# Gancheekim/ATM-VFI

Hardware: AMD Instinct MI355X
Metric: interpolated frames/s at 1080p (network_base, bs=1) (higher is better)
Workload: dtype f32 (contractions as fp16 hi/lo split x3 MFMA, fp32 accumulate; ~22 significand bits)

## Files before the change

atm-vfi_amd/csrc/api.hip:

```cpp
#include "common.h"

#include <string.h>

#include <vector>

namespace atmvfi {

static thread_local char g_err[512] = "";

void set_error(const char* fmt, ...) {
    va_list ap;
    va_start(ap, fmt);
    vsnprintf(g_err, sizeof(g_err), fmt, ap);
    va_end(ap);
}

int check_launch(const char* what) {
    const hipError_t e = hipGetLastError();
    if (e != hipSuccess) {
        set_error("%s: launch failed: %s", what, hipGetErrorString(e));
        return ATMVFI_ELAUNCH;
    }
    return ATMVFI_OK;
}

#ifdef ATMVFI_RANGE_CHECK
static std::vector<RangeWordSetter>& range_registry() {
    static std::vector<RangeWordSetter> v;
    return v;
}
void range_registry_add(RangeWordSetter s) { range_registry().push_back(s); }
#endif

}

extern "C" int atmvfi_range_word_set(uint32_t* word, void* stream) {
#ifdef ATMVFI_RANGE_CHECK
    for (atmvfi::RangeWordSetter set : atmvfi::range_registry()) {
        const int e = set(reinterpret_cast<unsigned*>(word), (hipStream_t)stream);
        ATMVFI_REQUIRE(e == 0, ATMVFI_ELAUNCH, "range_word_set: hipMemcpyToSymbolAsync failed (%d)", e);
    }
    return ATMVFI_OK;
#else
    (void)word; (void)stream;
    atmvfi::set_error("range_word_set: this is the default build; the operand range check lives in libatmvfi_hip_checked.so (make checked)");
    return ATMVFI_EINVAL;
#endif
}
extern "C" int atmvfi_range_checked(void) {
#ifdef ATMVFI_RANGE_CHECK
    return 1;
#else
    return 0;
#endif
}

extern "C" int atmvfi_version(void) { return (0 << 16) | (28 << 8) | 0; }
extern "C" const char* atmvfi_last_error(void) { return atmvfi::g_err; }
#ifndef ATMVFI_SOURCE_DIGEST
#define ATMVFI_SOURCE_DIGEST "unknown (api.hip compiled outside the Makefile)"
#endif
extern "C" const char* atmvfi_source_digest(void) { return ATMVFI_SOURCE_DIGEST; }
```

atm-vfi_amd/csrc/attention.hip:

```cpp
#include "common.h"

#include <math.h>

namespace {

__device__ __forceinline__ int slots16(int n) { return (n + 15) & ~15; }

template <int NT>
__global__ __launch_bounds__(64 * NT) void window_attn_kernel(
    const float* __restrict__ qkv, const RowSink out, float* __restrict__ motion,
    const int* __restrict__ labels, int N, int nW, int ws, int heads, int hd, int C, int Bw, int kv_shift,
    float scale) {
    fp16_saturate_on();
    extern __shared__ __attribute__((aligned(16))) float smem[];
    constexpr int NPAD = NT * 16;
    const int nchunks = (hd + 15) >> 4;
    const int DPAD = 16 * nchunks;
    const int PK = slots16(DPAD / 4), PV = slots16(NPAD / 4);
    float* Ks = smem;
    float* Vt = Ks + NPAD * PK * 4;
    int* Ls = reinterpret_cast<int*>(Vt + DPAD * PV * 4);

    const int tid = threadIdx.x;
    const int slot = blockIdx.x >> 3;
    const int b = (slot / heads) * 8 + (blockIdx.x & 7);
    const int h = slot % heads;
    if (b >= Bw) return;
    const int bk = (b + kv_shift) % Bw;
    const int C3 = 3 * C;
    const int lane = tid & 63;
    const int w = tid >> 6;
    const int r = lane & 15;
    const int g = lane >> 4;
    const int q = 16 * w + r;
    const bool qok = q < N;

    constexpr int MAXC = NT >= 13 ? 4 : 8;
    f32x4 qf[MAXC];
    const float* qrow = qkv + ((long long)b * N + (qok ? q : 0)) * C3 + h * hd;
#pragma unroll
    for (int c = 0; c < MAXC; ++c) {
        qf[c] = (f32x4){0.f, 0.f, 0.f, 0.f};
        const int d = 16 * c + 4 * g;
        if (c < nchunks && qok && d < hd) qf[c] = *reinterpret_cast<const f32x4*>(qrow + d);
    }

    const int dg = DPAD >> 2;
    constexpr int UNR = 6;
    for (int base = 0; base < NPAD * dg; base += 64 * NT * UNR) {
        f32x4 kv[UNR], vv[UNR];
        int keyv[UNR], d4v[UNR];
        bool okv[UNR];
#pragma unroll
        for (int u = 0; u < UNR; ++u) {
            const int idx = base + u * 64 * NT + tid;
            const int key = idx / dg;
            const int d4 = idx - key * dg;
            keyv[u] = key;
            d4v[u] = d4;
            okv[u] = key < N && (d4 << 2) < hd;
            const float* p = qkv + ((long long)bk * N + (okv[u] ? key : 0)) * C3 + C + h * hd + (okv[u] ? (d4 << 2) : 0);
            kv[u] = *reinterpret_cast<const f32x4*>(p);
            vv[u] = *reinterpret_cast<const f32x4*>(p + C);
        }
#pragma unroll
        for (int u = 0; u < UNR; ++u) {
            const int key = keyv[u], d4 = d4v[u], d = d4 << 2;
            if (key < NPAD) {
                const f32x4 z = (f32x4){0.f, 0.f, 0.f, 0.f};
                const f32x4 k4 = okv[u] ? kv[u] : z, v4 = okv[u] ? vv[u] : z;
                *reinterpret_cast<f32x4*>(Ks + (key * PK + (d4 ^ (key & 15))) * 4) = k4;
                const int ks = key >> 2, ke = key & 3;
#pragma unroll
                for (int e = 0; e < 4; ++e) Vt[((d + e) * PV + (ks ^ ((d + e) & 15))) * 4 + ke] = v4[e];
            }
        }
    }
    for (int idx = tid; idx < NPAD; idx += 64 * NT)
        Ls[idx] = (labels && idx < N) ? labels[(long long)(b % nW) * N + idx] : 0;
    __syncthreads();

    f32x4 s[NT];
#pragma unroll
    for (int kt = 0; kt < NT; ++kt) s[kt] = (f32x4){0.f, 0.f, 0.f, 0.f};
#pragma unroll
    for (int c = 0; c < MAXC; ++c) {
        if (c < nchunks) {
#pragma unroll
            for (int kt = 0; kt < NT; ++kt) {
                const f32x4 kf = *reinterpret_cast<const f32x4*>(Ks + ((16 * kt + r) * PK + ((4 * c + g) ^ r)) * 4);
#pragma unroll
                for (int ks = 0; ks < 4; ++ks)
                    s[kt] = __builtin_amdgcn_mfma_f32_16x16x4f32(kf[ks], qf[c][ks], s[kt], 0, 0, 0);
            }
        }
    }

    const int lab_q = Ls[qok ? q : 0];
    float mx = -INFINITY;
#pragma unroll
    for (int kt = 0; kt < NT; ++kt) {
        const int4 lk = *reinterpret_cast<const int4*>(Ls + 16 * kt + 4 * g);
        const int lks[4] = {lk.x, lk.y, lk.z, lk.w};
#pragma unroll
        for (int e = 0; e < 4; ++e) {
            const int key = 16 * kt + 4 * g + e;
            float v = s[kt][e] * scale;
// ... 3 lines not shown
            mx = fmaxf(mx, v);
        }
    }
    mx = fmaxf(mx, __shfl_xor(mx, 16));
    mx = fmaxf(mx, __shfl_xor(mx, 32));
    float sum = 0.f;
#pragma unroll
    for (int kt = 0; kt < NT; ++kt)
#pragma unroll
        for (int e = 0; e < 4; ++e) {
            const float p = expf(s[kt][e] - mx);
            s[kt][e] = p;
            sum += p;
        }
    const float inv_ws = 1.0f / (float)ws;
    sum += __shfl_xor(sum, 16);
    sum += __shfl_xor(sum, 32);
    const float inv = 1.0f / sum;
    const float qy = floorf(((float)q + 0.5f) * inv_ws), qx = (float)q - qy * (float)ws;
    float mox = 0.f, moy = 0.f;
#pragma unroll
    for (int kt = 0; kt < NT; ++kt)
#pragma unroll
        for (int e = 0; e < 4; ++e) {
            const int key = 16 * kt + 4 * g + e;
            const float p = s[kt][e] * inv;
            s[kt][e] = p;
            const float ky = floorf(((float)key + 0.5f) * inv_ws);
            mox += p * (((float)key - ky * (float)ws) - qx);
            moy += p * (ky - qy);
        }
    if (motion) {
        mox += __shfl_xor(mox, 16);
        mox += __shfl_xor(mox, 32);
        moy += __shfl_xor(moy, 16);
        moy += __shfl_xor(moy, 32);
        if (g == 0 && qok) {
            float* mp = motion + (((long long)b * N + q) * heads + h) * 2;
            mp[0] = mox;
            mp[1] = moy;
        }
    }

    const long long orow = (long long)b * N + (qok ? q : 0);
    for (int dt = 0; dt < nchunks; ++dt) {
        f32x4 o = (f32x4){0.f, 0.f, 0.f, 0.f};
#pragma unroll
        for (int kt = 0; kt < NT; ++kt) {
            const f32x4 vf = *reinterpret_cast<const f32x4*>(Vt + ((16 * dt + r) * PV + ((4 * kt + g) ^ r)) * 4);
#pragma unroll
            for (int ks = 0; ks < 4; ++ks)
                o = __builtin_amdgcn_mfma_f32_16x16x4f32(vf[ks], s[kt][ks], o, 0, 0, 0);
        }
        const int d = 16 * dt + 4 * g;
        if (qok && d < hd) sink_store4(out, orow, h * hd + d, o);
    }
}

typedef __fp16 h16x4_t __attribute__((__vector_size__(4 * sizeof(__fp16))));
__device__ __forceinline__ f16x8_t tr_pair(unsigned a0, unsigned a1) {
    const h16x4_t x = __builtin_amdgcn_ds_read_tr16_b64_v4f16((__attribute__((address_space(3))) h16x4_t*)(unsigned long long)a0);
    const h16x4_t y = __builtin_amdgcn_ds_read_tr16_b64_v4f16((__attribute__((address_space(3))) h16x4_t*)(unsigned long long)a1);
    struct Two { h16x4_t x, y; };
    return __builtin_bit_cast(f16x8_t, (Two){x, y});
}

#ifdef ATMVFI_STAMP
__device__ unsigned long long* g_attn_stamp = nullptr;
#define AT_STAMP(i)                                                     \
    do {                                                                \
        if (stamping) {                                                 \
            const unsigned long long t_ = __builtin_amdgcn_s_memtime(); \
            tacc[i] += t_ - tlast;                                      \
            tlast = t_;                                                 \
        }                                                               \
    } while (0)
#else
#define AT_STAMP(i) do { } while (0)
#endif
template <int NT, int DCH>
__global__ __launch_bounds__(64 * NT, (NT <= 4 ? 3 : NT <= 8 ? 2 : NT <= 12 ? 3 : 4)) void window_attn_x3_kernel(
    const float* __restrict__ qkv, const RowSink out, float* __restrict__ motion,
    const int* __restrict__ labels, int N, int nW, int ws, int heads, int hd, int C, int Bw, int kv_shift,
    float scale, int vitems) {
    extern __shared__ __attribute__((aligned(16))) float smem[];
    fp16_saturate_on();
    constexpr int NPAD = NT * 16, KT2 = (NT + 1) / 2, VROWS = 32 * KT2, T = 64 * NT;
    constexpr bool PERSIST = NT <= 8, PREFETCH = PERSIST, PREFETCH_Q = PERSIST;
    constexpr int UNR = 2 * DCH;
    constexpr int D32 = DCH;
    const int DT = (hd + (motion ? 4 : 0) + 15) >> 4;
    constexpr int SPK = D32 <= 1 ? 4 : D32 == 2 ? 8 : 16;
    constexpr int KS = SPK * 16;
    const int VS = 32 * DT + ((DT & 1) ? 0 : 32);
    unsigned char* Kh = reinterpret_cast<unsigned char*>(smem);
    unsigned char* Kl = Kh + NPAD * KS;
    unsigned char* Vh = Kl + NPAD * KS;
    unsigned char* Vl = Vh + VROWS * VS;
    int* Ls = reinterpret_cast<int*>(Vl + VROWS * VS);

    const int tid = threadIdx.x;
    const int C3 = 3 * C;
    const int lane = tid & 63;
    const int w = tid >> 6;
    const int r = lane & 15;
    const int g = lane >> 4;
    const int q = 16 * w + r;
    const bool qok = q < N;
    const float inv_ws = 1.0f / (float)ws;

    {
        const f32x4 z4 = (f32x4){0.f, 0.f, 0.f, 0.f};
        const f16x4 z = (f16x4){(_Float16)0.f, (_Float16)0.f, (_Float16)0.f, (_Float16)0.f};
        if constexpr (PERSIST) {
            const int words16 = (2 * NPAD * KS + 2 * VROWS * VS) >> 4;
            for (int idx = tid; idx < words16; idx += T) reinterpret_cast<f32x4*>(smem)[idx] = z4;
            __syncthreads();
        } else {
            const int dg0 = hd >> 2, kpad = 8 * DCH - dg0;
            auto kzero = [&](int row, int d4) {
                const int sw = SPK == 16 ? (row & 15) : SPK == 8 ? ((row >> 1) & 7) : ((0x1320 >> (((row >> 2) & 3) * 4)) & 3);
                const int off = row * KS + ((((d4 >> 1) ^ sw) & (SPK - 1)) << 4) + ((d4 & 1) << 3);
                *reinterpret_cast<f16x4*>(Kh + off) = z;
                *reinterpret_cast<f16x4*>(Kl + off) = z;
            };
            for (int idx = tid; idx < N * kpad; idx += T) kzero(idx / kpad, dg0 + idx % kpad);
            for (int idx = tid; idx < (NPAD - N) * 8 * DCH; idx += T) kzero(N + idx / (8 * DCH), idx % (8 * DCH));
            const int vtail16 = ((VROWS - N) * VS) >> 4;
            for (int idx = tid; idx < vtail16; idx += T) {
                reinterpret_cast<f32x4*>(Vh + N * VS)[idx] = z4;
                reinterpret_cast<f32x4*>(Vl + N * VS)[idx] = z4;
            }
        }
        if (motion && tid < N) {
            const float ky = floorf(((float)tid + 0.5f) * inv_ws), kx = (float)tid - ky * (float)ws;
            *reinterpret_cast<f16x4*>(Vh + tid * VS + (hd << 1)) = (f16x4){(_Float16)kx, (_Float16)ky, (_Float16)0.f, (_Float16)0.f};
            *reinterpret_cast<f16x4*>(Vl + tid * VS + (hd << 1)) = z;
        }
    }

    const int dgr = hd >> 2;
    const int units = N * dgr;
    const float inv_dgr = 1.0f / (float)dgr;
    constexpr int ksw_mask = SPK - 1;
    int goff[UNR], koff[UNR], voff[UNR];
    constexpr bool ROWGROUPS = DCH != 3;
    constexpr int LPR = 8 * DCH, RPP = T / LPR;
#pragma unroll
    for (int u = 0; u < UNR; ++u) {
        const int idx = u * T + tid;
        const int row = ROWGROUPS ? u * RPP + tid / LPR : (int)(((float)idx + 0.5f) * inv_dgr);
        const int d4 = ROWGROUPS ? tid % LPR : idx - row * dgr;
        const bool ok = ROWGROUPS ? (row < N && d4 < dgr) : idx < units;
        const int sw = SPK == 16 ? (row & 15) : SPK == 8 ? ((row >> 1) & 7) : ((0x1320 >> (((row >> 2) & 3) * 4)) & 3);
        goff[u] = ok ? row * C3 + (d4 << 2) : 0;
        koff[u] = ok ? row * KS + ((((d4 >> 1) ^ sw) & ksw_mask) << 4) + ((d4 & 1) << 3) : -1;
        voff[u] = row * VS + (d4 << 3);
    }

    auto item_of = [&](int v, int& b, int& h) {
        const int slot = v >> 3;
        b = (slot / heads) * 8 + (v & 7);
        h = slot % heads;
    };
    auto convert_store = [&](const f32x4 k4, const f32x4 v4, int ko, int vo) {
        f16x2 h0, l0, h1, l1;
        split_pair((f32x2){k4.x, k4.y}, h0, l0);
        split_pair((f32x2){k4.z, k4.w}, h1, l1);
        *reinterpret_cast<f16x4*>(Kh + ko) = (f16x4){h0.x, h0.y, h1.x, h1.y};
        *reinterpret_cast<f16x4*>(Kl + ko) = (f16x4){l0.x, l0.y, l1.x, l1.y};
        split_pair((f32x2){v4.x, v4.y}, h0, l0);
        split_pair((f32x2){v4.z, v4.w}, h1, l1);
        *reinterpret_cast<f16x4*>(Vh + vo) = (f16x4){h0.x, h0.y, h1.x, h1.y};
        *reinterpret_cast<f16x4*>(Vl + vo) = (f16x4){l0.x, l0.y, l1.x, l1.y};
    };

    int v = blockIdx.x, b, h;
    item_of(v, b, h);
    while (v < vitems && b >= Bw) {
        v += gridDim.x;
        item_of(v, b, h);
    }
    if (v >= vitems) return;

    f32x4 k0[UNR], v0[UNR];
    auto request0 = [&](int bb, int hh) {
        const float* kvbase = qkv + (long long)((bb + kv_shift) % Bw) * N * C3 + C + hh * hd;
#pragma unroll
        for (int u = 0; u < UNR; ++u) {
            if (ROWGROUPS ? u * RPP < N : u * T < units) {
                k0[u] = *reinterpret_cast<const f32x4*>(kvbase + goff[u]);
                v0[u] = *reinterpret_cast<const f32x4*>(kvbase + goff[u] + C);
            }
        }
    };
    request0(b, h);
    f32x4 qx[DCH][2];
    auto request_q = [&](int bb, int hh) {
        const float* qrow = qkv + ((long long)bb * N + (qok ? q : 0)) * C3 + hh * hd;
#pragma unroll
        for (int c = 0; c < DCH; ++c)
#pragma unroll
            for (int hf = 0; hf < 2; ++hf) {
                const int d = 32 * c + 8 * g + 4 * hf;
                qx[c][hf] = *reinterpret_cast<const f32x4*>(qrow + (d < hd ? d : 0));
            }
    };
    request_q(b, h);
#ifdef ATMVFI_STAMP
    const bool stamping = g_attn_stamp && blockIdx.x == 0 && tid < 64;
    unsigned long long tacc[8] = {0, 0, 0, 0, 0, 0, 0, 0}, tlast = 0, titems = 0;
#endif

    const int rsw = SPK == 16 ? r : SPK == 8 ? (r >> 1) : ((0x1320 >> ((r >> 2) * 4)) & 3);
    const unsigned vlane = (unsigned)((4 * g + ((lane >> 2) & 3)) * VS + ((lane & 3) << 3));
    const unsigned vh0 = lds_offset(Vh) + vlane, vl0 = lds_offset(Vl) + vlane;
    const float qy = floorf(((float)q + 0.5f) * inv_ws), qxc = (float)q - qy * (float)ws;
    constexpr float LOG2E = 1.4426950408889634f;
    const float sl2 = scale * LOG2E;

    for (;;) {
#ifdef ATMVFI_STAMP
        if (stamping) { tlast = __builtin_amdgcn_s_memtime(); ++titems; }
#endif
#pragma unroll
        for (int u = 0; u < UNR; ++u)
            if (koff[u] >= 0) convert_store(k0[u], v0[u], koff[u], voff[u]);
        AT_STAMP(0);
        if (labels && tid < N) Ls[tid] = labels[(long long)(b % nW) * N + tid];

        f16x8_t qh[DCH], ql[DCH];
#pragma unroll
        for (int c = 0; c < DCH; ++c) {
            if (c < D32) {
                f16x2 hh[4], ll[4];
#pragma unroll
                for (int hf = 0; hf < 2; ++hf) {
                    const bool ok = qok && (32 * c + 8 * g + 4 * hf) < hd;
                    const f32x4 x = qx[c][hf];
                    split_pair(ok ? (f32x2){x.x, x.y} : (f32x2){0.f, 0.f}, hh[2 * hf], ll[2 * hf]);
                    split_pair(ok ? (f32x2){x.z, x.w} : (f32x2){0.f, 0.f}, hh[2 * hf + 1], ll[2 * hf + 1]);
                }
                qh[c] = (f16x8_t){hh[0].x, hh[0].y, hh[1].x, hh[1].y, hh[2].x, hh[2].y, hh[3].x, hh[3].y};
                ql[c] = (f16x8_t){ll[0].x, ll[0].y, ll[1].x, ll[1].y, ll[2].x, ll[2].y, ll[3].x, ll[3].y};
// ... 91 lines not shown
        }

        AT_STAMP(5);
        const long long orow = (long long)b * N + (qok ? q : 0);
        for (int dt = 0; dt < DT; ++dt) {
            f32x4 acc = (f32x4){0.f, 0.f, 0.f, 0.f}, cor = (f32x4){0.f, 0.f, 0.f, 0.f};
#pragma unroll
            for (int k2 = 0; k2 < KT2; ++k2) {
                const unsigned o0 = (unsigned)(32 * k2 * VS + 32 * dt), o1 = o0 + (unsigned)(16 * VS);
                const f16x8_t vh = tr_pair(vh0 + o0, vh0 + o1), vl = tr_pair(vl0 + o0, vl0 + o1);
                acc = __builtin_amdgcn_mfma_f32_16x16x32_f16(vh, ph[k2], acc, 0, 0, 0);
                cor = __builtin_amdgcn_mfma_f32_16x16x32_f16(vh, pl[k2], cor, 0, 0, 0);
                cor = __builtin_amdgcn_mfma_f32_16x16x32_f16(vl, ph[k2], cor, 0, 0, 0);
            }
            const f32x4 o = (acc + cor * (1.0f / 1024.0f)) * inv;
            const int d = 16 * dt + 4 * g;
            if (qok && d < hd) sink_store4(out, orow, h * hd + d, o);
            if (motion && qok && d == hd) {
                float* mp = motion + (((long long)b * N + q) * heads + h) * 2;
                mp[0] = o[0] - qxc;
                mp[1] = o[1] - qy;
            }
        }
        AT_STAMP(6);
        if (!has_next) break;
        v = vn;
        b = bn;
        h = hn;
        if (!PREFETCH) request0(b, h);
        if (!PREFETCH_Q) request_q(b, h);
        __syncthreads();
        AT_STAMP(7);
    }
#ifdef ATMVFI_STAMP
    if (stamping && tid == 0) {
        for (int i = 0; i < 8; ++i) g_attn_stamp[i] = tacc[i];
        g_attn_stamp[8] = titems;
    }
#endif
}

__global__ void motion_head_kernel(const float* __restrict__ motion, const int* __restrict__ row_map,
                                   const float* __restrict__ w0, const float* __restrict__ b0,
                                   const float* __restrict__ w1, const float* __restrict__ b1,
                                   float* __restrict__ out, int out_ld, long long out_gstride, int out_rpg,
                                   long long rows, int heads, _Float16* __restrict__ phi, _Float16* __restrict__ plo,
                                   long long plane_rows, int pc0, int pgc) {
    fp16_saturate_on();
    const long long m = (long long)blockIdx.x * blockDim.x + threadIdx.x;
    if (m >= rows) return;
    const long long ro = row_map ? row_map[m] : m;
    if (ro < 0) return;
    const float* mp = motion + m * heads * 2;
    const int hid = heads >> 1;
    float ox = b1[0], oy = b1[0];
    for (int j = 0; j < hid; ++j) {
        float ax = b0[j], ay = b0[j];
        for (int hh = 0; hh < heads; ++hh) {
            const float wv = w0[j * heads + hh];
            ax += wv * mp[hh * 2];
            ay += wv * mp[hh * 2 + 1];
        }
        ox += w1[j] * gelu_erf(ax);
        oy += w1[j] * gelu_erf(ay);
    }
    const long long off = (out_rpg > 0) ? (ro / out_rpg) * out_gstride + (ro % out_rpg) * (long long)out_ld
                                        : ro * (long long)out_ld;
    out[off] = ox;
    out[off + 1] = oy;
    if (phi) {
        const long long grp = out_rpg > 0 ? ro / out_rpg : 0;
        const long long prow = out_rpg > 0 ? ro - grp * out_rpg : ro;
        const int c = pc0 + (int)grp * pgc;
        f16x2 h, l;
        split_pair((f32x2){ox, oy}, h, l);
        const long long poff = ((long long)(c >> 5) * plane_rows + prow) * 32 + (c & 31);
        *reinterpret_cast<f16x2*>(phi + poff) = h;
        *reinterpret_cast<f16x2*>(plo + poff) = l;
    }
}

template <int NT>
int launch_attn(const float* qkv, const RowSink out, float* motion, const int* labels, int Bw, int nW, int N, int ws,
                int heads, int hd, int kv_shift, hipStream_t s) {
    const int dpad = (hd + 15) / 16 * 16, npad = NT * 16;
    const size_t lds = ((size_t)npad * ((dpad / 4 + 15) / 16 * 16) * 4 + (size_t)dpad * ((npad / 4 + 15) / 16 * 16) * 4 + npad) * sizeof(float);
    ATMVFI_REQUIRE(hd <= (NT >= 13 ? 64 : 128), ATMVFI_EINVAL, "window_attention: head dim %d too large for a %d-token window", hd, N);
    ATMVFI_REQUIRE(lds <= 160 * 1024, ATMVFI_EINVAL,
                   "window_attention: K/V tile of %zu bytes exceeds the 160 KiB LDS (ws %d, hd %d)", lds, ws, hd);
    auto kern = window_attn_kernel<NT>;
    if (lds > 48 * 1024) {
        const hipError_t e = atmvfi::allow_dynamic_lds<window_attn_kernel<NT>>(lds);
        ATMVFI_REQUIRE(e == hipSuccess, ATMVFI_ELAUNCH, "window_attention: hipFuncSetAttribute: %s", hipGetErrorString(e));
    }
    const float scale = 1.0f / sqrtf((float)hd);
    hipLaunchKernelGGL(kern, dim3((unsigned)((Bw + 7) / 8 * 8 * heads)), dim3(64 * NT), lds, s, qkv, out, motion, labels, N, nW, ws,
                       heads, hd, heads * hd, Bw, kv_shift, scale);
    return atmvfi::check_launch("window_attention");
}

template <int NT, int DCH>
int launch_attn_x3(const float* qkv, const RowSink out, float* motion, const int* labels, int Bw, int nW, int N, int ws,
                   int heads, int hd, int kv_shift, hipStream_t s) {
    const int d32 = (hd + 31) / 32, dt = (hd + (motion ? 4 : 0) + 15) / 16, npad = NT * 16, vrows = 32 * ((NT + 1) / 2);
    const int ks = (d32 <= 1 ? 4 : d32 == 2 ? 8 : 16) * 16, vs = 32 * dt + ((dt & 1) ? 0 : 32);
    const size_t lds = 2 * (size_t)npad * ks + 2 * (size_t)vrows * vs + (size_t)npad * sizeof(int);
    ATMVFI_REQUIRE(hd <= (NT >= 13 ? 64 : 128), ATMVFI_EINVAL, "window_attention: head dim %d too large for a %d-token window", hd, N);
    ATMVFI_REQUIRE(lds <= 160 * 1024, ATMVFI_EINVAL,
                   "window_attention: K/V tile of %zu bytes exceeds the 160 KiB LDS (ws %d, hd %d)", lds, ws, hd);
    if (lds > 48 * 1024) {
        const hipError_t e = atmvfi::allow_dynamic_lds<window_attn_x3_kernel<NT, DCH>>(lds);
        ATMVFI_REQUIRE(e == hipSuccess, ATMVFI_ELAUNCH, "window_attention: hipFuncSetAttribute: %s", hipGetErrorString(e));
    }
    const float scale = 1.0f / sqrtf((float)hd);
    const int vitems = (Bw + 7) / 8 * 8 * heads;
    static std::atomic<long long> occ_cache[atmvfi::kMaxDevices];
    int dev = 0;
    const bool cached = hipGetDevice(&dev) == hipSuccess && dev >= 0 && dev < atmvfi::kMaxDevices;
    long long oc = cached ? occ_cache[dev].load(std::memory_order_relaxed) : 0;
    if ((oc >> 8) != (long long)lds || (oc & 255) == 0) {
        int n = 0;
        if (hipOccupancyMaxActiveBlocksPerMultiprocessor(&n, window_attn_x3_kernel<NT, DCH>, 64 * NT, lds) != hipSuccess || n < 1) n = 1;
        oc = ((long long)lds << 8) | (n > 255 ? 255 : n);
        if (cached) occ_cache[dev].store(oc, std::memory_order_relaxed);
    }
    const int per_cu = (int)(oc & 255);
    int grid = atmvfi::cu_count() * per_cu;
    if (grid > vitems || NT > 8) grid = vitems;
    hipLaunchKernelGGL((window_attn_x3_kernel<NT, DCH>), dim3((unsigned)grid), dim3(64 * NT), lds, s, qkv, out, motion, labels, N, nW, ws,
                       heads, hd, heads * hd, Bw, kv_shift, scale, vitems);
    return atmvfi::check_launch("window_attention_f16x3");
}

template <int NT>
int launch_attn_x3_d(const float* qkv, const RowSink out, float* motion, const int* labels, int Bw, int nW, int N, int ws,
                     int heads, int hd, int kv_shift, hipStream_t s) {
    ATMVFI_REQUIRE(hd <= (NT >= 13 ? 64 : 128), ATMVFI_EINVAL, "window_attention: head dim %d too large for a %d-token window", hd, N);
    switch ((hd + 31) / 32) {
        case 1: return launch_attn_x3<NT, 1>(qkv, out, motion, labels, Bw, nW, N, ws, heads, hd, kv_shift, s);
        case 2: return launch_attn_x3<NT, 2>(qkv, out, motion, labels, Bw, nW, N, ws, heads, hd, kv_shift, s);
    }
    if constexpr (NT <= 12) {
        if (hd <= 96) return launch_attn_x3<NT, 3>(qkv, out, motion, labels, Bw, nW, N, ws, heads, hd, kv_shift, s);
        return launch_attn_x3<NT, 4>(qkv, out, motion, labels, Bw, nW, N, ws, heads, hd, kv_shift, s);
    }
    return ATMVFI_EINVAL;
}

int attention_entry(bool x3, const float* qkv, float* out, float* motion, const int32_t* labels, int Bw, int nW, int ws, int heads,
                    int hd, int kv_shift, void* out_hi, void* out_lo, int plane_ld, void* stream) {
    ATMVFI_REQUIRE(qkv, ATMVFI_EINVAL, "window_attention: null pointer");
    ATMVFI_REQUIRE(sink_ok(out, heads * hd, heads * hd, out_hi, out_lo, plane_ld, (long long)Bw * ws * ws), ATMVFI_EALIGN,
                   "window_attention: output needs fp32 rows and/or both fp16 planes (plane rows >= Bw*ws*ws), 16-byte aligned");
    const RowSink sink{out, heads * hd, (_Float16*)out_hi, (_Float16*)out_lo, plane_ld};
    ATMVFI_REQUIRE(Bw > 0 && nW > 0 && Bw % nW == 0, ATMVFI_EINVAL, "window_attention: Bw %d must be a positive multiple of nW %d", Bw, nW);
    ATMVFI_REQUIRE(ws >= 1 && ws <= 16, ATMVFI_EINVAL, "window_attention: window size %d outside 1..16", ws);
    ATMVFI_REQUIRE(heads > 0 && hd > 0 && hd % 4 == 0 && hd <= 128, ATMVFI_EINVAL, "window_attention: head dim %d must be a multiple of 4, at most 128", hd);
    ATMVFI_REQUIRE(kv_shift >= 0 && kv_shift < Bw, ATMVFI_EINVAL, "window_attention: kv_shift out of range");
    ATMVFI_REQUIRE(atmvfi::aligned16(qkv), ATMVFI_EALIGN, "window_attention: qkv must be 16-byte aligned");
    ATMVFI_REQUIRE(((long long)Bw + 8) * heads < (1ll << 31), ATMVFI_EINVAL, "window_attention: grid too large");
    const int N = ws * ws;
    const int nt = (N + 15) / 16;
    hipStream_t s = (hipStream_t)stream;
#define ATMVFI_ATTN_CASE(k)                                                                                              \
    case k:                                                                                                              \
        return x3 ? launch_attn_x3_d<k>(qkv, sink, motion, labels, Bw, nW, N, ws, heads, hd, kv_shift, s)                 \
                  : launch_attn<k>(qkv, sink, motion, labels, Bw, nW, N, ws, heads, hd, kv_shift, s);
    switch (nt) {
        ATMVFI_ATTN_CASE(1) ATMVFI_ATTN_CASE(2) ATMVFI_ATTN_CASE(3) ATMVFI_ATTN_CASE(4) ATMVFI_ATTN_CASE(5)
        ATMVFI_ATTN_CASE(6) ATMVFI_ATTN_CASE(7) ATMVFI_ATTN_CASE(8) ATMVFI_ATTN_CASE(9) ATMVFI_ATTN_CASE(10)
        ATMVFI_ATTN_CASE(11) ATMVFI_ATTN_CASE(12) ATMVFI_ATTN_CASE(13) ATMVFI_ATTN_CASE(14) ATMVFI_ATTN_CASE(15)
        ATMVFI_ATTN_CASE(16)
    }
#undef ATMVFI_ATTN_CASE
    atmvfi::set_error("window_attention: unsupported token count %d", N);
    return ATMVFI_EINVAL;
}

}

#ifdef ATMVFI_STAMP
extern "C" int atmvfi_debug_set_attn_stamp_buffer(void* buf) {
    return hipMemcpyToSymbol(HIP_SYMBOL(g_attn_stamp), &buf, sizeof(buf)) == hipSuccess ? 0 : ATMVFI_ELAUNCH;
}
#endif

extern "C" int atmvfi_window_attention_f16x3(const float* qkv, float* out, float* motion, const int32_t* labels, int Bw,
                                              int nW, int ws, int heads, int hd, int kv_shift, void* out_hi, void* out_lo,
                                              int plane_ld, void* stream) {
    return attention_entry(true, qkv, out, motion, labels, Bw, nW, ws, heads, hd, kv_shift, out_hi, out_lo, plane_ld, stream);
}

extern "C" int atmvfi_window_attention(const float* qkv, float* out, float* motion, const int32_t* labels, int Bw,
                                        int nW, int ws, int heads, int hd, int kv_shift, void* out_hi, void* out_lo,
                                        int plane_ld, void* stream) {
    return attention_entry(false, qkv, out, motion, labels, Bw, nW, ws, heads, hd, kv_shift, out_hi, out_lo, plane_ld, stream);
}

extern "C" int atmvfi_window_attn_cross_motion(const float* qkv, float* out, float* motion, const int32_t* labels,
                                                int Bw, int nW, int ws, int heads, int hd, void* stream) {
    ATMVFI_REQUIRE(motion, ATMVFI_EINVAL, "window_attn_cross_motion: motion output required");
    ATMVFI_REQUIRE(Bw % 2 == 0, ATMVFI_EINVAL, "window_attn_cross_motion: Bw must be even (two frames)");
    return atmvfi_window_attention(qkv, out, motion, labels, Bw, nW, ws, heads, hd, Bw / 2, nullptr, nullptr, 0, stream);
}

extern "C" int atmvfi_window_attn_self(const float* qkv, float* out, const int32_t* labels, int Bw, int nW, int ws,
                                        int heads, int hd, void* stream) {
    return atmvfi_window_attention(qkv, out, nullptr, labels, Bw, nW, ws, heads, hd, 0, nullptr, nullptr, 0, stream);
}

extern "C" int atmvfi_motion_head_planes(const float* motion, const int32_t* row_map, const float* w0, const float* b0,
                                         const float* w1, const float* b1, float* out, int out_ld, int64_t out_gstride, int out_rpg,
                                         int64_t rows, int heads, void* out_hi, void* out_lo, int64_t plane_rows, int plane_c0, int plane_gc,
                                         void* stream) {
    ATMVFI_REQUIRE(motion && w0 && b0 && w1 && b1 && out, ATMVFI_EINVAL, "motion_head: null pointer");
    ATMVFI_REQUIRE(rows > 0 && heads >= 2 && heads % 2 == 0, ATMVFI_EINVAL, "motion_head: bad rows/heads");
    ATMVFI_REQUIRE((out_hi == nullptr) == (out_lo == nullptr), ATMVFI_EINVAL, "motion_head: the plane sink needs both planes");
    if (out_hi)
        ATMVFI_REQUIRE(plane_rows > 0 && plane_c0 >= 0 && plane_c0 % 2 == 0 && plane_gc % 2 == 0 && atmvfi::aligned16(out_hi) && atmvfi::aligned16(out_lo),
                       ATMVFI_EINVAL, "motion_head: plane sink needs plane_rows > 0, even channel offsets and 16-byte aligned planes");
    const unsigned blocks = (unsigned)((rows + 255) / 256);
    hipLaunchKernelGGL(motion_head_kernel, dim3(blocks), dim3(256), 0, (hipStream_t)stream, motion, row_map, w0, b0, w1,
                       b1, out, out_ld, (long long)out_gstride, out_rpg, (long long)rows, heads, (_Float16*)out_hi, (_Float16*)out_lo,
                       (long long)plane_rows, plane_c0, plane_gc);
    return atmvfi::check_launch("motion_head");
}

extern "C" int atmvfi_motion_head(const float* motion, const int32_t* row_map, const float* w0, const float* b0, const float* w1,
                                  const float* b1, float* out, int out_ld, int64_t out_gstride, int out_rpg, int64_t rows, int heads,
                                  void* stream) {
    return atmvfi_motion_head_planes(motion, row_map, w0, b0, w1, b1, out, out_ld, out_gstride, out_rpg, rows, heads, nullptr, nullptr, 0, 0,
                                     0, stream);
}
```

atm-vfi_amd/csrc/plan_dispatch.inc:

```
#define ATMVFI_PLAN_NFN 72
static const char* const kPlanFnNames[ATMVFI_PLAN_NFN] = {
    "atmvfi_conv2d",
    "atmvfi_conv3p",
    "atmvfi_conv3x3_f16x3",
    "atmvfi_deconv2x2",
    "atmvfi_dwconv3x3_gelu",
    "atmvfi_ensemble_select",
    "atmvfi_f32_to_yuv420p10",
    "atmvfi_field_bob",
    "atmvfi_field_rows",
    "atmvfi_final_residual",
    "atmvfi_flow_warp",
    "atmvfi_flow_warp_ex",
    "atmvfi_flow_warp_nhwc",
    "atmvfi_flow_warp_tiled",
    "atmvfi_flow_warp_up2",
    "atmvfi_flow_warp_up2_tiled",
    "atmvfi_frame_borders",
    "atmvfi_frame_compose",
    "atmvfi_frame_difference",
    "atmvfi_frame_f32_to_u8",
    "atmvfi_frame_half",
    "atmvfi_frame_rot180",
    "atmvfi_frame_signature",
    "atmvfi_frame_u8_to_f32",
    "atmvfi_frame_u8_window",
    "atmvfi_gemm",
    "atmvfi_head1x1_planes",
    "atmvfi_image_pyramid",
    "atmvfi_image_pyramid_pack",
    "atmvfi_l1_mean",
    "atmvfi_layernorm",
    "atmvfi_linear",
    "atmvfi_motion_head",
    "atmvfi_motion_head_planes",
    "atmvfi_pack_dw_weight",
    "atmvfi_pack_frames",
    "atmvfi_pack_weight",
    "atmvfi_pack_weight_conv3x3",
    "atmvfi_pack_weight_split",
    "atmvfi_pool_blocks",
    "atmvfi_range_word_set",
    "atmvfi_refine_tail",
    "atmvfi_resize_bilinear_ac",
    "atmvfi_rgb16_decode",
    "atmvfi_rgb16_encode",
    "atmvfi_rgb_to_yuv420",
    "atmvfi_shutter_accumulate",
    "atmvfi_shutter_resolve",
    "atmvfi_split_planes",
    "atmvfi_split_planes_at",
    "atmvfi_ssim_psnr",
    "atmvfi_stem_fused",
    "atmvfi_synth_up2",
    "atmvfi_tta_merge",
    "atmvfi_warp_blend",
    "atmvfi_warp_blend_planes",
    "atmvfi_warp_blend_tiled",
    "atmvfi_window_attention",
    "atmvfi_window_attention_f16x3",
    "atmvfi_window_attn_cross_motion",
    "atmvfi_window_attn_self",
    "atmvfi_yuv420_to_rgb",
    "atmvfi_yuv420_window",
    "atmvfi_yuv420p10_to_f32",
    "atmvfi_yuv_borders",
    "atmvfi_yuv_compose",
    "atmvfi_yuv_pack",
    "atmvfi_yuv_sub_decode",
    "atmvfi_yuv_sub_encode",
    "atmvfi_yuv_surface_decode",
    "atmvfi_yuv_surface_encode",
    "atmvfi_yuv_unpack",
};
static const int kPlanFnArgs[ATMVFI_PLAN_NFN] = {1, 1, 19, 1, 13, 13, 10, 10, 5, 8, 10, 9, 14, 10, 8, 8, 7, 15, 12, 9, 5, 5, 11, 9, 15, 1, 10, 8, 9, 7, 14, 1, 12, 17, 3, 6, 7, 5, 8, 8, 1, 10, 13, 15, 10, 13, 13, 7, 8, 10, 18, 21, 1, 11, 19, 23, 23, 13, 13, 9, 8, 14, 18, 14, 9, 24, 5, 25, 17, 24, 16, 6};
static int plan_call(const atmvfi_plan_op* op, void* stream) {
    const atmvfi_plan_arg* a = op->a;
    switch (op->fn) {
    case 0: return atmvfi_conv2d((const atmvfi_gemm_params*)(uintptr_t)a[0].u, stream);
    case 1: return atmvfi_conv3p((const atmvfi_conv3p_params*)(uintptr_t)a[0].u, stream);
    case 2: return atmvfi_conv3x3_f16x3((const float*)(uintptr_t)a[0].u, (int)a[1].i, (int)a[2].i, (int)a[3].i, (int)a[4].i, (int)a[5].i, (const void*)(uintptr_t)a[6].u, (const void*)(uintptr_t)a[7].u, (int)a[8].i, (float*)(uintptr_t)a[9].u, (int)a[10].i, (const float*)(uintptr_t)a[11].u, (const float*)(uintptr_t)a[12].u, (void*)(uintptr_t)a[13].u, (void*)(uintptr_t)a[14].u, (int64_t)a[15].i, (const float*)(uintptr_t)a[16].u, (int)a[17].i, (int)a[18].i, stream);
    case 3: return atmvfi_deconv2x2((const atmvfi_gemm_params*)(uintptr_t)a[0].u, stream);
    case 4: return atmvfi_dwconv3x3_gelu((const float*)(uintptr_t)a[0].u, (int)a[1].i, (float*)(uintptr_t)a[2].u, (int)a[3].i, (const float*)(uintptr_t)a[4].u, (const float*)(uintptr_t)a[5].u, (int)a[6].i, (int)a[7].i, (int)a[8].i, (int)a[9].i, (void*)(uintptr_t)a[10].u, (void*)(uintptr_t)a[11].u, (int)a[12].i, stream);
    case 5: return atmvfi_ensemble_select((const float*)(uintptr_t)a[0].u, (const float*)(uintptr_t)a[1].u, (const float*)(uintptr_t)a[2].u, (const float*)(uintptr_t)a[3].u, (const float*)(uintptr_t)a[4].u, (const float*)(uintptr_t)a[5].u, (const float*)(uintptr_t)a[6].u, (const float*)(uintptr_t)a[7].u, (const float*)(uintptr_t)a[8].u, (float*)(uintptr_t)a[9].u, (float*)(uintptr_t)a[10].u, (int)a[11].i, (int64_t)a[12].i, stream);
    case 6: return atmvfi_f32_to_yuv420p10((const float*)(uintptr_t)a[0].u, (int)a[1].i, (int)a[2].i, (int)a[3].i, (int)a[4].i, (int)a[5].i, (int)a[6].i, (int)a[7].i, (int)a[8].i, (void*)(uintptr_t)a[9].u, stream);
    case 7: return atmvfi_field_bob((const float*)(uintptr_t)a[0].u, (float*)(uintptr_t)a[1].u, (float*)(uintptr_t)a[2].u, (int)a[3].i, (int)a[4].i, (int)a[5].i, (int)a[6].i, (int)a[7].i, (int)a[8].i, (int)a[9].i, stream);
    case 8: return atmvfi_field_rows((void*)(uintptr_t)a[0].u, (const void*)(uintptr_t)a[1].u, (int)a[2].i, (const int64_t*)(uintptr_t)a[3].u, (int)a[4].i, stream);
    case 9: return atmvfi_final_residual((const float*)(uintptr_t)a[0].u, (const float*)(uintptr_t)a[1].u, (int)a[2].i, (float*)(uintptr_t)a[3].u, (float*)(uintptr_t)a[4].u, (int)a[5].i, (int)a[6].i, (int)a[7].i, stream);
    case 10: return atmvfi_flow_warp((const float*)(uintptr_t)a[0].u, (const float*)(uintptr_t)a[1].u, (int64_t)a[2].i, (int)a[3].i, (int)a[4].i, (float*)(uintptr_t)a[5].u, (int)a[6].i, (int)a[7].i, (int)a[8].i, (int)a[9].i, stream);
    case 11: return atmvfi_flow_warp_ex((const float*)(uintptr_t)a[0].u, (const float*)(uintptr_t)a[1].u, (float*)(uintptr_t)a[2].u, (uint8_t*)(uintptr_t)a[3].u, (int)a[4].i, (int)a[5].i, (int)a[6].i, (int)a[7].i, (int)a[8].i, stream);
    case 12: return atmvfi_flow_warp_nhwc((const float*)(uintptr_t)a[0].u, (int)a[1].i, (int64_t)a[2].i, (const float*)(uintptr_t)a[3].u, (int64_t)a[4].i, (int)a[5].i, (int)a[6].i, (float*)(uintptr_t)a[7].u, (int)a[8].i, (int64_t)a[9].i, (int)a[10].i, (int)a[11].i, (int)a[12].i, (int)a[13].i, stream);
    case 13: return atmvfi_flow_warp_tiled((const float*)(uintptr_t)a[0].u, (const float*)(uintptr_t)a[1].u, (int64_t)a[2].i, (int)a[3].i, (int)a[4].i, (float*)(uintptr_t)a[5].u, (int)a[6].i, (int)a[7].i, (int)a[8].i, (int)a[9].i, stream);
    case 14: return atmvfi_flow_warp_up2((const float*)(uintptr_t)a[0].u, (const float*)(uintptr_t)a[1].u, (float*)(uintptr_t)a[2].u, (float*)(uintptr_t)a[3].u, (int)a[4].i, (int)a[5].i, (int)a[6].i, (int)a[7].i, stream);
    case 15: return atmvfi_flow_warp_up2_tiled((const float*)(uintptr_t)a[0].u, (const float*)(uintptr_t)a[1].u, (float*)(uintptr_t)a[2].u, (float*)(uintptr_t)a[3].u, (int)a[4].i, (int)a[5].i, (int)a[6].i, (int)a[7].i, stream);
    case 16: return atmvfi_frame_borders((const void*)(uintptr_t)a[0].u, (int)a[1].i, (int)a[2].i, (int)a[3].i, (int32_t*)(uintptr_t)a[4].u, (int32_t*)(uintptr_t)a[5].u, (int64_t)a[6].i, stream);
    case 17: return atmvfi_frame_compose((void*)(uintptr_t)a[0].u, (const void*)(uintptr_t)a[1].u, (int)a[2].i, (int)a[3].i, (int)a[4].i, (int)a[5].i, (int)a[6].i, (int)a[7].i, (const float*)(uintptr_t)a[8].u, (int)a[9].i, (int)a[10].i, (int)a[11].i, (int)a[12].i, (const void*)(uintptr_t)a[13].u, (int)a[14].i, stream);
    case 18: return atmvfi_frame_difference((const void*)(uintptr_t)a[0].u, (const void*)(uintptr_t)a[1].u, (int)a[2].i, (int)a[3].i, (int)a[4].i, (int)a[5].i, (int)a[6].i, (int)a[7].i, (int)a[8].i, (int32_t*)(uintptr_t)a[9].u, (int32_t*)(uintptr_t)a[10].u, (int64_t)a[11].i, stream);
    case 19: return atmvfi_frame_f32_to_u8((const float*)(uintptr_t)a[0].u, (int)a[1].i, (int)a[2].i, (int)a[3].i, (int)a[4].i, (void*)(uintptr_t)a[5].u, (int)a[6].i, (int)a[7].i, (int)a[8].i, stream);
    case 20: return atmvfi_frame_half((const float*)(uintptr_t)a[0].u, (float*)(uintptr_t)a[1].u, (int)a[2].i, (int)a[3].i, (int)a[4].i, stream);
    case 21: return atmvfi_frame_rot180((const float*)(uintptr_t)a[0].u, (float*)(uintptr_t)a[1].u, (int)a[2].i, (int)a[3].i, (int)a[4].i, stream);
    case 22: return atmvfi_frame_signature((const void*)(uintptr_t)a[0].u, (int)a[1].i, (int)a[2].i, (int)a[3].i, (int)a[4].i, (int)a[5].i, (int)a[6].i, (int)a[7].i, (int32_t*)(uintptr_t)a[8].u, (int32_t*)(uintptr_t)a[9].u, (int64_t)a[10].i, stream);
    case 23: return atmvfi_frame_u8_to_f32((const void*)(uintptr_t)a[0].u, (int)a[1].i, (int)a[2].i, (int)a[3].i, (float*)(uintptr_t)a[4].u, (int)a[5].i, (int)a[6].i, (int)a[7].i, (int)a[8].i, stream);
    case 24: return atmvfi_frame_u8_window((const void*)(uintptr_t)a[0].u, (int)a[1].i, (int)a[2].i, (int)a[3].i, (int)a[4].i, (int)a[5].i, (int)a[6].i, (int)a[7].i, (int)a[8].i, (float*)(uintptr_t)a[9].u, (int)a[10].i, (int)a[11].i, (int)a[12].i, (int)a[13].i, (void*)(uintptr_t)a[14].u, stream);
    case 25: return atmvfi_gemm((const atmvfi_gemm_params*)(uintptr_t)a[0].u, stream);
    case 26: return atmvfi_head1x1_planes((const void*)(uintptr_t)a[0].u, (const void*)(uintptr_t)a[1].u, (int64_t)a[2].i, (int64_t)a[3].i, (int)a[4].i, (const float*)(uintptr_t)a[5].u, (const float*)(uintptr_t)a[6].u, (int)a[7].i, (float*)(uintptr_t)a[8].u, (int)a[9].i, stream);
    case 27: return atmvfi_image_pyramid((const float*)(uintptr_t)a[0].u, (const float*)(uintptr_t)a[1].u, (float*)(uintptr_t)a[2].u, (float*)(uintptr_t)a[3].u, (float*)(uintptr_t)a[4].u, (int)a[5].i, (int)a[6].i, (int)a[7].i, stream);
    case 28: return atmvfi_image_pyramid_pack((const float*)(uintptr_t)a[0].u, (const float*)(uintptr_t)a[1].u, (float*)(uintptr_t)a[2].u, (float*)(uintptr_t)a[3].u, (float*)(uintptr_t)a[4].u, (float*)(uintptr_t)a[5].u, (int)a[6].i, (int)a[7].i, (int)a[8].i, stream);
    case 29: return atmvfi_l1_mean((const float*)(uintptr_t)a[0].u, (const float*)(uintptr_t)a[1].u, (float*)(uintptr_t)a[2].u, (int)a[3].i, (int64_t)a[4].i, (float*)(uintptr_t)a[5].u, (int64_t)a[6].i, stream);
    case 30: return atmvfi_layernorm((const float*)(uintptr_t)a[0].u, (int)a[1].i, (int64_t)a[2].i, (int)a[3].i, (const int32_t*)(uintptr_t)a[4].u, (float*)(uintptr_t)a[5].u, (int)a[6].i, (const float*)(uintptr_t)a[7].u, (const float*)(uintptr_t)a[8].u, (int64_t)a[9].i, (int)a[10].i, (void*)(uintptr_t)a[11].u, (void*)(uintptr_t)a[12].u, (int)a[13].i, stream);
    case 31: return atmvfi_linear((const atmvfi_gemm_params*)(uintptr_t)a[0].u, stream);
    case 32: return atmvfi_motion_head((const float*)(uintptr_t)a[0].u, (const int32_t*)(uintptr_t)a[1].u, (const float*)(uintptr_t)a[2].u, (const float*)(uintptr_t)a[3].u, (const float*)(uintptr_t)a[4].u, (const float*)(uintptr_t)a[5].u, (float*)(uintptr_t)a[6].u, (int)a[7].i, (int64_t)a[8].i, (int)a[9].i, (int64_t)a[10].i, (int)a[11].i, stream);
    case 33: return atmvfi_motion_head_planes((const float*)(uintptr_t)a[0].u, (const int32_t*)(uintptr_t)a[1].u, (const float*)(uintptr_t)a[2].u, (const float*)(uintptr_t)a[3].u, (const float*)(uintptr_t)a[4].u, (const float*)(uintptr_t)a[5].u, (float*)(uintptr_t)a[6].u, (int)a[7].i, (int64_t)a[8].i, (int)a[9].i, (int64_t)a[10].i, (int)a[11].i, (void*)(uintptr_t)a[12].u, (void*)(uintptr_t)a[13].u, (int64_t)a[14].i, (int)a[15].i, (int)a[16].i, stream);
    case 34: return atmvfi_pack_dw_weight((const float*)(uintptr_t)a[0].u, (float*)(uintptr_t)a[1].u, (int)a[2].i, stream);
    case 35: return atmvfi_pack_frames((const float*)(uintptr_t)a[0].u, (const float*)(uintptr_t)a[1].u, (float*)(uintptr_t)a[2].u, (int)a[3].i, (int)a[4].i, (int)a[5].i, stream);
    case 36: return atmvfi_pack_weight((int)a[0].i, (const float*)(uintptr_t)a[1].u, (float*)(uintptr_t)a[2].u, (int)a[3].i, (int)a[4].i, (int)a[5].i, (int)a[6].i, stream);
    case 37: return atmvfi_pack_weight_conv3x3((const float*)(uintptr_t)a[0].u, (void*)(uintptr_t)a[1].u, (void*)(uintptr_t)a[2].u, (int)a[3].i, (int)a[4].i, stream);
    case 38: return atmvfi_pack_weight_split((int)a[0].i, (const float*)(uintptr_t)a[1].u, (void*)(uintptr_t)a[2].u, (void*)(uintptr_t)a[3].u, (int)a[4].i, (int)a[5].i, (int)a[6].i, (int)a[7].i, stream);
    case 39: return atmvfi_pool_blocks((void*)(uintptr_t)a[0].u, (int64_t)a[1].i, (int)a[2].i, (const int32_t*)(uintptr_t)a[3].u, (int)a[4].i, (int64_t)a[5].i, (void*)(uintptr_t)a[6].u, (int)a[7].i, stream);
    case 40: return atmvfi_range_word_set((uint32_t*)(uintptr_t)a[0].u, stream);
    case 41: return atmvfi_refine_tail((const float*)(uintptr_t)a[0].u, (int64_t)a[1].i, (const float*)(uintptr_t)a[2].u, (const float*)(uintptr_t)a[3].u, (const float*)(uintptr_t)a[4].u, (float*)(uintptr_t)a[5].u, (float*)(uintptr_t)a[6].u, (int)a[7].i, (int)a[8].i, (int)a[9].i, stream);
    case 42: return atmvfi_resize_bilinear_ac((const float*)(uintptr_t)a[0].u, (int64_t)a[1].i, (int64_t)a[2].i, (int64_t)a[3].i, (int64_t)a[4].i, (float*)(uintptr_t)a[5].u, (int)a[6].i, (int)a[7].i, (int)a[8].i, (int)a[9].i, (int)a[10].i, (int)a[11].i, (float)a[12].f, stream);
    case 43: return atmvfi_rgb16_decode((const void*)(uintptr_t)a[0].u, (int)a[1].i, (int)a[2].i, (int)a[3].i, (int)a[4].i, (int)a[5].i, (int)a[6].i, (int)a[7].i, (int)a[8].i, (float*)(uintptr_t)a[9].u, (int)a[10].i, (int)a[11].i, (int)a[12].i, (int)a[13].i, (void*)(uintptr_t)a[14].u, stream);
    case 44: return atmvfi_rgb16_encode((const float*)(uintptr_t)a[0].u, (int)a[1].i, (int)a[2].i, (int)a[3].i, (int)a[4].i, (void*)(uintptr_t)a[5].u, (int)a[6].i, (int)a[7].i, (int)a[8].i, (int)a[9].i, stream);
    case 45: return atmvfi_rgb_to_yuv420((const void*)(uintptr_t)a[0].u, (int)a[1].i, (const float*)(uintptr_t)a[2].u, (int)a[3].i, (int)a[4].i, (int)a[5].i, (int)a[6].i, (int)a[7].i, (int)a[8].i, (int)a[9].i, (int)a[10].i, (int)a[11].i, (void*)(uintptr_t)a[12].u, stream);
    case 46: return atmvfi_shutter_accumulate((int32_t*)(uintptr_t)a[0].u, (int)a[1].i, (int)a[2].i, (const float*)(uintptr_t)a[3].u, (int)a[4].i, (int)a[5].i, (int)a[6].i, (int)a[7].i, (const uint8_t*)(uintptr_t)a[8].u, (int)a[9].i, (int)a[10].i, (int)a[11].i, (int)a[12].i, stream);
    case 47: return atmvfi_shutter_resolve((const int32_t*)(uintptr_t)a[0].u, (int)a[1].i, (int)a[2].i, (int)a[3].i, (int)a[4].i, (uint8_t*)(uintptr_t)a[5].u, (int)a[6].i, stream);
    case 48: return atmvfi_split_planes((const float*)(uintptr_t)a[0].u, (int)a[1].i, (int64_t)a[2].i, (int)a[3].i, (const float*)(uintptr_t)a[4].u, (void*)(uintptr_t)a[5].u, (void*)(uintptr_t)a[6].u, (int)a[7].i, stream);
    case 49: return atmvfi_split_planes_at((const float*)(uintptr_t)a[0].u, (int)a[1].i, (int64_t)a[2].i, (int)a[3].i, (const float*)(uintptr_t)a[4].u, (void*)(uintptr_t)a[5].u, (void*)(uintptr_t)a[6].u, (int)a[7].i, (int)a[8].i, (int)a[9].i, stream);
    case 50: return atmvfi_ssim_psnr((const void*)(uintptr_t)a[0].u, (int64_t)a[1].i, (int64_t)a[2].i, (int64_t)a[3].i, (int64_t)a[4].i, (const float*)(uintptr_t)a[5].u, (int64_t)a[6].i, (int64_t)a[7].i, (int64_t)a[8].i, (int64_t)a[9].i, (int)a[10].i, (int)a[11].i, (int)a[12].i, (float)a[13].f, (int)a[14].i, (double*)(uintptr_t)a[15].u, (float*)(uintptr_t)a[16].u, (int64_t)a[17].i, stream);
    case 51: return atmvfi_stem_fused((const float*)(uintptr_t)a[0].u, (int)a[1].i, (int)a[2].i, (int)a[3].i, (int)a[4].i, (int)a[5].i, (const void*)(uintptr_t)a[6].u, (const void*)(uintptr_t)a[7].u, (const float*)(uintptr_t)a[8].u, (const float*)(uintptr_t)a[9].u, (const void*)(uintptr_t)a[10].u, (const void*)(uintptr_t)a[11].u, (const float*)(uintptr_t)a[12].u, (const float*)(uintptr_t)a[13].u, (const void*)(uintptr_t)a[14].u, (const void*)(uintptr_t)a[15].u, (const float*)(uintptr_t)a[16].u, (const float*)(uintptr_t)a[17].u, (void*)(uintptr_t)a[18].u, (void*)(uintptr_t)a[19].u, (int64_t)a[20].i, stream);
    case 52: return atmvfi_synth_up2((const atmvfi_synth_up2_params*)(uintptr_t)a[0].u, stream);
    case 53: return atmvfi_tta_merge((const float*)(uintptr_t)a[0].u, (const float*)(uintptr_t)a[1].u, (float*)(uintptr_t)a[2].u, (void*)(uintptr_t)a[3].u, (int)a[4].i, (int)a[5].i, (int)a[6].i, (int)a[7].i, (int)a[8].i, (int)a[9].i, (int)a[10].i, stream);
    case 54: return atmvfi_warp_blend((const float*)(uintptr_t)a[0].u, (const float*)(uintptr_t)a[1].u, (const float*)(uintptr_t)a[2].u, (int)a[3].i, (int64_t)a[4].i, (float*)(uintptr_t)a[5].u, (float*)(uintptr_t)a[6].u, (float*)(uintptr_t)a[7].u, (float*)(uintptr_t)a[8].u, (float*)(uintptr_t)a[9].u, (float*)(uintptr_t)a[10].u, (float*)(uintptr_t)a[11].u, (const float*)(uintptr_t)a[12].u, (const float*)(uintptr_t)a[13].u, (float*)(uintptr_t)a[14].u, (int)a[15].i, (int)a[16].i, (int)a[17].i, (int)a[18].i, stream);
    case 55: return atmvfi_warp_blend_planes((const float*)(uintptr_t)a[0].u, (const float*)(uintptr_t)a[1].u, (const float*)(uintptr_t)a[2].u, (int)a[3].i, (int64_t)a[4].i, (float*)(uintptr_t)a[5].u, (float*)(uintptr_t)a[6].u, (float*)(uintptr_t)a[7].u, (float*)(uintptr_t)a[8].u, (float*)(uintptr_t)a[9].u, (float*)(uintptr_t)a[10].u, (float*)(uintptr_t)a[11].u, (const float*)(uintptr_t)a[12].u, (const float*)(uintptr_t)a[13].u, (float*)(uintptr_t)a[14].u, (int)a[15].i, (void*)(uintptr_t)a[16].u, (void*)(uintptr_t)a[17].u, (int64_t)a[18].i, (int)a[19].i, (int)a[20].i, (int)a[21].i, (int)a[22].i, stream);
    case 56: return atmvfi_warp_blend_tiled((const float*)(uintptr_t)a[0].u, (const float*)(uintptr_t)a[1].u, (const float*)(uintptr_t)a[2].u, (int)a[3].i, (int64_t)a[4].i, (float*)(uintptr_t)a[5].u, (float*)(uintptr_t)a[6].u, (float*)(uintptr_t)a[7].u, (float*)(uintptr_t)a[8].u, (float*)(uintptr_t)a[9].u, (float*)(uintptr_t)a[10].u, (float*)(uintptr_t)a[11].u, (const float*)(uintptr_t)a[12].u, (const float*)(uintptr_t)a[13].u, (float*)(uintptr_t)a[14].u, (int)a[15].i, (void*)(uintptr_t)a[16].u, (void*)(uintptr_t)a[17].u, (int64_t)a[18].i, (int)a[19].i, (int)a[20].i, (int)a[21].i, (int)a[22].i, stream);
    case 57: return atmvfi_window_attention((const float*)(uintptr_t)a[0].u, (float*)(uintptr_t)a[1].u, (float*)(uintptr_t)a[2].u, (const int32_t*)(uintptr_t)a[3].u, (int)a[4].i, (int)a[5].i, (int)a[6].i, (int)a[7].i, (int)a[8].i, (int)a[9].i, (void*)(uintptr_t)a[10].u, (void*)(uintptr_t)a[11].u, (int)a[12].i, stream);
    case 58: return atmvfi_window_attention_f16x3((const float*)(uintptr_t)a[0].u, (float*)(uintptr_t)a[1].u, (float*)(uintptr_t)a[2].u, (const int32_t*)(uintptr_t)a[3].u, (int)a[4].i, (int)a[5].i, (int)a[6].i, (int)a[7].i, (int)a[8].i, (int)a[9].i, (void*)(uintptr_t)a[10].u, (void*)(uintptr_t)a[11].u, (int)a[12].i, stream);
    case 59: return atmvfi_window_attn_cross_motion((const float*)(uintptr_t)a[0].u, (float*)(uintptr_t)a[1].u, (float*)(uintptr_t)a[2].u, (const int32_t*)(uintptr_t)a[3].u, (int)a[4].i, (int)a[5].i, (int)a[6].i, (int)a[7].i, (int)a[8].i, stream);
    case 60: return atmvfi_window_attn_self((const float*)(uintptr_t)a[0].u, (float*)(uintptr_t)a[1].u, (const int32_t*)(uintptr_t)a[2].u, (int)a[3].i, (int)a[4].i, (int)a[5].i, (int)a[6].i, (int)a[7].i, stream);
    case 61: return atmvfi_yuv420_to_rgb((const void*)(uintptr_t)a[0].u, (int)a[1].i, (int)a[2].i, (int)a[3].i, (int)a[4].i, (int)a[5].i, (int)a[6].i, (void*)(uintptr_t)a[7].u, (int)a[8].i, (float*)(uintptr_t)a[9].u, (int)a[10].i, (int)a[11].i, (int)a[12].i, (int)a[13].i, stream);
    case 62: return atmvfi_yuv420_window((const void*)(uintptr_t)a[0].u, (int)a[1].i, (int)a[2].i, (int)a[3].i, (int)a[4].i, (int)a[5].i, (int)a[6].i, (int)a[7].i, (int)a[8].i, (int)a[9].i, (int)a[10].i, (int)a[11].i, (float*)(uintptr_t)a[12].u, (int)a[13].i, (int)a[14].i, (int)a[15].i, (int)a[16].i, (void*)(uintptr_t)a[17].u, stream);
    case 63: return atmvfi_yuv420p10_to_f32((const void*)(uintptr_t)a[0].u, (int)a[1].i, (int)a[2].i, (int)a[3].i, (int)a[4].i, (int)a[5].i, (int)a[6].i, (int)a[7].i, (int)a[8].i, (float*)(uintptr_t)a[9].u, (int)a[10].i, (int)a[11].i, (int)a[12].i, (int)a[13].i, stream);
    case 64: return atmvfi_yuv_borders((const void*)(uintptr_t)a[0].u, (int)a[1].i, (int)a[2].i, (int)a[3].i, (int)a[4].i, (int64_t)a[5].i, (int32_t*)(uintptr_t)a[6].u, (int32_t*)(uintptr_t)a[7].u, (int64_t)a[8].i, stream);
    case 65: return atmvfi_yuv_compose((void*)(uintptr_t)a[0].u, (const void*)(uintptr_t)a[1].u, (int)a[2].i, (int)a[3].i, (int)a[4].i, (int)a[5].i, (int)a[6].i, (int)a[7].i, (int)a[8].i, (int)a[9].i, (int)a[10].i, (int64_t)a[11].i, (int64_t)a[12].i, (int64_t)a[13].i, (int)a[14].i, (int)a[15].i, (int)a[16].i, (int)a[17].i, (const float*)(uintptr_t)a[18].u, (int)a[19].i, (int)a[20].i, (int)a[21].i, (int)a[22].i, (const void*)(uintptr_t)a[23].u, stream);
    case 66: return atmvfi_yuv_pack((const void*)(uintptr_t)a[0].u, (int)a[1].i, (int)a[2].i, (int)a[3].i, (void*)(uintptr_t)a[4].u, stream);
    case 67: return atmvfi_yuv_sub_decode((const void*)(uintptr_t)a[0].u, (int)a[1].i, (int)a[2].i, (int)a[3].i, (int)a[4].i, (int)a[5].i, (int)a[6].i, (int)a[7].i, (int)a[8].i, (int)a[9].i, (int64_t)a[10].i, (int64_t)a[11].i, (int64_t)a[12].i, (int)a[13].i, (int)a[14].i, (int)a[15].i, (int)a[16].i, (int)a[17].i, (void*)(uintptr_t)a[18].u, (int)a[19].i, (float*)(uintptr_t)a[20].u, (int)a[21].i, (int)a[22].i, (int)a[23].i, (int)a[24].i, stream);
    case 68: return atmvfi_yuv_sub_encode((const void*)(uintptr_t)a[0].u, (int)a[1].i, (const float*)(uintptr_t)a[2].u, (int)a[3].i, (int)a[4].i, (int)a[5].i, (int)a[6].i, (int)a[7].i, (int)a[8].i, (int)a[9].i, (int)a[10].i, (int)a[11].i, (int)a[12].i, (int)a[13].i, (int)a[14].i, (int)a[15].i, (void*)(uintptr_t)a[16].u, stream);
    case 69: return atmvfi_yuv_surface_decode((const void*)(uintptr_t)a[0].u, (int)a[1].i, (int)a[2].i, (int)a[3].i, (int)a[4].i, (int)a[5].i, (int)a[6].i, (int)a[7].i, (int)a[8].i, (int64_t)a[9].i, (int64_t)a[10].i, (int64_t)a[11].i, (int)a[12].i, (int)a[13].i, (int)a[14].i, (int)a[15].i, (int)a[16].i, (void*)(uintptr_t)a[17].u, (int)a[18].i, (float*)(uintptr_t)a[19].u, (int)a[20].i, (int)a[21].i, (int)a[22].i, (int)a[23].i, stream);
    case 70: return atmvfi_yuv_surface_encode((const void*)(uintptr_t)a[0].u, (int)a[1].i, (const float*)(uintptr_t)a[2].u, (int)a[3].i, (int)a[4].i, (int)a[5].i, (int)a[6].i, (int)a[7].i, (int)a[8].i, (int)a[9].i, (int)a[10].i, (int)a[11].i, (int)a[12].i, (int)a[13].i, (int)a[14].i, (void*)(uintptr_t)a[15].u, stream);
    case 71: return atmvfi_yuv_unpack((const void*)(uintptr_t)a[0].u, (int)a[1].i, (int)a[2].i, (int)a[3].i, (int64_t)a[4].i, (void*)(uintptr_t)a[5].u, stream);
    default: break;
    }
    atmvfi::set_error("plan_run: unknown function id %d", op->fn);
    return ATMVFI_EINVAL;
}
```

atm-vfi_amd/csrc/pointwise.hip:

```cpp
#include "common.h"

#include <math.h>
#include <stdlib.h>

namespace {

__global__ __launch_bounds__(256) void layernorm_kernel(const float* __restrict__ in, int in_ld, long long in_gstride,
                                                        int in_rpg, const int* __restrict__ src_map,
                                                        const RowSink out,
                                                        const float* __restrict__ gamma, const float* __restrict__ beta,
                                                        long long rows, int C) {
    fp16_saturate_on();
    const int lane = threadIdx.x & 63;
    const long long row = (long long)blockIdx.x * 4 + (threadIdx.x >> 6);
    if (row >= rows) return;
    const int c4n = C >> 2;
    long long src = src_map ? src_map[row] : row;
    if (src < 0) {
        for (int i = lane; i < c4n; i += 64)
            sink_store4(out, row, 4 * i, *reinterpret_cast<const f32x4*>(beta + 4 * i));
        return;
    }
    const float* irow = in + ((in_rpg > 0) ? (src / in_rpg) * in_gstride + (src % in_rpg) * (long long)in_ld
                                           : src * (long long)in_ld);
    if (c4n <= 128) {
        const bool has1 = lane + 64 < c4n, has0 = lane < c4n;
        const f32x4 z = (f32x4){0.f, 0.f, 0.f, 0.f};
        const f32x4 v0 = has0 ? *reinterpret_cast<const f32x4*>(irow + 4 * lane) : z;
        const f32x4 v1 = has1 ? *reinterpret_cast<const f32x4*>(irow + 4 * (lane + 64)) : z;
        float sum = 0.f;
        if (has0) sum += (v0.x + v0.y) + (v0.z + v0.w);
        if (has1) sum += (v1.x + v1.y) + (v1.z + v1.w);
#pragma unroll
        for (int o = 32; o > 0; o >>= 1) sum += __shfl_xor(sum, o);
        const float mean = sum / (float)C;
        float sq = 0.f;
        if (has0) {
            const float a = v0.x - mean, b = v0.y - mean, c = v0.z - mean, d = v0.w - mean;
            sq += (a * a + b * b) + (c * c + d * d);
        }
        if (has1) {
            const float a = v1.x - mean, b = v1.y - mean, c = v1.z - mean, d = v1.w - mean;
            sq += (a * a + b * b) + (c * c + d * d);
        }
#pragma unroll
        for (int o = 32; o > 0; o >>= 1) sq += __shfl_xor(sq, o);
        const float rstd = 1.0f / sqrtf(sq / (float)C + 1e-5f);
#pragma unroll
        for (int k = 0; k < 2; ++k) {
            const int i = lane + 64 * k;
            if (k == 0 ? has0 : has1) {
                const f32x4 v = k == 0 ? v0 : v1;
                const f32x4 gm = *reinterpret_cast<const f32x4*>(gamma + 4 * i);
                const f32x4 bt = *reinterpret_cast<const f32x4*>(beta + 4 * i);
                f32x4 y;
                y.x = (v.x - mean) * rstd * gm.x + bt.x;
                y.y = (v.y - mean) * rstd * gm.y + bt.y;
                y.z = (v.z - mean) * rstd * gm.z + bt.z;
                y.w = (v.w - mean) * rstd * gm.w + bt.w;
                sink_store4(out, row, 4 * i, y);
            }
        }
        return;
    }
    float sum = 0.f;
    for (int i = lane; i < c4n; i += 64) {
        const f32x4 v = *reinterpret_cast<const f32x4*>(irow + 4 * i);
        sum += (v.x + v.y) + (v.z + v.w);
    }
#pragma unroll
    for (int o = 32; o > 0; o >>= 1) sum += __shfl_xor(sum, o);
    const float mean = sum / (float)C;
    float sq = 0.f;
    for (int i = lane; i < c4n; i += 64) {
        const f32x4 v = *reinterpret_cast<const f32x4*>(irow + 4 * i);
        const float a = v.x - mean, b = v.y - mean, c = v.z - mean, d = v.w - mean;
        sq += (a * a + b * b) + (c * c + d * d);
    }
#pragma unroll
    for (int o = 32; o > 0; o >>= 1) sq += __shfl_xor(sq, o);
    const float rstd = 1.0f / sqrtf(sq / (float)C + 1e-5f);
    for (int i = lane; i < c4n; i += 64) {
        const f32x4 v = *reinterpret_cast<const f32x4*>(irow + 4 * i);
        const f32x4 gm = *reinterpret_cast<const f32x4*>(gamma + 4 * i);
        const f32x4 bt = *reinterpret_cast<const f32x4*>(beta + 4 * i);
        f32x4 y;
        y.x = (v.x - mean) * rstd * gm.x + bt.x;
        y.y = (v.y - mean) * rstd * gm.y + bt.y;
        y.z = (v.z - mean) * rstd * gm.z + bt.z;
        y.w = (v.w - mean) * rstd * gm.w + bt.w;
        sink_store4(out, row, 4 * i, y);
    }
}

__global__ __launch_bounds__(256) void dwconv_gelu_kernel(const float* __restrict__ in, int in_ld,
                                                          const RowSink out,
                                                          const float* __restrict__ w9, const float* __restrict__ bias,
                                                          int N, int H, int W, int C) {
    fp16_saturate_on();
    const int c4n = C >> 2;
    const long long total = (long long)N * H * W * c4n;
    for (long long idx = (long long)blockIdx.x * blockDim.x + threadIdx.x; idx < total;
         idx += (long long)gridDim.x * blockDim.x) {
        const int c = (int)(idx % c4n) << 2;
        const long long pix = idx / c4n;
        const int x = (int)(pix % W);
        const int y = (int)((pix / W) % H);
        f32x4 acc = *reinterpret_cast<const f32x4*>(bias + c);
#pragma unroll
        for (int ky = 0; ky < 3; ++ky) {
            const int yy = y + ky - 1;
            if ((unsigned)yy >= (unsigned)H) continue;
#pragma unroll
            for (int kx = 0; kx < 3; ++kx) {
                const int xx = x + kx - 1;
                if ((unsigned)xx >= (unsigned)W) continue;
                const f32x4 v = *reinterpret_cast<const f32x4*>(in + (pix + (long long)(ky - 1) * W + (kx - 1)) * in_ld + c);
                const f32x4 wv = *reinterpret_cast<const f32x4*>(w9 + (ky * 3 + kx) * C + c);
                acc.x += v.x * wv.x;
                acc.y += v.y * wv.y;
                acc.z += v.z * wv.z;
                acc.w += v.w * wv.w;
            }
        }
        f32x4 o;
        o.x = gelu_erf2(acc.x);
        o.y = gelu_erf2(acc.y);
        o.z = gelu_erf2(acc.z);
        o.w = gelu_erf2(acc.w);
        sink_store4(out, pix, c, o);
    }
}

template <int RS>
__global__ __launch_bounds__(256) void dwconv_gelu_rows_kernel(const float* __restrict__ in, int in_ld,
                                                               const RowSink out,
                                                               const float* __restrict__ w9, const float* __restrict__ bias,
                                                               int N, int H, int W, int C, int xblocks, int cblocks, int strips) {
    fp16_saturate_on();
    int bid = blockIdx.x;
    const int cb = bid % cblocks; bid /= cblocks;
    const int xb = bid % xblocks; bid /= xblocks;
    const int sb = bid % strips;
    const int n = bid / strips;
    const int c = (cb * 16 + (threadIdx.x & 15)) << 2;
    const int x = xb * 16 + (threadIdx.x >> 4);
    if (x >= W) return;
    const int y0 = sb * RS;
    f32x4 wv[9];
#pragma unroll
    for (int t = 0; t < 9; ++t) wv[t] = *reinterpret_cast<const f32x4*>(w9 + t * C + c);
    const f32x4 bv = *reinterpret_cast<const f32x4*>(bias + c);
    const bool xm_ok = x > 0, xp_ok = x + 1 < W;
    const float* base = in + ((long long)n * H * W + x) * in_ld + c;
    const f32x4 zero = (f32x4){0.f, 0.f, 0.f, 0.f};
#pragma unroll
    for (int ky = 0; ky < 3; ++ky) {
        if (!xm_ok) wv[ky * 3 + 0] = zero;
        if (!xp_ok) wv[ky * 3 + 2] = zero;
    }
    auto run = [&](auto interior_tag, auto xedge_tag) {
        constexpr bool INTERIOR = decltype(interior_tag)::value;
        constexpr bool XEDGE = decltype(xedge_tag)::value;
        f32x4 win[4][3];
        const long long xm = xm_ok ? in_ld : 0, xp = xp_ok ? in_ld : 0;
        auto load_row = [&](int y, f32x4 (&dst)[3]) {
            if (INTERIOR || (unsigned)y < (unsigned)H) {
                const float* p = base + (long long)y * W * in_ld;
                dst[0] = *reinterpret_cast<const f32x4*>(p - xm);
                dst[1] = *reinterpret_cast<const f32x4*>(p);
                dst[2] = *reinterpret_cast<const f32x4*>(p + xp);
            } else {
                dst[0] = zero; dst[1] = zero; dst[2] = zero;
            }
        };
        load_row(y0 - 1, win[0]);
        load_row(y0, win[1]);
        load_row(y0 + 1, win[2]);
#pragma unroll
        for (int r = 0; r < RS; ++r) {
            const int y = y0 + r;
            if (r + 1 < RS) load_row(y + 2, win[(r + 3) % 4]);
            if (INTERIOR || y < H) {
                f32x2 a01 = bv.xy, a23 = bv.zw;
#pragma unroll
                for (int ky = 0; ky < 3; ++ky) {
                    const f32x4* row = win[(r + ky) % 4];
#pragma unroll
                    for (int kx = 0; kx < 3; ++kx) {
                        f32x4 v = row[kx];
                        const f32x4 wt = wv[ky * 3 + kx];
                        if (XEDGE && kx != 1) v = (kx == 0 ? xm_ok : xp_ok) ? v : zero;
                        a01 = __builtin_elementwise_fma(v.xy, wt.xy, a01);
                        a23 = __builtin_elementwise_fma(v.zw, wt.zw, a23);
                    }
                }
                const f32x4 acc = {a01.x, a01.y, a23.x, a23.y};
                f32x4 o;
                o.x = gelu_erf2(acc.x);
                o.y = gelu_erf2(acc.y);
                o.z = gelu_erf2(acc.z);
                o.w = gelu_erf2(acc.w);
                sink_store4(out, ((long long)n * H + y) * W + x, c, o);
            }
        }
    };
    const bool xedge = xb == 0 || xb == xblocks - 1;
    if (y0 >= 1 && y0 + RS + 1 <= H) {
        if (xedge) run(std::true_type{}, std::true_type{});
        else run(std::true_type{}, std::false_type{});
    } else {
        if (xedge) run(std::false_type{}, std::true_type{});
        else run(std::false_type{}, std::false_type{});
    }
}

constexpr int DW_RING = 6;
constexpr int DW_SLOT = 10 * 128;
template <int OFF>
__device__ __forceinline__ void lds_read4f(f32x4& d, unsigned addr) {
    static_assert(OFF >= 0 && OFF < 65536, "ds_read offset field is 16 bits");
    asm volatile("ds_read_b128 %0, %1 offset:%2" : "=v"(d) : "v"(addr), "n"(OFF) : "memory");
}
template <int N>
__device__ __forceinline__ void wait_vmcnt() { asm volatile("s_waitcnt vmcnt(%0)" ::"n"(N) : "memory"); }
template <int RS>
constexpr int dw_behind(int j) {
    const int rows = RS + 2;
    int n = 0;
    if (j < DW_RING) {
        n += 2 * ((DW_RING < rows ? DW_RING : rows) - 1 - j);
        for (int i = 0; i < j; ++i) n += (i + DW_RING < rows ? 2 : 0) + (i >= 2 ? 2 : 0);
    } else {
        const int i0 = j - DW_RING;
        n += i0 >= 2 ? 2 : 0;
        for (int i = i0 + 1; i < j; ++i) n += (i + DW_RING < rows ? 2 : 0) + (i >= 2 ? 2 : 0);
    }
    return n;
}
template <int RS>
__global__ __launch_bounds__(256) void dwconv_gelu_dma_kernel(const float* __restrict__ in, int in_ld, _Float16* __restrict__ out_hi,
                                                              _Float16* __restrict__ out_lo, long long plane_rows,
                                                              const float* __restrict__ w9, const float* __restrict__ bias, int N, int H,
                                                              int W, int C, int xgroups, int cblocks, int strips) {
    static_assert(RS + 2 >= DW_RING, "the prologue fills the whole ring");
    fp16_saturate_on();
    extern __shared__ __attribute__((aligned(16))) unsigned char dw_smem[];
    const int lane = threadIdx.x & 63;
    const int wave = __builtin_amdgcn_readfirstlane(threadIdx.x >> 6);
    unsigned u = blockIdx.x * 4u + (unsigned)wave;
    const int xg = (int)(u % (unsigned)xgroups); u /= (unsigned)xgroups;
    const int cbk = (int)(u % (unsigned)cblocks); u /= (unsigned)cblocks;
    const int sb = (int)(u % (unsigned)strips);
    const int n = (int)(u / (unsigned)strips);
    if (n >= N) return;
    int y0 = sb * RS;
    if (y0 + RS > H) y0 = H - RS;
    const int c = cbk * 32 + ((lane & 7) << 2);
    const int x = xg * 8 + (lane >> 3);
    unsigned char* ring = dw_smem + wave * (DW_RING * DW_SLOT);
    const unsigned rd = lds_offset(ring) + (unsigned)(lane * 16);

    f32x4 wv[9];
#pragma unroll
    for (int t = 0; t < 9; ++t) wv[t] = *reinterpret_cast<const f32x4*>(w9 + t * C + c);
    f32x4 bv = *reinterpret_cast<const f32x4*>(bias + c);
    const f32x4 zero = (f32x4){0.f, 0.f, 0.f, 0.f};
    const bool xm_ok = x > 0, xp_ok = x + 1 < W;
    auto clampx = [&](int xx) { return xx < 0 ? 0 : (xx >= W ? W - 1 : xx); };
    const int xa = clampx(xg * 8 - 1 + (lane >> 3));
    const int xb = clampx(xg * 8 + 7 + ((lane >> 3) & 1));
    const long long img = (long long)n * H * W;
    const float* src_a = in + (img + xa) * in_ld + c;
    const float* src_b = in + (img + xb) * in_ld + c;
    const long long row_stride = (long long)W * in_ld;
    auto issue_row = [&](int j) {
        int y = y0 - 1 + j;
        y = y < 0 ? 0 : (y >= H ? H - 1 : y);
        unsigned char* dst = ring + (j % DW_RING) * DW_SLOT;
        __builtin_amdgcn_global_load_lds((const __attribute__((address_space(1))) void*)(src_a + y * row_stride),
                                         (__attribute__((address_space(3))) void*)dst, 16, 0, 0);
        unsigned keep_m0;
        unsigned long long keep_exec;
        asm volatile("s_mov_b32 %0, m0\n\t"
                     "s_mov_b64 %1, exec\n\t"
                     "s_mov_b32 m0, %3\n\t"
                     "s_mov_b64 exec, 0xffff\n\t"
                     "global_load_lds_dwordx4 %2, off\n\t"
                     "s_mov_b64 exec, %1\n\t"
                     "s_mov_b32 m0, %0"
                     : "=&s"(keep_m0), "=&s"(keep_exec)
                     : "v"(src_b + y * row_stride), "s"(lds_offset(dst + 1024))
                     : "memory");
    };
    const bool top = y0 == 0, bottom = y0 + RS == H;
    const long long orow0 = img + (long long)y0 * W + x;
    const long long obase = ((long long)(c >> 5) * plane_rows) * 32 + (c & 31);
    __builtin_amdgcn_sched_barrier(0);
#pragma unroll
    for (int j = 0; j < DW_RING; ++j) issue_row(j);
    __builtin_amdgcn_sched_barrier(0);
#pragma unroll
    for (int ky = 0; ky < 3; ++ky) {
        if (!xm_ok) wv[ky * 3 + 0] = zero;
        if (!xp_ok) wv[ky * 3 + 2] = zero;
    }

    auto run = [&](auto xedge_tag) {
        constexpr bool XEDGE = decltype(xedge_tag)::value;
        f32x4 win[3][3];
        static_for<0, RS + 2>([&](auto jc) {
            constexpr int j = decltype(jc)::value;
            constexpr int slot = (j % DW_RING) * DW_SLOT;
            wait_vmcnt<dw_behind<RS>(j)>();
            lds_read4f<slot>(win[j % 3][0], rd);
            lds_read4f<slot + 128>(win[j % 3][1], rd);
            lds_read4f<slot + 256>(win[j % 3][2], rd);
            asm volatile("s_waitcnt lgkmcnt(0)" : "+v"(win[j % 3][0]), "+v"(win[j % 3][1]), "+v"(win[j % 3][2])::"memory");
            __builtin_amdgcn_sched_barrier(0);
            if constexpr (j + DW_RING < RS + 2) issue_row(j + DW_RING);
            __builtin_amdgcn_sched_barrier(0);
            if constexpr (j == 0) {
                if (top) { win[0][0] = zero; win[0][1] = zero; win[0][2] = zero; }
            }
            if constexpr (j == RS + 1) {
                if (bottom) { win[j % 3][0] = zero; win[j % 3][1] = zero; win[j % 3][2] = zero; }
            }
            if constexpr (j >= 2) {
                constexpr int r = j - 2;
                f32x2 a01 = bv.xy, a23 = bv.zw;
#pragma unroll
                for (int ky = 0; ky < 3; ++ky) {
                    const f32x4* row = win[(r + ky) % 3];
// ... 105 lines not shown
    const float s0 = slope ? slope[0] : 1.f, s1 = slope ? slope[1] : 1.f, s2 = slope ? slope[2] : 1.f;
    for (long long idx = (long long)blockIdx.x * blockDim.x + threadIdx.x; idx < total;
         idx += (long long)gridDim.x * blockDim.x) {
        const int b = (int)(idx / hw);
        const long long pix = idx - (long long)b * hw;
        const int y = (int)(pix / W), x = (int)(pix - (long long)y * W);
        float a0 = 0.f, a1 = 0.f, a2 = 0.f;
#pragma unroll
        for (int ky = 0; ky < 3; ++ky)
#pragma unroll
            for (int kx = 0; kx < 3; ++kx) {
                const int yy = y + ky - 1, xx = x + kx - 1;
                if ((unsigned)yy < (unsigned)H && (unsigned)xx < (unsigned)W) {
                    const float* tp = T + (long long)((ky * 3 + kx) * 3) * plane + idx + (long long)(ky - 1) * W + (kx - 1);
                    a0 += tp[0];
                    a1 += tp[plane];
                    a2 += tp[2 * plane];
                }
            }
        float r[3] = {a0 + b0, a1 + b1, a2 + b2};
        r[0] = r[0] > 0.f ? r[0] : s0 * r[0];
        r[1] = r[1] > 0.f ? r[1] : s1 * r[1];
        r[2] = r[2] > 0.f ? r[2] : s2 * r[2];
#pragma unroll
        for (int ch = 0; ch < 3; ++ch) {
            const long long o = ((long long)b * 3 + ch) * hw + pix;
            const float v = it[o] + (2.0f * sigmoidf_(r[ch]) - 1.0f);
            it_sum[o] = v;
            it_clamped[o] = fminf(fmaxf(v, 0.0f), 1.0f);
        }
    }
}

__global__ __launch_bounds__(256) void l1_partial_kernel(const float* __restrict__ a, const float* __restrict__ b,
                                                         float* __restrict__ part, long long per_sample) {
    __shared__ float red[4];
    const int s = blockIdx.y;
    const float* pa = a + (long long)s * per_sample;
    const float* pb = b + (long long)s * per_sample;
    float acc = 0.f;
    for (long long i = (long long)blockIdx.x * blockDim.x + threadIdx.x; i < per_sample; i += (long long)gridDim.x * blockDim.x)
        acc += fabsf(pa[i] - pb[i]);
#pragma unroll
    for (int o = 32; o > 0; o >>= 1) acc += __shfl_xor(acc, o);
    if ((threadIdx.x & 63) == 0) red[threadIdx.x >> 6] = acc;
    __syncthreads();
    if (threadIdx.x == 0) part[(long long)s * gridDim.x + blockIdx.x] = ((red[0] + red[1]) + red[2]) + red[3];
}
__global__ __launch_bounds__(256) void l1_final_kernel(const float* __restrict__ part, int nparts, float* __restrict__ out, long long per_sample) {
    __shared__ float red[4];
    const int s = blockIdx.x;
    float acc = 0.f;
    for (int i = threadIdx.x; i < nparts; i += blockDim.x) acc += part[(long long)s * nparts + i];
#pragma unroll
    for (int o = 32; o > 0; o >>= 1) acc += __shfl_xor(acc, o);
    if ((threadIdx.x & 63) == 0) red[threadIdx.x >> 6] = acc;
    __syncthreads();
    if (threadIdx.x == 0) out[s] = (((red[0] + red[1]) + red[2]) + red[3]) / (float)per_sample;
}

__global__ __launch_bounds__(256) void ensemble_select_kernel(const float* __restrict__ l0, const float* __restrict__ l1, const float* __restrict__ l2,
                                                              const float* __restrict__ a0, const float* __restrict__ b0,
                                                              const float* __restrict__ a1, const float* __restrict__ b1,
                                                              const float* __restrict__ a2, const float* __restrict__ b2,
                                                              float* __restrict__ out0, float* __restrict__ out1, int B, long long per_sample) {
    fp16_saturate_on();
    const long long total = (long long)B * per_sample;
    for (long long idx = (long long)blockIdx.x * blockDim.x + threadIdx.x; idx < total; idx += (long long)gridDim.x * blockDim.x) {
        const int s = (int)(idx / per_sample);
        const float x0 = l0[s], x1 = l1[s], x2 = l2[s];
        float mn = x0;
        if (x1 < mn) mn = x1;
        if (x2 < mn) mn = x2;
        const int pick = x0 == mn ? 0 : (x1 == mn ? 1 : 2);
        out0[idx] = pick == 0 ? a0[idx] : (pick == 1 ? a1[idx] : a2[idx]);
        out1[idx] = pick == 0 ? b0[idx] : (pick == 1 ? b1[idx] : b2[idx]);
    }
}

}

extern "C" int atmvfi_layernorm(const float* in, int in_ld, int64_t in_gstride, int in_rpg, const int32_t* src_row_map,
                                 float* out, int out_ld, const float* gamma, const float* beta, int64_t rows, int C,
                                 void* out_hi, void* out_lo, int plane_ld, void* stream) {
    ATMVFI_REQUIRE(in && gamma && beta, ATMVFI_EINVAL, "layernorm: null pointer");
    ATMVFI_REQUIRE(rows > 0 && C > 0 && C % 4 == 0, ATMVFI_EINVAL, "layernorm: C %d must be a positive multiple of 4", C);
    ATMVFI_REQUIRE(in_ld % 4 == 0 && in_ld >= C && in_gstride % 4 == 0, ATMVFI_EALIGN,
                   "layernorm: leading dimensions must be multiples of 4 and >= C");
    ATMVFI_REQUIRE(sink_ok(out, out_ld, C, out_hi, out_lo, plane_ld, rows), ATMVFI_EALIGN,
                   "layernorm: output needs fp32 rows (ld %% 4 == 0, >= C) and/or both fp16 planes (plane rows >= rows), 16-byte aligned");
    ATMVFI_REQUIRE(atmvfi::aligned16(in) && atmvfi::aligned16(gamma) && atmvfi::aligned16(beta),
                   ATMVFI_EALIGN, "layernorm: pointers must be 16-byte aligned");
    const unsigned blocks = (unsigned)((rows + 3) / 4);
    const RowSink sink{out, out_ld, (_Float16*)out_hi, (_Float16*)out_lo, plane_ld};
    hipLaunchKernelGGL(layernorm_kernel, dim3(blocks), dim3(256), 0, (hipStream_t)stream, in, in_ld, (long long)in_gstride,
                       in_rpg, src_row_map, sink, gamma, beta, (long long)rows, C);
    return atmvfi::check_launch("layernorm");
}

extern "C" int atmvfi_dwconv3x3_gelu(const float* in, int in_ld, float* out, int out_ld, const float* weight9,
                                      const float* bias, int N, int H, int W, int C, void* out_hi, void* out_lo,
                                      int plane_ld, void* stream) {
    ATMVFI_REQUIRE(in && weight9 && bias, ATMVFI_EINVAL, "dwconv3x3_gelu: null pointer");
    ATMVFI_REQUIRE(N > 0 && H > 0 && W > 0 && C > 0 && C % 4 == 0, ATMVFI_EINVAL, "dwconv3x3_gelu: bad shape");
    ATMVFI_REQUIRE(in_ld % 4 == 0 && in_ld >= C, ATMVFI_EALIGN, "dwconv3x3_gelu: bad ld");
    ATMVFI_REQUIRE(sink_ok(out, out_ld, C, out_hi, out_lo, plane_ld, (long long)N * H * W), ATMVFI_EALIGN,
                   "dwconv3x3_gelu: output needs fp32 rows (ld %% 4 == 0, >= C) and/or both fp16 planes (plane rows >= N*H*W), 16-byte aligned");
    const RowSink sink{out, out_ld, (_Float16*)out_hi, (_Float16*)out_lo, plane_ld};
    ATMVFI_REQUIRE(atmvfi::aligned16(in) && atmvfi::aligned16(out) && atmvfi::aligned16(weight9) && atmvfi::aligned16(bias),
                   ATMVFI_EALIGN, "dwconv3x3_gelu: pointers must be 16-byte aligned");
#if defined(ATMVFI_ABLATE)
    static const bool rows_only = getenv("ATMVFI_DWCONV_ROWS") != nullptr;
#else
    constexpr bool rows_only = false;
#endif
    if (!out && C % 64 == 0 && H >= 8 && !rows_only) {
        const int xgroups = (W + 7) / 8, cblocks = C / 32;
        int RS = H % 17 == 0 ? 17 : H % 16 == 0 ? 16 : H % 8 == 0 ? 8 : H >= 16 ? 16 : 8;
        if ((long long)N * ((H + RS - 1) / RS) * xgroups * cblocks < 8ll * atmvfi::cu_count()) RS = 8;
        const int strips = (H + RS - 1) / RS;
        const long long units = (long long)N * strips * xgroups * cblocks;
        const long long blocks = (units + 3) / 4;
        ATMVFI_REQUIRE(units < (1ll << 31), ATMVFI_EINVAL, "dwconv3x3_gelu: grid too large");
        const size_t lds = 4 * DW_RING * DW_SLOT;
        auto go = [&](auto kern) {
            hipLaunchKernelGGL(kern, dim3((unsigned)blocks), dim3(256), lds, (hipStream_t)stream, in, in_ld, (_Float16*)out_hi,
                               (_Float16*)out_lo, (long long)plane_ld, weight9, bias, N, H, W, C, xgroups, cblocks, strips);
        };
        if (RS == 17) go(dwconv_gelu_dma_kernel<17>);
        else if (RS == 16) go(dwconv_gelu_dma_kernel<16>);
        else go(dwconv_gelu_dma_kernel<8>);
        return atmvfi::check_launch("dwconv3x3_gelu");
    }
    if (C % 64 == 0) {
        const int xblocks = (W + 15) / 16, cblocks = C / 64;
        const bool tall = (long long)N * ((H + 15) / 16) * xblocks * cblocks >= 8ll * atmvfi::cu_count();
        const int RS = tall ? 16 : 8;
        const int strips = (H + RS - 1) / RS;
        const long long blocks = (long long)N * strips * xblocks * cblocks;
        ATMVFI_REQUIRE(blocks < (1ll << 31), ATMVFI_EINVAL, "dwconv3x3_gelu: grid too large");
        if (tall)
            hipLaunchKernelGGL(dwconv_gelu_rows_kernel<16>, dim3((unsigned)blocks), dim3(256), 0, (hipStream_t)stream, in, in_ld, sink,
                               weight9, bias, N, H, W, C, xblocks, cblocks, strips);
        else
            hipLaunchKernelGGL(dwconv_gelu_rows_kernel<8>, dim3((unsigned)blocks), dim3(256), 0, (hipStream_t)stream, in, in_ld, sink,
                               weight9, bias, N, H, W, C, xblocks, cblocks, strips);
        return atmvfi::check_launch("dwconv3x3_gelu");
    }
    const long long total = (long long)N * H * W * (C / 4);
    hipLaunchKernelGGL(dwconv_gelu_kernel, dim3(grid_for(total)), dim3(256), 0, (hipStream_t)stream, in, in_ld, sink,
                       weight9, bias, N, H, W, C);
    return atmvfi::check_launch("dwconv3x3_gelu");
}

extern "C" int atmvfi_pack_dw_weight(const float* src, float* dst, int C, void* stream) {
    ATMVFI_REQUIRE(src && dst && C > 0, ATMVFI_EINVAL, "pack_dw_weight: bad arguments");
    hipLaunchKernelGGL(pack_dw_kernel, dim3((9 * C + 255) / 256), dim3(256), 0, (hipStream_t)stream, src, dst, C);
    return atmvfi::check_launch("pack_dw_weight");
}

extern "C" int atmvfi_frame_u8_to_f32(const void* src, int H, int W, int bgr, float* dst, int Hp, int Wp, int pad_top, int pad_left,
                                       void* stream) {
    ATMVFI_REQUIRE(src && dst && H > 0 && W > 0 && Hp >= H && Wp >= W && pad_top >= 0 && pad_left >= 0 && pad_top + H <= Hp &&
                       pad_left + W <= Wp,
                   ATMVFI_EINVAL, "frame_u8_to_f32: bad geometry (H %d W %d -> Hp %d Wp %d, pad %d %d)", H, W, Hp, Wp, pad_top, pad_left);
    hipLaunchKernelGGL(frame_u8_to_f32_kernel, dim3(grid_for((long long)Hp * Wp)), dim3(256), 0, (hipStream_t)stream,
                       (const unsigned char*)src, H, W, bgr, dst, Hp, Wp, pad_top, pad_left);
    return atmvfi::check_launch("frame_u8_to_f32");
}

extern "C" int atmvfi_frame_f32_to_u8(const float* src, int Hp, int Wp, int pad_top, int pad_left, void* dst, int H, int W, int bgr,
                                       void* stream) {
    ATMVFI_REQUIRE(src && dst && H > 0 && W > 0 && Hp >= H && Wp >= W && pad_top >= 0 && pad_left >= 0 && pad_top + H <= Hp &&
                       pad_left + W <= Wp,
                   ATMVFI_EINVAL, "frame_f32_to_u8: bad geometry (Hp %d Wp %d -> H %d W %d, pad %d %d)", Hp, Wp, H, W, pad_top, pad_left);
    hipLaunchKernelGGL(frame_f32_to_u8_kernel, dim3(grid_for((long long)H * W)), dim3(256), 0, (hipStream_t)stream, src, Hp, Wp,
                       pad_top, pad_left, (unsigned char*)dst, H, W, bgr);
    return atmvfi::check_launch("frame_f32_to_u8");
}

extern "C" int atmvfi_final_residual(const float* it, const float* r, int r_ld, float* it_sum, float* it_clamped, int B,
                                      int H, int W, void* stream) {
    ATMVFI_REQUIRE(it && r && it_sum && it_clamped && B > 0 && H > 0 && W > 0 && r_ld >= 3, ATMVFI_EINVAL,
                   "final_residual: bad arguments");
    hipLaunchKernelGGL(final_residual_kernel, dim3(grid_for((long long)B * H * W)), dim3(256), 0, (hipStream_t)stream, it, r,
                       r_ld, it_sum, it_clamped, B, H, W);
    return atmvfi::check_launch("final_residual");
}

extern "C" int atmvfi_refine_tail(const float* contrib, int64_t contrib_plane, const float* bias, const float* slope, const float* it,
                                  float* it_sum, float* it_clamped, int B, int H, int W, void* stream) {
    ATMVFI_REQUIRE(contrib && it && it_sum && it_clamped && B > 0 && H > 0 && W > 0 && contrib_plane >= (int64_t)B * H * W, ATMVFI_EINVAL,
                   "refine_tail: bad arguments");
    hipLaunchKernelGGL(refine_tail_kernel, dim3(grid_for((long long)B * H * W)), dim3(256), 0, (hipStream_t)stream, contrib,
                       (long long)contrib_plane, bias, slope, it, it_sum, it_clamped, B, H, W);
    return atmvfi::check_launch("refine_tail");
}

extern "C" int atmvfi_ensemble_select(const float* loss0, const float* loss1, const float* loss2, const float* c0_l0, const float* c1_l0,
                                      const float* c0_l1, const float* c1_l1, const float* c0_l2, const float* c1_l2, float* out0, float* out1, int B,
                                      int64_t per_sample, void* stream) {
    ATMVFI_REQUIRE(loss0 && loss1 && loss2 && c0_l0 && c1_l0 && c0_l1 && c1_l1 && c0_l2 && c1_l2 && out0 && out1 && B > 0 && per_sample > 0,
                   ATMVFI_EINVAL, "ensemble_select: bad arguments");
    hipLaunchKernelGGL(ensemble_select_kernel, dim3(grid_for((long long)B * per_sample)), dim3(256), 0, (hipStream_t)stream, loss0, loss1, loss2,
                       c0_l0, c1_l0, c0_l1, c1_l1, c0_l2, c1_l2, out0, out1, B, (long long)per_sample);
    return atmvfi::check_launch("ensemble_select");
}

static int l1_mean_blocks(int64_t per_sample) {
    long long bx = (per_sample + 256 * 16 - 1) / (256 * 16);
    return (int)(bx > 1024 ? 1024 : bx);
}
extern "C" int64_t atmvfi_l1_mean_workspace_floats(int B, int64_t per_sample) {
    return (B > 0 && per_sample > 0) ? (int64_t)B * l1_mean_blocks(per_sample) : 0;
}
extern "C" int atmvfi_l1_mean(const float* a, const float* b, float* out, int B, int64_t per_sample, float* workspace, int64_t workspace_floats,
                              void* stream) {
    ATMVFI_REQUIRE(a && b && out && B > 0 && per_sample > 0, ATMVFI_EINVAL, "l1_mean: bad arguments");
    const int bx = l1_mean_blocks(per_sample);
    ATMVFI_REQUIRE(workspace && workspace_floats >= (int64_t)B * bx, ATMVFI_EINVAL,
                   "l1_mean: needs a workspace of atmvfi_l1_mean_workspace_floats(B, per_sample) = %lld floats", (long long)B * bx);
    hipLaunchKernelGGL(l1_partial_kernel, dim3((unsigned)bx, (unsigned)B), dim3(256), 0, (hipStream_t)stream, a, b, workspace,
                       (long long)per_sample);
    hipLaunchKernelGGL(l1_final_kernel, dim3((unsigned)B), dim3(256), 0, (hipStream_t)stream, workspace, bx, out, (long long)per_sample);
    return atmvfi::check_launch("l1_mean");
}
```

atm-vfi_amd/hip_ops.py:

```python
from __future__ import annotations

import ctypes
import os
from dataclasses import dataclass
from typing import List, Optional

import torch

from .pixfmt import DeepRGB, Packed, Surface, _not_420, _origin_error, as_surface

_HERE = os.path.dirname(os.path.abspath(__file__))
LIB_PATH = os.path.join(_HERE, "libatmvfi_hip.so")
CHECKED_LIB_PATH = os.path.join(_HERE, "libatmvfi_hip_checked.so")

GEMM_CONV, GEMM_LINEAR, GEMM_DECONV = 0, 1, 2

c_f = ctypes.c_void_p
c_i = ctypes.c_int
C_SLOTS = ctypes.POINTER(ctypes.c_int32)
c_l = ctypes.c_int64


class HipLibraryMissing(RuntimeError):
    pass
# ... 3 lines not shown
    _fields_ = [
        ("mode", ctypes.c_int32),
        ("in_", c_f), ("in_ld", ctypes.c_int32), ("N", ctypes.c_int32), ("H", ctypes.c_int32),
        ("W", ctypes.c_int32), ("Cin", ctypes.c_int32),
        ("in_gstride", ctypes.c_int64), ("in_rpg", ctypes.c_int32),
        ("weight", c_f),
        ("Cout", ctypes.c_int32), ("kh", ctypes.c_int32), ("kw", ctypes.c_int32), ("stride", ctypes.c_int32),
        ("pad", ctypes.c_int32), ("dil", ctypes.c_int32),
        ("Ho", ctypes.c_int32), ("Wo", ctypes.c_int32),
        ("M", ctypes.c_int64),
        ("out", c_f), ("out_ld", ctypes.c_int32),
        ("out_gstride", ctypes.c_int64), ("out_rpg", ctypes.c_int32),
        ("out_row_map", c_f),
        ("bias", c_f), ("prelu", c_f), ("in_prelu", c_f), ("residual", c_f),
        ("res_ld", ctypes.c_int32),
        ("precision", ctypes.c_int32), ("weight_hi", c_f), ("weight_lo", c_f),
        ("in_hi", c_f), ("in_lo", c_f),
        ("out_hi", c_f), ("out_lo", c_f), ("out_plane_rows", ctypes.c_int64), ("out_plane_c0", ctypes.c_int32),
        ("out_plane_gc", ctypes.c_int32), ("tile_wn", ctypes.c_int32),
        ("in_hi2", c_f), ("in_lo2", c_f), ("in_ld2", ctypes.c_int32), ("in_split_chunks", ctypes.c_int32),
        ("workspace", c_f), ("workspace_floats", ctypes.c_int64),
    ]


class Conv3pParams(ctypes.Structure):
    _fields_ = [
        ("in_hi", c_f), ("in_lo", c_f), ("in_rows", ctypes.c_int64),
        ("N", ctypes.c_int32), ("H", ctypes.c_int32), ("W", ctypes.c_int32), ("Cin", ctypes.c_int32),
        ("w_hi", c_f), ("w_lo", c_f), ("Cout", ctypes.c_int32),
        ("bias", c_f), ("prelu", c_f),
        ("out", c_f), ("out_ld", ctypes.c_int32), ("out_cmin", ctypes.c_int32),
        ("out_hi", c_f), ("out_lo", c_f), ("plane_rows", ctypes.c_int64), ("out_c0", ctypes.c_int32), ("plane_prelu", c_f),
        ("out_hi2", c_f), ("out_lo2", c_f), ("plane_rows2", ctypes.c_int64), ("out_c02", ctypes.c_int32),
        ("wn", ctypes.c_int32), ("workspace", c_f), ("workspace_floats", ctypes.c_int64),
        ("readout_w", c_f), ("readout", c_f), ("readout_plane", ctypes.c_int64),
        ("terms", ctypes.c_int32),
    ]


class PlanArg(ctypes.Union):
    _fields_ = [("u", ctypes.c_uint64), ("i", ctypes.c_int64), ("f", ctypes.c_double)]


PLAN_MAX_ARGS = 28


class PlanOp(ctypes.Structure):
    _fields_ = [("fn", ctypes.c_int32), ("nargs", ctypes.c_int32), ("a", PlanArg * PLAN_MAX_ARGS)]


class PlanPatch(ctypes.Structure):
    _fields_ = [("op", ctypes.c_int32), ("arg", ctypes.c_int32), ("slot", ctypes.c_int32), ("reserved", ctypes.c_int32),
                ("offset", ctypes.c_int64)]


SIGNATURES = {
    "atmvfi_version": (c_i, []),
    "atmvfi_last_error": (ctypes.c_char_p, []),
    "atmvfi_source_digest": (ctypes.c_char_p, []),
    "atmvfi_range_word_set": (c_i, [c_f, c_f]),
    "atmvfi_range_checked": (c_i, []),
    "atmvfi_gemm": (c_i, [ctypes.POINTER(GemmParams), c_f]),
    "atmvfi_gemm_workspace_floats": (c_l, [c_l, c_i, c_i]),
    "atmvfi_split_planes": (c_i, [c_f, c_i, c_l, c_i, c_f, c_f, c_f, c_i, c_f]),
    "atmvfi_split_planes_at": (c_i, [c_f, c_i, c_l, c_i, c_f, c_f, c_f, c_i, c_i, c_i, c_f]),
    "atmvfi_conv2d": (c_i, [ctypes.POINTER(GemmParams), c_f]),
    "atmvfi_linear": (c_i, [ctypes.POINTER(GemmParams), c_f]),
    "atmvfi_deconv2x2": (c_i, [ctypes.POINTER(GemmParams), c_f]),
    "atmvfi_packed_weight_floats": (c_l, [c_i, c_i, c_i, c_i, c_i]),
    "atmvfi_pack_weight": (c_i, [c_i, c_f, c_f, c_i, c_i, c_i, c_i, c_f]),
    "atmvfi_split_weight_halves": (c_l, [c_i, c_i, c_i, c_i, c_i]),
    "atmvfi_pack_weight_split": (c_i, [c_i, c_f, c_f, c_f, c_i, c_i, c_i, c_i, c_f]),
    "atmvfi_conv3x3_weight_halves": (c_l, [c_i, c_i]),
    "atmvfi_pack_weight_conv3x3": (c_i, [c_f, c_f, c_f, c_i, c_i, c_f]),
    "atmvfi_conv3x3_f16x3": (c_i, [c_f, c_i, c_i, c_i, c_i, c_i, c_f, c_f, c_i, c_f, c_i, c_f, c_f, c_f, c_f, c_l, c_f, c_i, c_i, c_f]),
    "atmvfi_conv3p": (c_i, [ctypes.POINTER(Conv3pParams), c_f]),
    "atmvfi_flow_warp_up2": (c_i, [c_f, c_f, c_f, c_f, c_i, c_i, c_i, c_i, c_f]),
    "atmvfi_flow_warp_up2_tiled": (c_i, [c_f, c_f, c_f, c_f, c_i, c_i, c_i, c_i, c_f]),
    "atmvfi_image_pyramid": (c_i, [c_f, c_f, c_f, c_f, c_f, c_i, c_i, c_i, c_f]),
    "atmvfi_image_pyramid_pack": (c_i, [c_f, c_f, c_f, c_f, c_f, c_f, c_i, c_i, c_i, c_f]),
    "atmvfi_head1x1_planes": (c_i, [c_f, c_f, c_l, c_l, c_i, c_f, c_f, c_i, c_f, c_i, c_f]),
    "atmvfi_conv3x3_planes_workspace_floats": (c_l, [c_i, c_i, c_i, c_i, c_i]),
    "atmvfi_refine_tail": (c_i, [c_f, c_l, c_f, c_f, c_f, c_f, c_f, c_i, c_i, c_i, c_f]),
    "atmvfi_layernorm": (c_i, [c_f, c_i, c_l, c_i, c_f, c_f, c_i, c_f, c_f, c_l, c_i, c_f, c_f, c_i, c_f]),
    "atmvfi_dwconv3x3_gelu": (c_i, [c_f, c_i, c_f, c_i, c_f, c_f, c_i, c_i, c_i, c_i, c_f, c_f, c_i, c_f]),
    "atmvfi_pack_dw_weight": (c_i, [c_f, c_f, c_i, c_f]),
    "atmvfi_window_attention": (c_i, [c_f, c_f, c_f, c_f, c_i, c_i, c_i, c_i, c_i, c_i, c_f, c_f, c_i, c_f]),
    "atmvfi_window_attention_f16x3": (c_i, [c_f, c_f, c_f, c_f, c_i, c_i, c_i, c_i, c_i, c_i, c_f, c_f, c_i, c_f]),
    "atmvfi_window_attn_cross_motion": (c_i, [c_f, c_f, c_f, c_f, c_i, c_i, c_i, c_i, c_i, c_f]),
    "atmvfi_window_attn_self": (c_i, [c_f, c_f, c_f, c_i, c_i, c_i, c_i, c_i, c_f]),
    "atmvfi_motion_head": (c_i, [c_f, c_f, c_f, c_f, c_f, c_f, c_f, c_i, c_l, c_i, c_l, c_i, c_f]),
    "atmvfi_motion_head_planes": (c_i, [c_f, c_f, c_f, c_f, c_f, c_f, c_f, c_i, c_l, c_i, c_l, c_i, c_f, c_f, c_l, c_i, c_i, c_f]),
    "atmvfi_flow_warp": (c_i, [c_f, c_f, c_l, c_i, c_i, c_f, c_i, c_i, c_i, c_i, c_f]),
    "atmvfi_flow_warp_tiled": (c_i, [c_f, c_f, c_l, c_i, c_i, c_f, c_i, c_i, c_i, c_i, c_f]),
    "atmvfi_flow_warp_ex": (c_i, [c_f, c_f, c_f, c_f, c_i, c_i, c_i, c_i, c_i, c_f]),
    "atmvfi_flow_warp_nhwc": (c_i, [c_f, c_i, c_l, c_f, c_l, c_i, c_i, c_f, c_i, c_l, c_i, c_i, c_i, c_i, c_f]),
    "atmvfi_warp_blend": (c_i, [c_f, c_f, c_f, c_i, c_l, c_f, c_f, c_f, c_f, c_f, c_f, c_f, c_f, c_f, c_f, c_i,
                                c_i, c_i, c_i, c_f]),
    "atmvfi_warp_blend_planes": (c_i, [c_f, c_f, c_f, c_i, c_l, c_f, c_f, c_f, c_f, c_f, c_f, c_f, c_f, c_f, c_f, c_i,
                                       c_f, c_f, c_l, c_i, c_i, c_i, c_i, c_f]),
    "atmvfi_warp_blend_tiled": (c_i, [c_f, c_f, c_f, c_i, c_l, c_f, c_f, c_f, c_f, c_f, c_f, c_f, c_f, c_f, c_f, c_i,
                                      c_f, c_f, c_l, c_i, c_i, c_i, c_i, c_f]),
    "atmvfi_resize_bilinear_ac": (c_i, [c_f, c_l, c_l, c_l, c_l, c_f, c_i, c_i, c_i, c_i, c_i, c_i, ctypes.c_float, c_f]),
    "atmvfi_frame_u8_to_f32": (c_i, [c_f, c_i, c_i, c_i, c_f, c_i, c_i, c_i, c_i, c_f]),
    "atmvfi_frame_u8_window": (c_i, [c_f, c_i, c_i, c_i, c_i, c_i, c_i, c_i, c_i, c_f, c_i, c_i, c_i, c_i, c_f, c_f]),
    "atmvfi_frame_f32_to_u8": (c_i, [c_f, c_i, c_i, c_i, c_i, c_f, c_i, c_i, c_i, c_f]),
    "atmvfi_pool_blocks": (c_i, [c_f, c_l, c_i, C_SLOTS, c_i, c_l, c_f, c_i, c_f]),
    "atmvfi_tta_merge": (c_i, [c_f, c_f, c_f, c_f, c_i, c_i, c_i, c_i, c_i, c_i, c_i, c_f]),
    "atmvfi_frame_rot180": (c_i, [c_f, c_f, c_i, c_i, c_i, c_f]),
    "atmvfi_frame_signature_workspace_ints": (c_l, [c_i, c_i]),
    "atmvfi_frame_signature": (c_i, [c_f, c_i, c_i, c_i, c_i, c_i, c_i, c_i, c_f, c_f, c_l, c_f]),
    "atmvfi_frame_difference_workspace_ints": (c_l, [c_i, c_i]),
    "atmvfi_frame_difference": (c_i, [c_f, c_f, c_i, c_i, c_i, c_i, c_i, c_i, c_i, c_f, c_f, c_l, c_f]),
    "atmvfi_frame_borders_workspace_ints": (c_l, [c_i, c_i]),
    "atmvfi_frame_borders": (c_i, [c_f, c_i, c_i, c_i, c_f, c_f, c_l, c_f]),
    "atmvfi_frame_compose": (c_i, [c_f, c_f, c_i, c_i, c_i, c_i, c_i, c_i, c_f, c_i, c_i, c_i, c_i, c_f, c_i, c_f]),
    "atmvfi_yuv_borders_workspace_ints": (c_l, [c_i, c_i]),
    "atmvfi_yuv_borders": (c_i, [c_f, c_i, c_i, c_i, c_i, c_l, c_f, c_f, c_l, c_f]),
    "atmvfi_yuv_compose": (c_i, [c_f, c_f] + [c_i] * 9 + [c_l] * 3 + [c_i] * 4 + [c_f] + [c_i] * 4 + [c_f, c_f]),
    "atmvfi_shutter_accumulate": (c_i, [c_f, c_i, c_i, c_f, c_i, c_i, c_i, c_i, c_f, c_i, c_i, c_i, c_i, c_f]),
    "atmvfi_shutter_resolve": (c_i, [c_f, c_i, c_i, c_i, c_i, c_f, c_i, c_f]),
    "atmvfi_shutter_table": (c_i, [c_i, ctypes.POINTER(ctypes.c_uint16)]),
    "atmvfi_yuv420_to_rgb": (c_i, [c_f, c_i, c_i, c_i, c_i, c_i, c_i, c_f, c_i, c_f, c_i, c_i, c_i, c_i, c_f]),
    "atmvfi_yuv420_window": (c_i, [c_f, c_i, c_i, c_i, c_i, c_i, c_i, c_i, c_i, c_i, c_i, c_i, c_f, c_i, c_i, c_i, c_i, c_f, c_f]),
    "atmvfi_rgb_to_yuv420": (c_i, [c_f, c_i, c_f, c_i, c_i, c_i, c_i, c_i, c_i, c_i, c_i, c_i, c_f, c_f]),
    "atmvfi_yuv420p10_to_f32": (c_i, [c_f, c_i, c_i, c_i, c_i, c_i, c_i, c_i, c_i, c_f, c_i, c_i, c_i, c_i, c_f]),
    "atmvfi_f32_to_yuv420p10": (c_i, [c_f, c_i, c_i, c_i, c_i, c_i, c_i, c_i, c_i, c_f, c_f]),
    "atmvfi_yuv_surface_decode": (c_i, [c_f, c_i, c_i, c_i, c_i, c_i, c_i, c_i, c_i, c_l, c_l, c_l, c_i, c_i, c_i, c_i, c_i, c_f, c_i, c_f, c_i, c_i,
                                        c_i, c_i, c_f]),
    "atmvfi_yuv_surface_encode": (c_i, [c_f, c_i, c_f, c_i, c_i, c_i, c_i, c_i, c_i, c_i, c_i, c_i, c_i, c_i, c_i, c_f, c_f]),
    "atmvfi_yuv_sub_decode": (c_i, [c_f, c_i, c_i, c_i, c_i, c_i, c_i, c_i, c_i, c_i, c_l, c_l, c_l, c_i, c_i, c_i, c_i, c_i, c_f, c_i, c_f, c_i, c_i,
                                    c_i, c_i, c_f]),
    "atmvfi_yuv_sub_encode": (c_i, [c_f, c_i, c_f, c_i, c_i, c_i, c_i, c_i, c_i, c_i, c_i, c_i, c_i, c_i, c_i, c_i, c_f, c_f]),
    "atmvfi_yuv_unpack": (c_i, [c_f, c_i, c_i, c_i, c_l, c_f, c_f]),
    "atmvfi_yuv_pack": (c_i, [c_f, c_i, c_i, c_i, c_f, c_f]),
    "atmvfi_rgb16_decode": (c_i, [c_f, c_i, c_i, c_i, c_i, c_i, c_i, c_i, c_i, c_f, c_i, c_i, c_i, c_i, c_f, c_f]),
    "atmvfi_rgb16_encode": (c_i, [c_f, c_i, c_i, c_i, c_i, c_f, c_i, c_i, c_i, c_i, c_f]),
    "atmvfi_frame_half": (c_i, [c_f, c_f, c_i, c_i, c_i, c_f]),
    "atmvfi_field_bob": (c_i, [c_f, c_f, c_f, c_i, c_i, c_i, c_i, c_i, c_i, c_i, c_f]),
    "atmvfi_field_rows": (c_i, [c_f, c_f, c_i, ctypes.POINTER(ctypes.c_int64), c_i, c_f]),
    "atmvfi_synth_up2": (c_i, [c_f, c_f]),
    "atmvfi_synth_up2_workspace_floats": (c_l, [c_i, c_i, c_i]),
    "atmvfi_pack_frames": (c_i, [c_f, c_f, c_f, c_i, c_i, c_i, c_f]),
    "atmvfi_final_residual": (c_i, [c_f, c_f, c_i, c_f, c_f, c_i, c_i, c_i, c_f]),
    "atmvfi_l1_mean": (c_i, [c_f, c_f, c_f, c_i, c_l, c_f, c_l, c_f]),
    "atmvfi_l1_mean_workspace_floats": (c_l, [c_i, c_l]),
    "atmvfi_ssim_psnr": (c_i, [c_f, c_l, c_l, c_l, c_l, c_f, c_l, c_l, c_l, c_l, c_i, c_i, c_i, ctypes.c_float, c_i, c_f, c_f, c_l, c_f]),
    "atmvfi_ssim_psnr_workspace_floats": (c_l, [c_i, c_i, c_i]),
    "atmvfi_ensemble_select": (c_i, [c_f, c_f, c_f, c_f, c_f, c_f, c_f, c_f, c_f, c_f, c_f, c_i, c_l, c_f]),
    "atmvfi_stem_fused": (c_i, [c_f, c_i, c_i, c_i, c_i, c_i, c_f, c_f, c_f, c_f, c_f, c_f, c_f, c_f, c_f, c_f, c_f, c_f, c_f, c_f, c_l, c_f]),
    "atmvfi_plan_fn_id": (c_i, [ctypes.c_char_p]),
    "atmvfi_plan_run": (c_i, [ctypes.POINTER(PlanOp), c_i, ctypes.POINTER(PlanPatch), c_i, ctypes.POINTER(ctypes.c_uint64), c_i,
                              ctypes.POINTER(c_i), c_f]),
}
FIELD_BOB_STRIP = 16
SSIM_X_U8, SSIM_X_BGR, SSIM_ROUND_Y, SSIM_ACCUMULATE, SSIM_MSE_F32 = 1, 2, 4, 8, 16


class SynthUp2Params(ctypes.Structure):
    _fields_ = ([(n, ctypes.c_void_p) for n in ("it_sum", "it0", "it1", "flow0", "flow1", "m1", "store0", "store1", "slots0", "slots1", "dst_f32",
                                                 "dst_u8", "f0_out", "f1_out", "m_out", "workspace")]
                + [(n, ctypes.c_int32) for n in ("B", "h", "w", "S0", "S1", "pad_top", "pad_left", "hh", "ww", "bgr", "path", "reserved")])


def load_library(path: str = LIB_PATH, optional=()) -> ctypes.CDLL:
    if not os.path.exists(path):
        raise HipLibraryMissing(
            f"{path} not found: build it with `python -c 'import __graft_entry__ as g; g.build()'` "
            "(hipcc --offload-arch=gfx950).  There is no CPU fallback.")
    lib = ctypes.CDLL(path)
    for name, (res, args) in SIGNATURES.items():
# ... 767 lines not shown
                       bias=_ptr(bias), prelu=_ptr(prelu), in_prelu=_ptr(in_prelu), residual=None, res_ld=0)
        p.precision, p.weight_hi, p.weight_lo = self._prec(w)
        p.tile_wn = self.gemm_tile_wn
        self._gemm_sink(p, sink, n * oh * ow, cout, sink_c0, 0, 1, "deconv")
        use_planes = planes is not None and p.precision == 1
        if x is None and not use_planes:
            raise ValueError("deconv: plane input needs the f16x3 engine")
        if use_planes:
            if planes.rows < n * h * wd or planes.c != cin:
                raise ValueError("deconv: planes do not match the input rows")
            p.in_, p.in_ld, p.in_prelu = None, planes.ld_rows, None
            p.in_hi, p.in_lo = planes.t[0].data_ptr(), planes.t[1].data_ptr()
        meta = {"flops": 2.0 * n * h * wd * 4 * cout * cin, "bytes": 4.0 * (n * h * wd * cin + n * oh * ow * cout + 4 * cout * cin),
                "shape": f"M{n * h * wd} N{4 * cout} K{cin}"}
        ws = self._gemm_splitk(p, n * h * wd, 4 * ((cout + 3) // 4 * 4), (cin + 31) // 32) if use_planes else None
        p._srcs = (x, out, bias, prelu, in_prelu, ws)
        self._plane_prec(p)
        self._run("deconv2x2_split" if use_planes else "deconv2x2_f16x3" if p.precision else "deconv2x2", meta, self.lib.atmvfi_deconv2x2,
                  ctypes.byref(p), self._stream())

    split_planes_ok = True
    pyramid_packs = True
    motion_head_sink = True

    def split_planes(self, x, out: Planes, prelu=None, c0: Optional[int] = None):
        ld, m, c, gs, _ = rows_view(x, "split_planes.in")
        if gs != 0 or m != out.rows or (c0 is None and c != out.c) or (c0 is not None and (c0 % 8 or c0 + c > out.chunks * 32)):
            raise ValueError("split_planes: expected a plain [rows,C] view matching the planes")
        if prelu is not None and prelu.numel() < c:
            raise ValueError("split_planes: prelu needs one slope per channel")
        meta = {"bytes": 4.0 * m * c + 4.0 * m * ((c + 31) // 32 * 32 if c0 is None else (c + 7) // 8 * 8)}
        if c0 is None:
            self._run("split_planes", meta, self.lib.atmvfi_split_planes, _ptr(x), ld, m, c, _ptr(prelu), _ptr(out.t[0]),
                      _ptr(out.t[1]), out.ld_rows, self._stream())
        else:
            self._run("split_planes", meta, self.lib.atmvfi_split_planes_at, _ptr(x), ld, m, c, _ptr(prelu), _ptr(out.t[0]),
                      _ptr(out.t[1]), out.ld_rows, c0, 8, self._stream())

    def linear(self, x, w: PackedWeight, out, bias=None, residual=None, out_row_map=None, sink: Optional[Planes] = None,
               sink_c0: int = 0, sink_gc: int = 0):
        planes = x if isinstance(x, Planes) else None
        if planes is not None:
            if self.precision != "f16x3" or w.hi is None:
                raise ValueError("linear: split-plane input needs the f16x3 engine and split weights")
            ld, m, cin, gs, rpg = planes.ld_rows, planes.rows, planes.c, 0, 0
        else:
            ld, m, cin, gs, rpg = rows_view(x, "linear.in")
        old, mo, cout, ogs, orpg = rows_view(out, "linear.out")
        if cin != w.cin or cout != w.cout or w.kh != 1 or w.mode == GEMM_DECONV:
            raise ValueError(f"linear: shape mismatch in {tuple(x.shape)} w ({w.cout},{w.cin}) out {tuple(out.shape)}")
        if out_row_map is None and mo != m:
            raise ValueError("linear: row count mismatch")
        if out_row_map is not None and (out_row_map.numel() != m or out_row_map.dtype != torch.int32 or not out_row_map.is_cuda):
            raise ValueError("linear: out_row_map must be a CUDA int32 tensor with one entry per GEMM row")
        res_ld = 0
        if residual is not None:
            res_ld, rm, rc, rgs, _ = rows_view(residual, "linear.residual")
            if rm != m or rc != cout or rgs != 0:
                raise ValueError("linear: residual must be a plain [M,Cout] view")
        p = GemmParams(mode=GEMM_LINEAR, in_=None if planes is not None else x.data_ptr(), in_ld=ld, N=1, H=1, W=1, Cin=cin, in_gstride=gs, in_rpg=rpg,
                       weight=w.packed.data_ptr(), Cout=cout, kh=1, kw=1, stride=1, pad=0, dil=1, Ho=1, Wo=1, M=m,
                       out=out.data_ptr(), out_ld=old, out_gstride=ogs, out_rpg=orpg, out_row_map=_ptr(out_row_map),
                       bias=_ptr(bias), prelu=None, in_prelu=None, residual=_ptr(residual), res_ld=res_ld)
        p.precision, p.weight_hi, p.weight_lo = self._prec(w)
        p.tile_wn = self.gemm_tile_wn
        if planes is not None:
            p.in_hi, p.in_lo = planes.t[0].data_ptr(), planes.t[1].data_ptr()
        if sink is not None:
            self._gemm_sink(p, sink, orpg if orpg else mo, cout, sink_c0, sink_gc, (mo // orpg) if orpg else 1, "linear")
        meta = {"flops": 2.0 * m * cout * cin, "bytes": 4.0 * (m * cin + m * cout + cout * cin), "shape": f"M{m} N{cout} K{cin}"}
        ws = self._gemm_splitk(p, m, cout, (cin + 31) // 32) if planes is not None else None
        p._srcs = (None if planes is not None else x, out, bias, residual, out_row_map, ws)
        self._plane_prec(p)
        self._run("linear_split" if planes is not None else "linear_f16x3" if p.precision else "linear", meta, self.lib.atmvfi_linear, ctypes.byref(p), self._stream())

    @staticmethod
    def _sink(planes: Optional[Planes], rows: int, c: int, what: str):
        if planes is None:
            return None, None, 0
        if planes.rows != rows or planes.c != c:
            raise ValueError(f"{what}: planes hold {planes.rows} x {planes.c}, kernel writes {rows} x {c}")
        return _ptr(planes.t[0]), _ptr(planes.t[1]), planes.ld_rows

    def layernorm(self, x, out, gamma, beta, src_row_map=None, planes: Optional[Planes] = None):
        ld, m, c, gs, rpg = rows_view(x, "layernorm.in")
        if out is None:
            if planes is None:
                raise ValueError("layernorm: no output")
            old, mo, co, ogs = 0, planes.rows, planes.c, 0
        else:
            old, mo, co, ogs, _ = rows_view(out, "layernorm.out")
        if co != c or ogs != 0:
            raise ValueError("layernorm: output must be a plain [rows,C] view")
        if src_row_map is None and mo != m:
            raise ValueError("layernorm: row count mismatch")
        if src_row_map is not None and src_row_map.numel() != mo:
            raise ValueError("layernorm: src_row_map needs one entry per output row")
        hi, lo, pld = self._sink(planes, mo, c, "layernorm")
        meta = {"bytes": 4.0 * mo * c * (1 + (out is not None) + (planes is not None))}
        self._run("layernorm", meta, self.lib.atmvfi_layernorm, _ptr(x), ld, gs, rpg, _ptr(src_row_map), _ptr(out), old,
                  _ptr(gamma), _ptr(beta), mo, c, hi, lo, pld, self._stream())

    def dwconv_gelu(self, x, out, w9, bias, planes: Optional[Planes] = None):
        ld, n, h, w, c = nhwc_view(x, "dwconv.in")
        old = 0
        if out is not None:
            old, on, oh, ow, oc = nhwc_view(out, "dwconv.out")
            if (on, oh, ow, oc) != (n, h, w, c):
                raise ValueError("dwconv: shape mismatch")
        elif planes is None:
            raise ValueError("dwconv: no output")
        hi, lo, pld = self._sink(planes, n * h * w, c, "dwconv")
        meta = {"bytes": 4.0 * n * h * w * c * (1 + (out is not None) + (planes is not None))}
        self._run("dwconv3x3_gelu", meta, self.lib.atmvfi_dwconv3x3_gelu, _ptr(x), ld, _ptr(out), old, _ptr(w9), _ptr(bias),
                  n, h, w, c, hi, lo, pld, self._stream())

    def window_attention(self, qkv, out, motion, labels, bw, nw, ws, heads, hd, kv_shift, planes: Optional[Planes] = None):
        _chk(qkv, "attn.qkv")
        n = ws * ws
        c = heads * hd
        if out is None and planes is None:
            raise ValueError("window_attention: no output")
        if out is not None:
            _chk(out, "attn.out")
        if tuple(qkv.shape) != (bw * n, 3 * c) or not qkv.is_contiguous() or (
                out is not None and (tuple(out.shape) != (bw * n, c) or not out.is_contiguous())):
            raise ValueError(f"window_attention: qkv {tuple(qkv.shape)} / out do not match Bw {bw} N {n} C {c}")
        if motion is not None and (tuple(motion.shape) != (bw * n, heads, 2) or not motion.is_contiguous()):
            raise ValueError("window_attention: motion must be contiguous [Bw*N, heads, 2]")
        if labels is not None and (tuple(labels.shape) != (nw, n) or labels.dtype != torch.int32 or not labels.is_cuda):
            raise ValueError("window_attention: labels must be CUDA int32 [nW, N]")
        meta = {"flops": 4.0 * bw * heads * n * n * hd, "bytes": 4.0 * bw * n * 4 * c}
        hi, lo, pld = self._sink(planes, bw * n, c, "window_attention")
        fn = self.lib.atmvfi_window_attention_f16x3 if self.precision == "f16x3" and self.attention_f16x3 else self.lib.atmvfi_window_attention
        self._run("window_attention", meta, fn, _ptr(qkv), _ptr(out), _ptr(motion), _ptr(labels),
                  bw, nw, ws, heads, hd, kv_shift, hi, lo, pld, self._stream())

    def motion_head(self, motion, row_map, w0, b0, w1, b1, out, planes: Optional[Planes] = None, planes_c0: int = 0, planes_gc: int = 0):
        old, mo, co, ogs, orpg = rows_view(out, "motion_head.out")
        rows = motion.shape[0]
        if co != 2:
            raise ValueError("motion_head: output view must have 2 channels")
        if planes is not None:
            groups = (mo // orpg) if orpg else 1
            if planes.rows != (orpg if orpg else mo) or planes_c0 % 2 or planes_gc % 2 or planes_c0 + (groups - 1) * planes_gc + 2 > planes.chunks * 32:
                raise ValueError("motion_head: the plane sink must hold one row per row of a group and even channel offsets inside its chunks")
        self._run("motion_head", {"bytes": 4.0 * rows * 18}, self.lib.atmvfi_motion_head_planes, _ptr(motion), _ptr(row_map), _ptr(w0),
                  _ptr(b0), _ptr(w1), _ptr(b1), _ptr(out), old, ogs, orpg, rows, motion.shape[1],
                  _ptr(planes.t[0]) if planes is not None else None, _ptr(planes.t[1]) if planes is not None else None,
                  planes.ld_rows if planes is not None else 0, planes_c0, planes_gc, self._stream())

    def _tiled_warp_ok(self, w, *planes) -> bool:
        return self.warp_tiles and w % 4 == 0 and all(t.data_ptr() % 16 == 0 for t in planes)

    def flow_warp(self, src, flow, dst):
        _chk(src, "flow_warp.src"); _chk(dst, "flow_warp.dst")
        b, c, h, w = src.shape
        if not src.is_contiguous() or not dst.is_contiguous() or tuple(dst.shape) != (b, c, h, w):
            raise ValueError("flow_warp: src/dst must be contiguous NCHW of equal shape")
        bs, ps, cs = flow_view(flow, h, w, "flow_warp.flow")
        meta = {"bytes": 4.0 * b * h * w * (2 * c + 2)}
        fn = self.lib.atmvfi_flow_warp_tiled if self._tiled_warp_ok(w, src) else self.lib.atmvfi_flow_warp
        self._run("flow_warp", meta, fn, _ptr(src), _ptr(flow), bs, ps, cs, _ptr(dst), b, c, h, w, self._stream())

    PADDING_MODES = {"zeros": 0, "border": 1, "reflection": 2}

    def flow_warp_ex(self, src, flow, dst, mask=None, padding_mode="zeros"):
        _chk(src, "flow_warp_ex.src"); _chk(dst, "flow_warp_ex.dst"); _chk(flow, "flow_warp_ex.flow")
        b, c, h, w = src.shape
        if padding_mode not in self.PADDING_MODES:
            raise ValueError(f"flow_warp: padding_mode must be one of {sorted(self.PADDING_MODES)}, got {padding_mode!r}")
        if (not all(t.is_contiguous() for t in (src, flow, dst)) or tuple(dst.shape) != (b, c, h, w) or tuple(flow.shape) != (b, 2, h, w)):
            raise ValueError("flow_warp_ex: contiguous src/dst [B,C,H,W] and flow [B,2,H,W] expected")
        if mask is not None and (mask.device != src.device or not mask.is_contiguous() or tuple(mask.shape) != (b, h, w) or mask.element_size() != 1):
            raise ValueError("flow_warp_ex: mask must be a contiguous [B,H,W] bool / uint8 tensor on the source's device")
        meta = {"bytes": 4.0 * b * h * w * (2 * c + 2)}
        self._run("flow_warp_ex", meta, self.lib.atmvfi_flow_warp_ex, _ptr(src), _ptr(flow), _ptr(dst), 0 if mask is None else mask.data_ptr(),
                  b, c, h, w, self.PADDING_MODES[padding_mode], self._stream())

    def flow_warp_up2(self, src, flow, dst, flow_up):
        b, c, h, w = src.shape
        if (not all(t.is_contiguous() for t in (src, flow, dst, flow_up)) or tuple(dst.shape) != (b, c, h, w) or tuple(flow.shape) != (b, 2, h, w)
                or tuple(flow_up.shape) != (b, 2, 2 * h, 2 * w)):
            raise ValueError("flow_warp_up2: contiguous src/dst [B,C,H,W], flow [B,2,H,W], flow_up [B,2,2H,2W] expected")
        meta = {"bytes": 4.0 * b * h * w * (2 * c + 2 + 8)}
        fn = self.lib.atmvfi_flow_warp_up2_tiled if self._tiled_warp_ok(w, src) else self.lib.atmvfi_flow_warp_up2
        self._run("flow_warp_up2", meta, fn, _ptr(src), _ptr(flow), _ptr(dst), _ptr(flow_up), b, c, h, w, self._stream())

    def flow_warp_nhwc(self, src, flow, dst):
        ld, b, h, w, c = nhwc_view(src, "flow_warp_nhwc.src")
        old, ob, oh, ow, oc = nhwc_view(dst, "flow_warp_nhwc.dst")
        if (ob, oh, ow, oc) != (b, h, w, c):
            raise ValueError("flow_warp_nhwc: shape mismatch")
        bs, ps, cs = flow_view(flow, h, w, "flow_warp_nhwc.flow")
        meta = {"bytes": 4.0 * b * h * w * (2 * c + 2)}
        self._run("flow_warp_nhwc", meta, self.lib.atmvfi_flow_warp_nhwc, _ptr(src), ld, src.stride(0), _ptr(flow), bs, ps, cs,
                  _ptr(dst), old, dst.stride(0), b, c, h, w, self._stream())

    def warp_blend(self, im0, im1, motion, i0w, i1w, it, flow0=None, flow1=None, mask1=None, mask2=None,
                   orig0=None, orig1=None, pack15=None, pack_planes: Optional[Planes] = None, pack_c0: int = 0):
        _planar(im0, 3, "warp_blend.im0"); _planar(im1, 3, "warp_blend.im1")
        b, _, h, w = im0.shape
        mld, mb, mh, mw, mc = nhwc_view(motion, "warp_blend.motion")
        if (mb, mh, mw, mc) != (b, h, w, 5):
            raise ValueError(f"warp_blend: motion view {tuple(motion.shape)} != [{b},{h},{w},5]")
        for t in (i0w, i1w, it):
            _planar(t, 3, "warp_blend.out")
        pld = 0
        if pack15 is not None:
            pld, pb, ph, pw, pc = nhwc_view(pack15, "warp_blend.pack15")
            if (pb, ph, pw, pc) != (b, h, w, 15):
                raise ValueError("warp_blend: pack15 view must be [B,H,W,15]")
            _planar(orig0, 3, "warp_blend.orig0"); _planar(orig1, 3, "warp_blend.orig1")
        per_px = 6 + 5 + 9 + (6 if flow0 is not None else 0) + ((6 + 15) if pack15 is not None else 0) + ((6 + 16) if pack_planes is not None else 0)
        meta = {"bytes": 4.0 * b * h * w * per_px}
        if pack_planes is not None:
            if pack_planes.rows != b * h * w or pack_c0 % 4 or pack_c0 + 16 > pack_planes.chunks * 32:
                raise ValueError("warp_blend: the plane sink must hold B*H*W rows and 16 channels at the offset")
            _planar(orig0, 3, "warp_blend.orig0"); _planar(orig1, 3, "warp_blend.orig1")
# ... 715 lines not shown
```

atm-vfi_amd/network.py:

```python
from __future__ import annotations

import math
import operator
from typing import Dict, List, Optional, Tuple

import torch
import torch.nn as nn

from . import scaled
from . import schema as S
from .hip_ops import GEMM_CONV, GEMM_DECONV, GEMM_LINEAR, HipOps, PackedWeight, Planes, PlanUnsupported
from .windows import WindowGeometry, build_window_geometry


_VERSION_OF = operator.attrgetter("_version")
_DATA_PTR_OF = torch.Tensor.data_ptr


_PARAM_EPOCH = [0]


class _ParamWatch:

    def __setattr__(self, name, value):
        d = self.__dict__
        if isinstance(value, (nn.Parameter, nn.Module)) or name in d.get("_parameters", ()) or name in d.get("_modules", ()):
            _PARAM_EPOCH[0] += 1
        super().__setattr__(name, value)

    def __delattr__(self, name):
        d = self.__dict__
        if name in d.get("_parameters", ()) or name in d.get("_modules", ()):
            _PARAM_EPOCH[0] += 1
        super().__delattr__(name)

    def register_parameter(self, name, param):
        _PARAM_EPOCH[0] += 1
        super().register_parameter(name, param)

    def add_module(self, name, module):
        _PARAM_EPOCH[0] += 1
        super().add_module(name, module)

    def register_module(self, name, module):
        _PARAM_EPOCH[0] += 1
        super().register_module(name, module)


class _Node(_ParamWatch, nn.Module):
    """Anonymous container used to reproduce the reference's dotted parameter names."""


def _r4(c: int) -> int:
    return (c + 3) // 4 * 4


class _PMap:
    __slots__ = ("p", "n", "h", "w", "chunk0", "c")

    def __init__(self, p, n, h, w, chunk0, c):
        self.p, self.n, self.h, self.w, self.chunk0, self.c = p, n, h, w, chunk0, c


class BlockRunner:

    def _init_runner(self):
        self._ops_obj = None
        self._bufs: Dict[Tuple, object] = {}
        self._geo: Dict[Tuple, Tuple[WindowGeometry, torch.Tensor, Optional[torch.Tensor]]] = {}

    def buf(self, name: str, *shape) -> torch.Tensor:
        key = (name,) + tuple(shape)
        t = self._bufs.get(key)
        if t is None:
            if getattr(self._ops_obj, "recording", None) is not None:
                raise PlanUnsupported(f"workspace buffer {name} created while recording")
            t = self._ops_obj.empty(*shape)
            self._bufs[key] = t
        return t

    def planes(self, name: str, rows: int, c: int) -> Planes:
        key = ("planes", name, rows, c)
        p = self._bufs.get(key)
        if p is None:
            if getattr(self._ops_obj, "recording", None) is not None:
                raise PlanUnsupported(f"workspace planes {name} created while recording")
            p = Planes.alloc(rows, c, self._ops_obj.device)
            self._bufs[key] = p
        return p

    def geometry(self, frames, h, w, ws, shift):
        key = (frames, h, w, ws, shift)
        g = self._geo.get(key)
        if g is None:
            if getattr(self._ops_obj, "recording", None) is not None:
                raise PlanUnsupported("window maps created while recording")
            geo = build_window_geometry(frames, h, w, ws, shift)
            ops = self._ops_obj
            g = (geo, ops.to_device_int(geo.row_map), None if geo.labels is None else ops.to_device_int(geo.labels))
            self._geo[key] = g
        return g

    @staticmethod
    def _plane_deconvs(ops) -> bool:
        return getattr(ops, "precision", None) == "f16x3" and getattr(ops, "split_planes_ok", False)

    def _block(self, ops, P, p, x, frames, h, w, ws, shift, cross, out, motion_dst, tag, out_sink=None, motion_sink=None):
        c = x.shape[-1]
        heads = S.NUM_HEADS
        hd = c // heads
        geo, row_map, labels = self.geometry(frames, h, w, ws, shift)
        mw = frames * geo.n_windows * geo.tokens
        bw = frames * geo.n_windows
        pl = self._plane_deconvs(ops)
        xn = self.buf(f"{tag}xn", mw, c)
        xn_p = self.planes(f"{tag}xn_p", mw, c) if pl else None
        ops.layernorm(x, xn, P[f"{p}.norm1.weight"], P[f"{p}.norm1.bias"], src_row_map=row_map, **({"planes": xn_p} if pl else {}))
        qkv = self.buf(f"{tag}qkv", mw, 3 * c)
        ops.linear(xn_p if pl else xn, P[f"pk:{p}.attn.qkv.weight"], qkv)
        ao = None if pl else self.buf(f"{tag}ao", mw, c)
        ao_p = self.planes(f"{tag}ao_p", mw, c) if pl else None
        mo = self.buf(f"{tag}mo", mw, heads, 2) if cross else None
        ops.window_attention(qkv, ao, mo, labels, bw, geo.n_windows, ws, heads, hd, bw // 2 if cross else 0,
                             **({"planes": ao_p} if pl else {}))
        xb = self.buf(f"{tag}xb", frames * h * w, c)
        ops.linear(ao_p if pl else ao, P[f"pk:{p}.attn.proj.weight"], xb, bias=P[f"{p}.attn.proj.bias"], residual=xn, out_row_map=row_map)
        if cross:
            mk = {} if motion_sink is None else {"planes": motion_sink[0], "planes_c0": motion_sink[1], "planes_gc": motion_sink[2]}
            ops.motion_head(mo, row_map, P[f"{p}.attn.mlp.0.weight"], P[f"{p}.attn.mlp.0.bias"],
                            P[f"{p}.attn.mlp.2.weight"], P[f"{p}.attn.mlp.2.bias"], motion_dst, **mk)
        hid = P[f"{p}.mlp.fc1.bias"].shape[0]
        f1 = self.buf(f"{tag}fc1", frames, h, w, hid)
        if pl:
            y_p = self.planes(f"{tag}ln2_p", frames * h * w, c)
            ops.layernorm(xb, None, P[f"{p}.norm2.weight"], P[f"{p}.norm2.bias"], planes=y_p)
            ops.linear(y_p, P[f"pk:{p}.mlp.fc1.weight"], f1.reshape(frames * h * w, hid), bias=P[f"{p}.mlp.fc1.bias"])
            f2_p = self.planes(f"{tag}dw_p", frames * h * w, hid)
            ops.dwconv_gelu(f1, None, P[f"pk:{p}.mlp.dwconv.dwconv.weight"], P[f"{p}.mlp.dwconv.dwconv.bias"], planes=f2_p)
            sk = {} if out_sink is None else {"sink": out_sink[0], "sink_c0": out_sink[1], "sink_gc": out_sink[2]}
            ops.linear(f2_p, P[f"pk:{p}.mlp.fc2.weight"], out, bias=P[f"{p}.mlp.fc2.bias"], residual=xb, **sk)
        else:
            y = self.buf(f"{tag}ln2", frames * h * w, c)
            ops.layernorm(xb, y, P[f"{p}.norm2.weight"], P[f"{p}.norm2.bias"])
            ops.linear(y, P[f"pk:{p}.mlp.fc1.weight"], f1.reshape(frames * h * w, hid), bias=P[f"{p}.mlp.fc1.bias"])
            f2 = self.buf(f"{tag}dw", frames, h, w, hid)
            ops.dwconv_gelu(f1, f2, P[f"pk:{p}.mlp.dwconv.dwconv.weight"], P[f"{p}.mlp.dwconv.dwconv.bias"])
            ops.linear(f2.reshape(frames * h * w, hid), P[f"pk:{p}.mlp.fc2.weight"], out, bias=P[f"{p}.mlp.fc2.bias"], residual=xb)


class Network(_ParamWatch, BlockRunner, nn.Module):
    VARIANT = "base"

    SELECTIONS = ("use_plans",)

    def __init__(self, global_motion: bool = True, ensemble_global_motion: bool = False, variant: Optional[str] = None,
                 selections: Optional[Dict[str, bool]] = None):
        super().__init__()
        self.variant_name = variant or self.VARIANT
        v = S.VARIANTS[self.variant_name]
        self._v = v
        self.pyramid_level = S.PYRAMID_LEVELS
        self.hidden_dims = list(v.hidden_dims)
        self.global_motion = global_motion
        self.ensemble_global_motion = ensemble_global_motion
        self.local_motion_args = {"window_size": v.local_window, "num_heads": S.NUM_HEADS, "patch_size": 1,
                                  "dim": v.local_dim, "enhance_window": 8}
        self.global_motion_args = {"window_size": v.global_window, "num_heads": S.NUM_HEADS, "patch_size": 1,
                                   "dim": v.global_dim}
        if self.variant_name == "lite":
            self.local_motion_args["mlp_ratio"] = v.mlp_ratio
            self.global_motion_args["mlp_ratio"] = v.mlp_ratio
        self.fused_dim = v.fused_dim
        self.motion_out_dim = S.MOTION_OUT
        self.fused_dim1, self.fused_dim2, self.fused_dim3 = v.decoder_widths
        self.fused_dims = [self.fused_dim1, self.fused_dim2, self.fused_dim3, 2 * self.fused_dim1]
        gen = torch.Generator().manual_seed(torch.initial_seed() % (2 ** 31))
        for sp in S.param_schema(v):
            t = S.init_tensor(sp, gen)
            parts = sp.key.split(".")
            node: nn.Module = self
            for name in parts[:-1]:
                if name not in node._modules:
                    node.add_module(name, _Node())
                node = node._modules[name]
            if sp.is_buffer:
                node.register_buffer(parts[-1], t)
            else:
                node.register_parameter(parts[-1], nn.Parameter(t))
        self._init_runner()
        self._precision = "f16x3"
        self._checked = False
        self._prepared: Dict[str, object] = {}
        self._prepared_sig = None
        self.max_workspaces = 2
        self.workspace_cap_bytes = 96 << 30
        self._workspaces: Dict[Tuple, Dict[Tuple, object]] = {}
        self._ws_key: Optional[Tuple] = None
        self._bufs: Dict[Tuple, object] = {}
        self._geo: Dict[Tuple, Tuple[WindowGeometry, torch.Tensor, Optional[torch.Tensor]]] = {}
        self.use_graphs = False
        self._frame_cache_on = False
        self._rows_fit_planes = True
        self._frame_cache = None
        self._reuse_first = False
        self._graphs: Dict[Tuple, Tuple] = {}
        self._graph_sig = None
        self.use_plans = True
        self._plans: Dict[Tuple, object] = {}
        self._plan_sig = None
        self._pool_plans: Dict[Tuple, object] = {}
        self._pooled_plans_on = True
        self._splitk_memo: Dict[Tuple, Tuple] = {}
        self._scaled_halves: Dict[Tuple, Tuple] = {}
        self._plan_stats = self._new_plan_stats()
        self._plist = None
        self._pepoch = -1
        self._primary: Optional["Network"] = None
        self._prepare_lock = None
        for name, flag in (selections or {}).items():
            if name not in self.SELECTIONS:
                raise ValueError(f"unknown kernel selection {name!r}; one of {self.SELECTIONS}")
            setattr(self, name, bool(flag))

# ... 272 lines not shown
            return
        ops.conv(x, P[f"pk:{p}.weight"], out, stride=stride, pad=pad, dil=dil, bias=P[f"{p}.bias"])

    def _plane_convs(self, ops) -> bool:
        return self._plane_deconvs(ops) and self._rows_fit_planes

    def _c3p(self, ops, P, p, xp, n, h, w, out=None, act=True, sink=None, sink_c0=0, sink_prelu=None, wkey=None, out_cmin=0, sink2=None):
        if act:
            wk, bias, prelu = wkey or f"pk:{p}.0.weight", P[f"{p}.0.bias"], P[f"{p}.1.weight"]
        else:
            wk, bias, prelu = wkey or f"pk:{p}.weight", P[f"{p}.bias"], None
        extra = {} if sink2 is None else {"planes2": sink2}
        need = ops.conv3x3_workspace_floats(n, h, w, P[wk].cin, P[wk].cout)
        if need:
            extra["workspace"] = self.buf("splitk_ws", need)
        ops.conv3x3_planes(xp, n, h, w, P[wk], out=out, bias=bias, prelu=prelu, planes=sink, planes_c0=sink_c0, planes_prelu=sink_prelu,
                           out_cmin=out_cmin, **extra)

    def _conv_p(self, ops, P, p, src: "_PMap", stride=1, pad=1, dil=1, act=True, out=None, sink=None, sink_c0=0, src2: "Optional[_PMap]" = None):
        if act:
            wk, bias, prelu = f"pk:{p}.0.weight", P[f"{p}.0.bias"], P[f"{p}.1.weight"]
        else:
            wk, bias, prelu = f"pk:{p}.weight", P[f"{p}.bias"], None
        two = {} if src2 is None else {"x2": src2.p, "x2_chunk0": src2.chunk0, "split_chunks": src.c // 32}
        ops.conv_planes(src.p, src.n, src.h, src.w, P[wk], out=out, stride=stride, pad=pad, dil=dil, bias=bias, prelu=prelu, sink=sink,
                        sink_c0=sink_c0, in_chunk0=src.chunk0, **two)

    def _deconv_act(self, ops, P, p, x, out, in_prelu=None, split: Optional[str] = None, planes=None):
        w = P[f"pk:{p}.0.weight"]
        if planes is not None:
            ops.deconv(x, w, out, bias=P[f"{p}.0.bias"], prelu=P[f"{p}.1.weight"], planes=planes)
            return
        if split is not None and self._plane_deconvs(ops) and w.hi is not None:
            b, h, wd, cin = x.shape
            xp = self.planes(split, b * h * wd, cin)
            ops.split_planes(x.flatten(0, 2), xp, prelu=in_prelu)
            ops.deconv(x, w, out, bias=P[f"{p}.0.bias"], prelu=P[f"{p}.1.weight"], planes=xp)
            return
        ops.deconv(x, w, out, bias=P[f"{p}.0.bias"], prelu=P[f"{p}.1.weight"], in_prelu=in_prelu)

    def _encoder(self, ops, P, x0, tag: str):
        d = self._v.hidden_dims
        f, h, w, _ = x0.shape
        if self._plane_convs(ops):
            ld = self._v.local_dim
            fuse_p = self.planes(f"{tag}fuse_l_p", f * (h // 8) * (w // 8), ld)
            src, outs = None, []
            for st in (1, 2, 3):
                hs, ws = h >> st, w >> st
                ap = self.planes(f"{tag}e{st}a_p", f * hs * ws, d[st])
                if st == 1:
                    ops.stem_fused(x0, P["stem"], ap)
                else:
                    self._conv_p(ops, P, f"feat_extracts.{st}.0", src, stride=2, sink=ap)
                if st == 3:
                    self._c3p(ops, P, "feat_extracts.3.1", ap, f, hs, ws, sink=fuse_p, sink_c0=ld - d[3])
                    outs.append(_PMap(fuse_p, f, hs, ws, 0, ld))
                else:
                    ep = self.planes(f"{tag}e{st}_p", f * hs * ws, d[st])
                    self._c3p(ops, P, f"feat_extracts.{st}.1", ap, f, hs, ws, sink=ep)
                    outs.append(_PMap(ep, f, hs, ws, 0, d[st]))
                    src = outs[-1]
            return outs[0], outs[1], outs[2]
        a = self.buf(f"{tag}e0a", f, h, w, d[0]); self._conv_act(ops, P, "feat_extracts.0.0", x0[..., :3], a)
        e0 = self.buf(f"{tag}e0", f, h, w, d[0]); self._conv_act(ops, P, "feat_extracts.0.1", a, e0)
        a = self.buf(f"{tag}e1a", f, h // 2, w // 2, d[1]); self._conv_act(ops, P, "feat_extracts.1.0", e0, a, 2)
        e1 = self.buf(f"{tag}e1", f, h // 2, w // 2, d[1]); self._conv_act(ops, P, "feat_extracts.1.1", a, e1)
        a = self.buf(f"{tag}e2a", f, h // 4, w // 4, d[2]); self._conv_act(ops, P, "feat_extracts.2.0", e1, a, 2)
        e2 = self.buf(f"{tag}e2", f, h // 4, w // 4, d[2]); self._conv_act(ops, P, "feat_extracts.2.1", a, e2)
        a = self.buf(f"{tag}e3a", f, h // 8, w // 8, d[3]); self._conv_act(ops, P, "feat_extracts.3.0", e2, a, 2)
        fuse = self.buf(f"{tag}fuse_l", f, h // 8, w // 8, self._v.local_dim)
        self._conv_act(ops, P, "feat_extracts.3.1", a, fuse[..., self._v.local_dim - d[3]:])
        return e1, e2, fuse

    def _fusion(self, ops, P, p, fine, mid, fuse, c_mid, c_fine, tag):
        if isinstance(fuse, _PMap):
            f, h, w, c = fuse.n, fuse.h, fuse.w, fuse.c
            self._conv_p(ops, P, f"{p}.layers.0", mid, stride=2, pad=1, dil=1, act=False, sink=fuse.p, sink_c0=0)
            self._conv_p(ops, P, f"{p}.layers.1", fine, stride=4, pad=1, dil=1, act=False, sink=fuse.p, sink_c0=c_mid)
            self._conv_p(ops, P, f"{p}.layers.2", fine, stride=4, pad=2, dil=2, act=False, sink=fuse.p, sink_c0=c_mid + c_fine)
            t = self.buf(f"{tag}fproj", f * h * w, c)
            ops.linear(fuse.p, P[f"pk:{p}.proj.weight"], t, bias=P[f"{p}.proj.bias"])
            out = self.buf(f"{tag}fnorm", f * h * w, c)
            ops.layernorm(t, out, P[f"{p}.norm.weight"], P[f"{p}.norm.bias"])
            return out
        f, h, w, c = fuse.shape
        self._conv_plain(ops, P, f"{p}.layers.0", mid, fuse[..., 0:c_mid], stride=2, pad=1, dil=1)
        self._conv_plain(ops, P, f"{p}.layers.1", fine, fuse[..., c_mid:c_mid + c_fine], stride=4, pad=1, dil=1)
        self._conv_plain(ops, P, f"{p}.layers.2", fine, fuse[..., c_mid + c_fine:c_mid + 2 * c_fine], stride=4, pad=2, dil=2)
        t = self.buf(f"{tag}fproj", f * h * w, c)
        ops.linear(fuse.reshape(f * h * w, c), P[f"pk:{p}.proj.weight"], t, bias=P[f"{p}.proj.bias"])
        out = self.buf(f"{tag}fnorm", f * h * w, c)
        ops.layernorm(t, out, P[f"{p}.norm.weight"], P[f"{p}.norm.bias"])
        return out

    @staticmethod
    def _stacked(buf, off, c):
        b, h, w, ld = buf.shape
        flat = buf.reshape(b * h * w, ld)[:, off:off + 2 * c]
        return flat.unflatten(1, (2, c)).permute(1, 0, 2)

    def _motion_branch(self, ops, P, branch, mlp, x_tokens, b, h, w, ws, tag):
        c = x_tokens.shape[-1]
        cin = 8 + 2 * c
        mlp_in = self.buf(f"{tag}mlp_in", b, h, w, cin)
        flat = mlp_in.reshape(b * h * w, cin)
        pc = self._plane_convs(ops)
        mlp_in_p = self.planes(f"{tag}mlp_in_p", b * h * w, cin) if pc else None
        x = x_tokens
        for blk in range(2):
            mdst = flat[:, 4 * blk:4 * blk + 4].unflatten(1, (2, 2)).permute(1, 0, 2)
            out = self._stacked(mlp_in, 8, c) if blk == 1 else self.buf(f"{tag}blk0", 2 * b * h * w, c)
            msink = (mlp_in_p, 4 * blk, 2) if (pc and getattr(ops, "motion_head_sink", False)) else None
            self._block(ops, P, f"{branch}.{blk}", x, 2 * b, h, w, ws, 0 if blk == 0 else ws // 2, True, out, mdst, tag,
                        out_sink=(mlp_in_p, 8, c) if (pc and blk == 1) else None, motion_sink=msink)
            x = out
        hid = P[f"{mlp}.0.0.bias"].shape[0]
        if pc:
            if not getattr(ops, "motion_head_sink", False):
                ops.split_planes(flat[:, 0:8], mlp_in_p, c0=0)
            t1p = self.planes(f"{tag}mm1_p", b * h * w, hid)
            t2p = self.planes(f"{tag}mm2_p", b * h * w, hid)
            self._c3p(ops, P, f"{mlp}.0", mlp_in_p, b, h, w, sink=t1p)
            self._c3p(ops, P, f"{mlp}.1", t1p, b, h, w, sink=t2p)
            return mlp_in, t2p
        t1 = self.buf(f"{tag}mm1", b, h, w, hid); self._conv_act(ops, P, f"{mlp}.0", mlp_in, t1)
        t2 = self.buf(f"{tag}mm2", b, h, w, hid); self._conv_act(ops, P, f"{mlp}.1", t1, t2)
        return mlp_in, t2

    def _global_tokens(self, ops, P, e2, fuse_l, tag):
        v = self._v
        d = v.hidden_dims
        if isinstance(fuse_l, _PMap):
            f, h8, w8 = fuse_l.n, fuse_l.h, fuse_l.w
            h_, w_ = h8 // 2, w8 // 2
            s3 = _PMap(fuse_l.p, f, h8, w8, (v.local_dim - d[3]) // 32, d[3])
            fuse_g = _PMap(self.planes(f"{tag}fuse_g_p", f * h_ * w_, v.global_dim), f, h_, w_, 0, v.global_dim)
            ap = self.planes(f"{tag}ga_p", f * h_ * w_, v.last_feat_dim)
            self._conv_p(ops, P, "last_feat_extract.0", s3, stride=2, sink=ap)
            self._c3p(ops, P, "last_feat_extract.1", ap, f, h_, w_, sink=fuse_g.p, sink_c0=d[3] + 2 * d[2])
            return self._fusion(ops, P, "global_feature_fusion", e2, s3, fuse_g, d[3], d[2], tag + "g")
        f, h8, w8, _ = fuse_l.shape
        h_, w_ = h8 // 2, w8 // 2
        s3 = fuse_l[..., v.local_dim - d[3]:]
        fuse_g = self.buf(f"{tag}fuse_g", f, h_, w_, v.global_dim)
        a = self.buf(f"{tag}ga", f, h_, w_, v.last_feat_dim)
        self._conv_act(ops, P, "last_feat_extract.0", s3, a, 2)
        self._conv_act(ops, P, "last_feat_extract.1", a, fuse_g[..., d[3] + 2 * d[2]:])
        return self._fusion(ops, P, "global_feature_fusion", e2, s3, fuse_g, d[3], d[2], tag + "g")

    def _global_from_tokens(self, ops, P, tokens, b, h_, w_, tag):
        mlp_in, t2 = self._motion_branch(ops, P, "global_motion_atmformer", "global_motion_mlp", tokens, b, h_, w_,
                                         self.global_motion_args["window_size"], tag + "g")
        gout = self.buf(f"{tag}gout", b, h_, w_, 8)
        self._head1x1(ops, P, "global_motion_mlp.2", t2, b, h_, w_, gout[..., :5])
        return gout

    def _global_motion(self, ops, P, e2, fuse_l, b, tag):
        if isinstance(fuse_l, _PMap):
            h_, w_ = fuse_l.h // 2, fuse_l.w // 2
        else:
            h_, w_ = fuse_l.shape[1] // 2, fuse_l.shape[2] // 2
        tokens = self._global_tokens(ops, P, e2, fuse_l, tag)
        return self._global_from_tokens(ops, P, tokens, b, h_, w_, tag)

    def _head1x1(self, ops, P, p, t2, b, h, w, out):
        if isinstance(t2, Planes):
# ... 694 lines not shown
```

include/atmvfi.h:

```cpp
#ifndef ATMVFI_H
#define ATMVFI_H

#include <stdint.h>

#ifdef __cplusplus
extern "C" {
#endif

#define ATMVFI_OK        0
#define ATMVFI_EINVAL   -1
#define ATMVFI_EALIGN   -2
#define ATMVFI_ELAUNCH  -3

int         atmvfi_version(void);
const char* atmvfi_last_error(void);
const char* atmvfi_source_digest(void);
int atmvfi_range_word_set(uint32_t* word, void* stream);
int atmvfi_range_checked(void);

#define ATMVFI_GEMM_CONV   0
#define ATMVFI_GEMM_LINEAR 1
#define ATMVFI_GEMM_DECONV 2

typedef struct atmvfi_gemm_params {
// ... 14 lines not shown
    const float* in_prelu;
    const float* residual;
    int32_t res_ld;
    int32_t precision;
    const void* weight_hi;
    const void* weight_lo;
    const void* in_hi;
    const void* in_lo;
    void* out_hi;
    void* out_lo;
    int64_t out_plane_rows;
    int32_t out_plane_c0, out_plane_gc;
    int32_t tile_wn;
    const void* in_hi2;
    const void* in_lo2;
    int32_t in_ld2, in_split_chunks;
    float* workspace;
    int64_t workspace_floats;
} atmvfi_gemm_params;

#define ATMVFI_PREC_F32   0
#define ATMVFI_PREC_F16X3 1
#define ATMVFI_PREC_F16   2

int atmvfi_gemm(const atmvfi_gemm_params* p, void* stream);
int64_t atmvfi_gemm_workspace_floats(int64_t M, int ngemm, int ksteps);

int atmvfi_head1x1_planes(const void* in_hi, const void* in_lo, int64_t plane_rows, int64_t rows, int Cin, const float* weight,
                          const float* bias, int Cout, float* out, int out_ld, void* stream);

int atmvfi_split_planes(const float* in, int in_ld, int64_t M, int C, const float* prelu, void* hi, void* lo, int plane_rows, void* stream);
int atmvfi_split_planes_at(const float* in, int in_ld, int64_t M, int C, const float* prelu, void* hi, void* lo, int plane_rows, int c0,
                           int pad_to, void* stream);

int atmvfi_conv2d(const atmvfi_gemm_params* p, void* stream);
int atmvfi_linear(const atmvfi_gemm_params* p, void* stream);
int atmvfi_deconv2x2(const atmvfi_gemm_params* p, void* stream);

int64_t atmvfi_packed_weight_floats(int mode, int Cout, int Cin, int kh, int kw);
int atmvfi_pack_weight(int mode, const float* src, float* dst, int Cout, int Cin, int kh, int kw, void* stream);

int64_t atmvfi_split_weight_halves(int mode, int Cout, int Cin, int kh, int kw);
int atmvfi_pack_weight_split(int mode, const float* src, void* dst_hi, void* dst_lo, int Cout, int Cin, int kh, int kw,
                             void* stream);
int64_t atmvfi_conv3x3_weight_halves(int Cout, int Cin);
int atmvfi_pack_weight_conv3x3(const float* src, void* dst_hi, void* dst_lo, int Cout, int Cin, void* stream);
int atmvfi_conv3x3_f16x3(const float* in, int in_ld, int N, int H, int W, int Cin, const void* w_hi, const void* w_lo,
                         int Cout, float* out, int out_ld, const float* bias, const float* prelu, void* out_hi, void* out_lo,
                         int64_t plane_rows, const float* plane_prelu, int schedule, int wn, void* stream);
typedef struct atmvfi_conv3p_params {
    const void* in_hi;
    const void* in_lo;
    int64_t in_rows;
    int32_t N, H, W, Cin;
    const void* w_hi;
    const void* w_lo;
    int32_t Cout;
    const float* bias;
    const float* prelu;
    float* out;
    int32_t out_ld, out_cmin;
    void* out_hi;
    void* out_lo;
    int64_t plane_rows;
    int32_t out_c0;
    const float* plane_prelu;
    void* out_hi2;
    void* out_lo2;
    int64_t plane_rows2;
    int32_t out_c02;
    int32_t wn;
    float* workspace;
    int64_t workspace_floats;
    const void* readout_w;
    float* readout;
    int64_t readout_plane;
    int32_t terms;
} atmvfi_conv3p_params;
int atmvfi_conv3p(const atmvfi_conv3p_params* p, void* stream);
int64_t atmvfi_conv3x3_planes_workspace_floats(int N, int H, int W, int Cin, int Cout);
int atmvfi_layernorm(const float* in, int in_ld, int64_t in_gstride, int in_rpg,
                     const int32_t* src_row_map, float* out, int out_ld,
                     const float* gamma, const float* beta, int64_t rows, int C,
                     void* out_hi, void* out_lo, int plane_rows, void* stream);

int atmvfi_dwconv3x3_gelu(const float* in, int in_ld, float* out, int out_ld,
                          const float* weight9, const float* bias,
                          int N, int H, int W, int C, void* out_hi, void* out_lo, int plane_rows, void* stream);
int atmvfi_pack_dw_weight(const float* src , float* dst , int C, void* stream);

int atmvfi_window_attention(const float* qkv, float* out , float* motion,
                            const int32_t* labels, int Bw, int nW, int ws, int heads, int hd,
                            int kv_shift, void* out_hi, void* out_lo, int plane_rows, void* stream);
int atmvfi_window_attention_f16x3(const float* qkv, float* out , float* motion,
                                  const int32_t* labels, int Bw, int nW, int ws, int heads, int hd,
                                  int kv_shift, void* out_hi, void* out_lo, int plane_rows, void* stream);
int atmvfi_window_attn_cross_motion(const float* qkv, float* out, float* motion, const int32_t* labels,
                                    int Bw, int nW, int ws, int heads, int hd, void* stream);
int atmvfi_window_attn_self(const float* qkv, float* out, const int32_t* labels,
                            int Bw, int nW, int ws, int heads, int hd, void* stream);

int atmvfi_motion_head(const float* motion , const int32_t* row_map,
                       const float* w0 , const float* b0, const float* w1 ,
                       const float* b1, float* out, int out_ld, int64_t out_gstride, int out_rpg,
                       int64_t rows, int heads, void* stream);
int atmvfi_motion_head_planes(const float* motion, const int32_t* row_map, const float* w0, const float* b0, const float* w1,
                              const float* b1, float* out, int out_ld, int64_t out_gstride, int out_rpg, int64_t rows, int heads,
                              void* out_hi, void* out_lo, int64_t plane_rows, int plane_c0, int plane_gc, void* stream);

int atmvfi_flow_warp(const float* src , const float* flow, int64_t flow_bstride,
                     int flow_pstride, int flow_cstride, float* dst, int B, int C, int H, int W, void* stream);
int atmvfi_flow_warp_tiled(const float* src , const float* flow, int64_t flow_bstride,
                           int flow_pstride, int flow_cstride, float* dst, int B, int C, int H, int W, void* stream);
int atmvfi_flow_warp_ex(const float* src , const float* flow , float* dst, uint8_t* mask ,
                        int B, int C, int H, int W, int padding_mode, void* stream);
int atmvfi_flow_warp_nhwc(const float* src, int src_ld, int64_t src_bstride,
                          const float* flow, int64_t flow_bstride, int flow_pstride, int flow_cstride,
                          float* dst, int dst_ld, int64_t dst_bstride, int B, int C, int H, int W, void* stream);

int atmvfi_warp_blend(const float* im0, const float* im1 ,
                      const float* motion, int motion_ld, int64_t motion_bstride,
                      float* i0w, float* i1w, float* it ,
                      float* flow0_out, float* flow1_out , float* mask1_out, float* mask2_out ,
                      const float* orig0, const float* orig1, float* pack15, int pack_ld,
                      int B, int H, int W, void* stream);
int atmvfi_warp_blend_planes(const float* im0, const float* im1, const float* motion, int motion_ld, int64_t motion_bstride,
                             float* i0w, float* i1w, float* it, float* flow0_out, float* flow1_out, float* mask1_out, float* mask2_out,
                             const float* orig0, const float* orig1, float* pack15, int pack_ld, void* pack_hi, void* pack_lo,
                             int64_t pack_rows, int pack_c0, int B, int H, int W, void* stream);
int atmvfi_warp_blend_tiled(const float* im0, const float* im1, const float* motion, int motion_ld, int64_t motion_bstride,
                            float* i0w, float* i1w, float* it, float* flow0_out, float* flow1_out, float* mask1_out, float* mask2_out,
                            const float* orig0, const float* orig1, float* pack15, int pack_ld, void* pack_hi, void* pack_lo,
                            int64_t pack_rows, int pack_c0, int B, int H, int W, void* stream);
#define atmvfi_blend atmvfi_warp_blend

int atmvfi_frame_half(const float* src, float* dst, int planes, int H, int W, void* stream);
typedef struct atmvfi_synth_up2_params {
    const float *it_sum, *it0, *it1;
    const float *flow0, *flow1;
    const float* m1;
    const float *store0, *store1;
    const int32_t *slots0, *slots1;
    float* dst_f32;
    void* dst_u8;
    float *f0_out, *f1_out, *m_out;
    float* workspace;
    int32_t B, h, w, S0, S1;
    int32_t pad_top, pad_left, hh, ww, bgr;
    int32_t path;
    int32_t reserved;
} atmvfi_synth_up2_params;
int atmvfi_synth_up2(const atmvfi_synth_up2_params* p, void* stream);
int64_t atmvfi_synth_up2_workspace_floats(int B, int h, int w);

int atmvfi_resize_bilinear_ac(const float* src, int64_t src_bstride, int64_t src_cstride, int64_t src_ystride,
                              int64_t src_xstride, float* dst, int B, int C, int Hi, int Wi, int Ho, int Wo,
                              float value_scale, void* stream);

int atmvfi_image_pyramid(const float* im0, const float* im1, float* l1, float* l2, float* l3, int B, int H, int W, void* stream);
int atmvfi_image_pyramid_pack(const float* im0, const float* im1, float* l1, float* l2, float* l3, float* pack, int B, int H, int W,
                              void* stream);

int atmvfi_flow_warp_up2(const float* src, const float* flow, float* dst, float* flow_up, int B, int C, int H, int W, void* stream);
int atmvfi_flow_warp_up2_tiled(const float* src, const float* flow, float* dst, float* flow_up, int B, int C, int H, int W, void* stream);

int atmvfi_pack_frames(const float* im0, const float* im1, float* dst , int B, int H, int W, void* stream);

int atmvfi_final_residual(const float* it , const float* r, int r_ld,
                          float* it_sum, float* it_clamped, int B, int H, int W, void* stream);

int atmvfi_refine_tail(const float* contrib, int64_t contrib_plane, const float* bias , const float* slope ,
                       const float* it , float* it_sum, float* it_clamped, int B, int H, int W, void* stream);

int atmvfi_frame_u8_to_f32(const void* src, int H, int W, int bgr, float* dst, int Hp, int Wp, int pad_top, int pad_left, void* stream);
int atmvfi_frame_f32_to_u8(const float* src, int Hp, int Wp, int pad_top, int pad_left, void* dst, int H, int W, int bgr, void* stream);
int atmvfi_frame_u8_window(const void* src, int H, int W, int bgr, int mode, int y0, int x0, int h, int w, float* dst, int Hp, int Wp,
                           int pad_top, int pad_left, void* dst_u8, void* stream);

int atmvfi_pool_blocks(void* pool, int64_t slot_bytes, int n_slots, const int32_t* slots , int n ,
// ... 112 lines not shown
```

Before: 51.64.

## Reverse attention block traversal order to reuse data left in cache by producer

Adds a `walk` parameter to window attention, layernorm and dwconv kernels that can reverse the order in which blocks visit work items. A small Python tracker records the direction each buffer was last written and picks the opposite direction for the consumer, so attention starts on the rows the qkv producer wrote last and may still hit in L2/MALL. Only attention uses a non-zero walk today; layernorm and dwconv are passed 0. The cost is extra API arguments and host-side bookkeeping keyed by storage pointer.

New measurement: 51.70 (median of 6 runs). Within noise of the previous version (+0.1%).

```diff
diff --git a/atm-vfi_amd/csrc/api.hip b/atm-vfi_amd/csrc/api.hip
--- a/atm-vfi_amd/csrc/api.hip
+++ b/atm-vfi_amd/csrc/api.hip
@@ -55,7 +55,7 @@
 #endif
 }
 
-extern "C" int atmvfi_version(void) { return (0 << 16) | (28 << 8) | 0; }
+extern "C" int atmvfi_version(void) { return (0 << 16) | (29 << 8) | 0; }
 extern "C" const char* atmvfi_last_error(void) { return atmvfi::g_err; }
 #ifndef ATMVFI_SOURCE_DIGEST
 #define ATMVFI_SOURCE_DIGEST "unknown (api.hip compiled outside the Makefile)"
diff --git a/atm-vfi_amd/csrc/attention.hip b/atm-vfi_amd/csrc/attention.hip
--- a/atm-vfi_amd/csrc/attention.hip
+++ b/atm-vfi_amd/csrc/attention.hip
@@ -10,7 +10,7 @@
 __global__ __launch_bounds__(64 * NT) void window_attn_kernel(
     const float* __restrict__ qkv, const RowSink out, float* __restrict__ motion,
     const int* __restrict__ labels, int N, int nW, int ws, int heads, int hd, int C, int Bw, int kv_shift,
-    float scale) {
+    float scale, int walk) {
     fp16_saturate_on();
     extern __shared__ __attribute__((aligned(16))) float smem[];
     constexpr int NPAD = NT * 16;
@@ -22,7 +22,7 @@
     int* Ls = reinterpret_cast<int*>(Vt + DPAD * PV * 4);
 
     const int tid = threadIdx.x;
-    const int slot = blockIdx.x >> 3;
+    const int slot = walk ? (int)(gridDim.x >> 3) - 1 - (int)(blockIdx.x >> 3) : (int)(blockIdx.x >> 3);
     const int b = (slot / heads) * 8 + (blockIdx.x & 7);
     const int h = slot % heads;
     if (b >= Bw) return;
@@ -192,7 +192,7 @@
 __global__ __launch_bounds__(64 * NT, (NT <= 4 ? 3 : NT <= 8 ? 2 : NT <= 12 ? 3 : 4)) void window_attn_x3_kernel(
     const float* __restrict__ qkv, const RowSink out, float* __restrict__ motion,
     const int* __restrict__ labels, int N, int nW, int ws, int heads, int hd, int C, int Bw, int kv_shift,
-    float scale, int vitems) {
+    float scale, int vitems, int walk) {
     extern __shared__ __attribute__((aligned(16))) float smem[];
     fp16_saturate_on();
     constexpr int NPAD = NT * 16, KT2 = (NT + 1) / 2, VROWS = 32 * KT2, T = 64 * NT;
@@ -268,8 +268,9 @@
         voff[u] = row * VS + (d4 << 3);
     }
 
+    const int slot0 = walk ? (vitems >> 3) - 1 : 0, slot_step = walk ? -1 : 1;
     auto item_of = [&](int v, int& b, int& h) {
-        const int slot = v >> 3;
+        const int slot = slot0 + slot_step * (v >> 3);
         b = (slot / heads) * 8 + (v & 7);
         h = slot % heads;
     };
@@ -527,7 +528,7 @@
 
 template <int NT>
 int launch_attn(const float* qkv, const RowSink out, float* motion, const int* labels, int Bw, int nW, int N, int ws,
-                int heads, int hd, int kv_shift, hipStream_t s) {
+                int heads, int hd, int kv_shift, int walk, hipStream_t s) {
     const int dpad = (hd + 15) / 16 * 16, npad = NT * 16;
     const size_t lds = ((size_t)npad * ((dpad / 4 + 15) / 16 * 16) * 4 + (size_t)dpad * ((npad / 4 + 15) / 16 * 16) * 4 + npad) * sizeof(float);
     ATMVFI_REQUIRE(hd <= (NT >= 13 ? 64 : 128), ATMVFI_EINVAL, "window_attention: head dim %d too large for a %d-token window", hd, N);
@@ -540,13 +541,13 @@
     }
     const float scale = 1.0f / sqrtf((float)hd);
     hipLaunchKernelGGL(kern, dim3((unsigned)((Bw + 7) / 8 * 8 * heads)), dim3(64 * NT), lds, s, qkv, out, motion, labels, N, nW, ws,
-                       heads, hd, heads * hd, Bw, kv_shift, scale);
+                       heads, hd, heads * hd, Bw, kv_shift, scale, walk);
     return atmvfi::check_launch("window_attention");
 }
 
 template <int NT, int DCH>
 int launch_attn_x3(const float* qkv, const RowSink out, float* motion, const int* labels, int Bw, int nW, int N, int ws,
-                   int heads, int hd, int kv_shift, hipStream_t s) {
+                   int heads, int hd, int kv_shift, int walk, hipStream_t s) {
     const int d32 = (hd + 31) / 32, dt = (hd + (motion ? 4 : 0) + 15) / 16, npad = NT * 16, vrows = 32 * ((NT + 1) / 2);
     const int ks = (d32 <= 1 ? 4 : d32 == 2 ? 8 : 16) * 16, vs = 32 * dt + ((dt & 1) ? 0 : 32);
     const size_t lds = 2 * (size_t)npad * ks + 2 * (size_t)vrows * vs + (size_t)npad * sizeof(int);
@@ -573,28 +574,29 @@
     int grid = atmvfi::cu_count() * per_cu;
     if (grid > vitems || NT > 8) grid = vitems;
     hipLaunchKernelGGL((window_attn_x3_kernel<NT, DCH>), dim3((unsigned)grid), dim3(64 * NT), lds, s, qkv, out, motion, labels, N, nW, ws,
-                       heads, hd, heads * hd, Bw, kv_shift, scale, vitems);
+                       heads, hd, heads * hd, Bw, kv_shift, scale, vitems, walk);
     return atmvfi::check_launch("window_attention_f16x3");
 }
 
 template <int NT>
 int launch_attn_x3_d(const float* qkv, const RowSink out, float* motion, const int* labels, int Bw, int nW, int N, int ws,
-                     int heads, int hd, int kv_shift, hipStream_t s) {
+                     int heads, int hd, int kv_shift, int walk, hipStream_t s) {
     ATMVFI_REQUIRE(hd <= (NT >= 13 ? 64 : 128), ATMVFI_EINVAL, "window_attention: head dim %d too large for a %d-token window", hd, N);
     switch ((hd + 31) / 32) {
-        case 1: return launch_attn_x3<NT, 1>(qkv, out, motion, labels, Bw, nW, N, ws, heads, hd, kv_shift, s);
-        case 2: return launch_attn_x3<NT, 2>(qkv, out, motion, labels, Bw, nW, N, ws, heads, hd, kv_shift, s);
+        case 1: return launch_attn_x3<NT, 1>(qkv, out, motion, labels, Bw, nW, N, ws, heads, hd, kv_shift, walk, s);
+        case 2: return launch_attn_x3<NT, 2>(qkv, out, motion, labels, Bw, nW, N, ws, heads, hd, kv_shift, walk, s);
     }
     if constexpr (NT <= 12) {
-        if (hd <= 96) return launch_attn_x3<NT, 3>(qkv, out, motion, labels, Bw, nW, N, ws, heads, hd, kv_shift, s);
-        return launch_attn_x3<NT, 4>(qkv, out, motion, labels, Bw, nW, N, ws, heads, hd, kv_shift, s);
+        if (hd <= 96) return launch_attn_x3<NT, 3>(qkv, out, motion, labels, Bw, nW, N, ws, heads, hd, kv_shift, walk, s);
+        return launch_attn_x3<NT, 4>(qkv, out, motion, labels, Bw, nW, N, ws, heads, hd, kv_shift, walk, s);
     }
     return ATMVFI_EINVAL;
 }
 
 int attention_entry(bool x3, const float* qkv, float* out, float* motion, const int32_t* labels, int Bw, int nW, int ws, int heads,
-                    int hd, int kv_shift, void* out_hi, void* out_lo, int plane_ld, void* stream) {
+                    int hd, int kv_shift, void* out_hi, void* out_lo, int plane_ld, int walk, void* stream) {
     ATMVFI_REQUIRE(qkv, ATMVFI_EINVAL, "window_attention: null pointer");
+    ATMVFI_REQUIRE(walk == 0 || walk == 1, ATMVFI_EINVAL, "window_attention: walk %d must be 0 (ascending) or 1 (descending)", walk);
     ATMVFI_REQUIRE(sink_ok(out, heads * hd, heads * hd, out_hi, out_lo, plane_ld, (long long)Bw * ws * ws), ATMVFI_EALIGN,
                    "window_attention: output needs fp32 rows and/or both fp16 planes (plane rows >= Bw*ws*ws), 16-byte aligned");
     const RowSink sink{out, heads * hd, (_Float16*)out_hi, (_Float16*)out_lo, plane_ld};
@@ -609,8 +611,8 @@
     hipStream_t s = (hipStream_t)stream;
 #define ATMVFI_ATTN_CASE(k)                                                                                              \
     case k:                                                                                                              \
-        return x3 ? launch_attn_x3_d<k>(qkv, sink, motion, labels, Bw, nW, N, ws, heads, hd, kv_shift, s)                 \
-                  : launch_attn<k>(qkv, sink, motion, labels, Bw, nW, N, ws, heads, hd, kv_shift, s);
+        return x3 ? launch_attn_x3_d<k>(qkv, sink, motion, labels, Bw, nW, N, ws, heads, hd, kv_shift, walk, s)                 \
+                  : launch_attn<k>(qkv, sink, motion, labels, Bw, nW, N, ws, heads, hd, kv_shift, walk, s);
     switch (nt) {
         ATMVFI_ATTN_CASE(1) ATMVFI_ATTN_CASE(2) ATMVFI_ATTN_CASE(3) ATMVFI_ATTN_CASE(4) ATMVFI_ATTN_CASE(5)
         ATMVFI_ATTN_CASE(6) ATMVFI_ATTN_CASE(7) ATMVFI_ATTN_CASE(8) ATMVFI_ATTN_CASE(9) ATMVFI_ATTN_CASE(10)
@@ -632,26 +634,26 @@
 
 extern "C" int atmvfi_window_attention_f16x3(const float* qkv, float* out, float* motion, const int32_t* labels, int Bw,
                                               int nW, int ws, int heads, int hd, int kv_shift, void* out_hi, void* out_lo,
-                                              int plane_ld, void* stream) {
-    return attention_entry(true, qkv, out, motion, labels, Bw, nW, ws, heads, hd, kv_shift, out_hi, out_lo, plane_ld, stream);
+                                              int plane_ld, int walk, void* stream) {
+    return attention_entry(true, qkv, out, motion, labels, Bw, nW, ws, heads, hd, kv_shift, out_hi, out_lo, plane_ld, walk, stream);
 }
 
 extern "C" int atmvfi_window_attention(const float* qkv, float* out, float* motion, const int32_t* labels, int Bw,
                                         int nW, int ws, int heads, int hd, int kv_shift, void* out_hi, void* out_lo,
-                                        int plane_ld, void* stream) {
-    return attention_entry(false, qkv, out, motion, labels, Bw, nW, ws, heads, hd, kv_shift, out_hi, out_lo, plane_ld, stream);
+                                        int plane_ld, int walk, void* stream) {
+    return attention_entry(false, qkv, out, motion, labels, Bw, nW, ws, heads, hd, kv_shift, out_hi, out_lo, plane_ld, walk, stream);
 }
 
 extern "C" int atmvfi_window_attn_cross_motion(const float* qkv, float* out, float* motion, const int32_t* labels,
                                                 int Bw, int nW, int ws, int heads, int hd, void* stream) {
     ATMVFI_REQUIRE(motion, ATMVFI_EINVAL, "window_attn_cross_motion: motion output required");
     ATMVFI_REQUIRE(Bw % 2 == 0, ATMVFI_EINVAL, "window_attn_cross_motion: Bw must be even (two frames)");
-    return atmvfi_window_attention(qkv, out, motion, labels, Bw, nW, ws, heads, hd, Bw / 2, nullptr, nullptr, 0, stream);
+    return atmvfi_window_attention(qkv, out, motion, labels, Bw, nW, ws, heads, hd, Bw / 2, nullptr, nullptr, 0, 0, stream);
 }
 
 extern "C" int atmvfi_window_attn_self(const float* qkv, float* out, const int32_t* labels, int Bw, int nW, int ws,
                                         int heads, int hd, void* stream) {
-    return atmvfi_window_attention(qkv, out, nullptr, labels, Bw, nW, ws, heads, hd, 0, nullptr, nullptr, 0, stream);
+    return atmvfi_window_attention(qkv, out, nullptr, labels, Bw, nW, ws, heads, hd, 0, nullptr, nullptr, 0, 0, stream);
 }
 
 extern "C" int atmvfi_motion_head_planes(const float* motion, const int32_t* row_map, const float* w0, const float* b0,
diff --git a/atm-vfi_amd/csrc/plan_dispatch.inc b/atm-vfi_amd/csrc/plan_dispatch.inc
--- a/atm-vfi_amd/csrc/plan_dispatch.inc
+++ b/atm-vfi_amd/csrc/plan_dispatch.inc
@@ -73,7 +73,7 @@
     "atmvfi_yuv_surface_encode",
     "atmvfi_yuv_unpack",
 };
-static const int kPlanFnArgs[ATMVFI_PLAN_NFN] = {1, 1, 19, 1, 13, 13, 10, 10, 5, 8, 10, 9, 14, 10, 8, 8, 7, 15, 12, 9, 5, 5, 11, 9, 15, 1, 10, 8, 9, 7, 14, 1, 12, 17, 3, 6, 7, 5, 8, 8, 1, 10, 13, 15, 10, 13, 13, 7, 8, 10, 18, 21, 1, 11, 19, 23, 23, 13, 13, 9, 8, 14, 18, 14, 9, 24, 5, 25, 17, 24, 16, 6};
+static const int kPlanFnArgs[ATMVFI_PLAN_NFN] = {1, 1, 19, 1, 14, 13, 10, 10, 5, 8, 10, 9, 14, 10, 8, 8, 7, 15, 12, 9, 5, 5, 11, 9, 15, 1, 10, 8, 9, 7, 15, 1, 12, 17, 3, 6, 7, 5, 8, 8, 1, 10, 13, 15, 10, 13, 13, 7, 8, 10, 18, 21, 1, 11, 19, 23, 23, 14, 14, 9, 8, 14, 18, 14, 9, 24, 5, 25, 17, 24, 16, 6};
 static int plan_call(const atmvfi_plan_op* op, void* stream) {
     const atmvfi_plan_arg* a = op->a;
     switch (op->fn) {
@@ -81,7 +81,7 @@
     case 1: return atmvfi_conv3p((const atmvfi_conv3p_params*)(uintptr_t)a[0].u, stream);
     case 2: return atmvfi_conv3x3_f16x3((const float*)(uintptr_t)a[0].u, (int)a[1].i, (int)a[2].i, (int)a[3].i, (int)a[4].i, (int)a[5].i, (const void*)(uintptr_t)a[6].u, (const void*)(uintptr_t)a[7].u, (int)a[8].i, (float*)(uintptr_t)a[9].u, (int)a[10].i, (const float*)(uintptr_t)a[11].u, (const float*)(uintptr_t)a[12].u, (void*)(uintptr_t)a[13].u, (void*)(uintptr_t)a[14].u, (int64_t)a[15].i, (const float*)(uintptr_t)a[16].u, (int)a[17].i, (int)a[18].i, stream);
     case 3: return atmvfi_deconv2x2((const atmvfi_gemm_params*)(uintptr_t)a[0].u, stream);
-    case 4: return atmvfi_dwconv3x3_gelu((const float*)(uintptr_t)a[0].u, (int)a[1].i, (float*)(uintptr_t)a[2].u, (int)a[3].i, (const float*)(uintptr_t)a[4].u, (const float*)(uintptr_t)a[5].u, (int)a[6].i, (int)a[7].i, (int)a[8].i, (int)a[9].i, (void*)(uintptr_t)a[10].u, (void*)(uintptr_t)a[11].u, (int)a[12].i, stream);
+    case 4: return atmvfi_dwconv3x3_gelu((const float*)(uintptr_t)a[0].u, (int)a[1].i, (float*)(uintptr_t)a[2].u, (int)a[3].i, (const float*)(uintptr_t)a[4].u, (const float*)(uintptr_t)a[5].u, (int)a[6].i, (int)a[7].i, (int)a[8].i, (int)a[9].i, (void*)(uintptr_t)a[10].u, (void*)(uintptr_t)a[11].u, (int)a[12].i, (int)a[13].i, stream);
     case 5: return atmvfi_ensemble_select((const float*)(uintptr_t)a[0].u, (const float*)(uintptr_t)a[1].u, (const float*)(uintptr_t)a[2].u, (const float*)(uintptr_t)a[3].u, (const float*)(uintptr_t)a[4].u, (const float*)(uintptr_t)a[5].u, (const float*)(uintptr_t)a[6].u, (const float*)(uintptr_t)a[7].u, (const float*)(uintptr_t)a[8].u, (float*)(uintptr_t)a[9].u, (float*)(uintptr_t)a[10].u, (int)a[11].i, (int64_t)a[12].i, stream);
     case 6: return atmvfi_f32_to_yuv420p10((const float*)(uintptr_t)a[0].u, (int)a[1].i, (int)a[2].i, (int)a[3].i, (int)a[4].i, (int)a[5].i, (int)a[6].i, (int)a[7].i, (int)a[8].i, (void*)(uintptr_t)a[9].u, stream);
     case 7: return atmvfi_field_bob((const float*)(uintptr_t)a[0].u, (float*)(uintptr_t)a[1].u, (float*)(uintptr_t)a[2].u, (int)a[3].i, (int)a[4].i, (int)a[5].i, (int)a[6].i, (int)a[7].i, (int)a[8].i, (int)a[9].i, stream);
@@ -107,7 +107,7 @@
     case 27: return atmvfi_image_pyramid((const float*)(uintptr_t)a[0].u, (const float*)(uintptr_t)a[1].u, (float*)(uintptr_t)a[2].u, (float*)(uintptr_t)a[3].u, (float*)(uintptr_t)a[4].u, (int)a[5].i, (int)a[6].i, (int)a[7].i, stream);
     case 28: return atmvfi_image_pyramid_pack((const float*)(uintptr_t)a[0].u, (const float*)(uintptr_t)a[1].u, (float*)(uintptr_t)a[2].u, (float*)(uintptr_t)a[3].u, (float*)(uintptr_t)a[4].u, (float*)(uintptr_t)a[5].u, (int)a[6].i, (int)a[7].i, (int)a[8].i, stream);
     case 29: return atmvfi_l1_mean((const float*)(uintptr_t)a[0].u, (const float*)(uintptr_t)a[1].u, (float*)(uintptr_t)a[2].u, (int)a[3].i, (int64_t)a[4].i, (float*)(uintptr_t)a[5].u, (int64_t)a[6].i, stream);
-    case 30: return atmvfi_layernorm((const float*)(uintptr_t)a[0].u, (int)a[1].i, (int64_t)a[2].i, (int)a[3].i, (const int32_t*)(uintptr_t)a[4].u, (float*)(uintptr_t)a[5].u, (int)a[6].i, (const float*)(uintptr_t)a[7].u, (const float*)(uintptr_t)a[8].u, (int64_t)a[9].i, (int)a[10].i, (void*)(uintptr_t)a[11].u, (void*)(uintptr_t)a[12].u, (int)a[13].i, stream);
+    case 30: return atmvfi_layernorm((const float*)(uintptr_t)a[0].u, (int)a[1].i, (int64_t)a[2].i, (int)a[3].i, (const int32_t*)(uintptr_t)a[4].u, (float*)(uintptr_t)a[5].u, (int)a[6].i, (const float*)(uintptr_t)a[7].u, (const float*)(uintptr_t)a[8].u, (int64_t)a[9].i, (int)a[10].i, (void*)(uintptr_t)a[11].u, (void*)(uintptr_t)a[12].u, (int)a[13].i, (int)a[14].i, stream);
     case 31: return atmvfi_linear((const atmvfi_gemm_params*)(uintptr_t)a[0].u, stream);
     case 32: return atmvfi_motion_head((const float*)(uintptr_t)a[0].u, (const int32_t*)(uintptr_t)a[1].u, (const float*)(uintptr_t)a[2].u, (const float*)(uintptr_t)a[3].u, (const float*)(uintptr_t)a[4].u, (const float*)(uintptr_t)a[5].u, (float*)(uintptr_t)a[6].u, (int)a[7].i, (int64_t)a[8].i, (int)a[9].i, (int64_t)a[10].i, (int)a[11].i, stream);
     case 33: return atmvfi_motion_head_planes((const float*)(uintptr_t)a[0].u, (const int32_t*)(uintptr_t)a[1].u, (const float*)(uintptr_t)a[2].u, (const float*)(uintptr_t)a[3].u, (const float*)(uintptr_t)a[4].u, (const float*)(uintptr_t)a[5].u, (float*)(uintptr_t)a[6].u, (int)a[7].i, (int64_t)a[8].i, (int)a[9].i, (int64_t)a[10].i, (int)a[11].i, (void*)(uintptr_t)a[12].u, (void*)(uintptr_t)a[13].u, (int64_t)a[14].i, (int)a[15].i, (int)a[16].i, stream);
@@ -134,8 +134,8 @@
     case 54: return atmvfi_warp_blend((const float*)(uintptr_t)a[0].u, (const float*)(uintptr_t)a[1].u, (const float*)(uintptr_t)a[2].u, (int)a[3].i, (int64_t)a[4].i, (float*)(uintptr_t)a[5].u, (float*)(uintptr_t)a[6].u, (float*)(uintptr_t)a[7].u, (float*)(uintptr_t)a[8].u, (float*)(uintptr_t)a[9].u, (float*)(uintptr_t)a[10].u, (float*)(uintptr_t)a[11].u, (const float*)(uintptr_t)a[12].u, (const float*)(uintptr_t)a[13].u, (float*)(uintptr_t)a[14].u, (int)a[15].i, (int)a[16].i, (int)a[17].i, (int)a[18].i, stream);
     case 55: return atmvfi_warp_blend_planes((const float*)(uintptr_t)a[0].u, (const float*)(uintptr_t)a[1].u, (const float*)(uintptr_t)a[2].u, (int)a[3].i, (int64_t)a[4].i, (float*)(uintptr_t)a[5].u, (float*)(uintptr_t)a[6].u, (float*)(uintptr_t)a[7].u, (float*)(uintptr_t)a[8].u, (float*)(uintptr_t)a[9].u, (float*)(uintptr_t)a[10].u, (float*)(uintptr_t)a[11].u, (const float*)(uintptr_t)a[12].u, (const float*)(uintptr_t)a[13].u, (float*)(uintptr_t)a[14].u, (int)a[15].i, (void*)(uintptr_t)a[16].u, (void*)(uintptr_t)a[17].u, (int64_t)a[18].i, (int)a[19].i, (int)a[20].i, (int)a[21].i, (int)a[22].i, stream);
     case 56: return atmvfi_warp_blend_tiled((const float*)(uintptr_t)a[0].u, (const float*)(uintptr_t)a[1].u, (const float*)(uintptr_t)a[2].u, (int)a[3].i, (int64_t)a[4].i, (float*)(uintptr_t)a[5].u, (float*)(uintptr_t)a[6].u, (float*)(uintptr_t)a[7].u, (float*)(uintptr_t)a[8].u, (float*)(uintptr_t)a[9].u, (float*)(uintptr_t)a[10].u, (float*)(uintptr_t)a[11].u, (const float*)(uintptr_t)a[12].u, (const float*)(uintptr_t)a[13].u, (float*)(uintptr_t)a[14].u, (int)a[15].i, (void*)(uintptr_t)a[16].u, (void*)(uintptr_t)a[17].u, (int64_t)a[18].i, (int)a[19].i, (int)a[20].i, (int)a[21].i, (int)a[22].i, stream);
-    case 57: return atmvfi_window_attention((const float*)(uintptr_t)a[0].u, (float*)(uintptr_t)a[1].u, (float*)(uintptr_t)a[2].u, (const int32_t*)(uintptr_t)a[3].u, (int)a[4].i, (int)a[5].i, (int)a[6].i, (int)a[7].i, (int)a[8].i, (int)a[9].i, (void*)(uintptr_t)a[10].u, (void*)(uintptr_t)a[11].u, (int)a[12].i, stream);
-    case 58: return atmvfi_window_attention_f16x3((const float*)(uintptr_t)a[0].u, (float*)(uintptr_t)a[1].u, (float*)(uintptr_t)a[2].u, (const int32_t*)(uintptr_t)a[3].u, (int)a[4].i, (int)a[5].i, (int)a[6].i, (int)a[7].i, (int)a[8].i, (int)a[9].i, (void*)(uintptr_t)a[10].u, (void*)(uintptr_t)a[11].u, (int)a[12].i, stream);
+    case 57: return atmvfi_window_attention((const float*)(uintptr_t)a[0].u, (float*)(uintptr_t)a[1].u, (float*)(uintptr_t)a[2].u, (const int32_t*)(uintptr_t)a[3].u, (int)a[4].i, (int)a[5].i, (int)a[6].i, (int)a[7].i, (int)a[8].i, (int)a[9].i, (void*)(uintptr_t)a[10].u, (void*)(uintptr_t)a[11].u, (int)a[12].i, (int)a[13].i, stream);
+    case 58: return atmvfi_window_attention_f16x3((const float*)(uintptr_t)a[0].u, (float*)(uintptr_t)a[1].u, (float*)(uintptr_t)a[2].u, (const int32_t*)(uintptr_t)a[3].u, (int)a[4].i, (int)a[5].i, (int)a[6].i, (int)a[7].i, (int)a[8].i, (int)a[9].i, (void*)(uintptr_t)a[10].u, (void*)(uintptr_t)a[11].u, (int)a[12].i, (int)a[13].i, stream);
     case 59: return atmvfi_window_attn_cross_motion((const float*)(uintptr_t)a[0].u, (float*)(uintptr_t)a[1].u, (float*)(uintptr_t)a[2].u, (const int32_t*)(uintptr_t)a[3].u, (int)a[4].i, (int)a[5].i, (int)a[6].i, (int)a[7].i, (int)a[8].i, stream);
     case 60: return atmvfi_window_attn_self((const float*)(uintptr_t)a[0].u, (float*)(uintptr_t)a[1].u, (const int32_t*)(uintptr_t)a[2].u, (int)a[3].i, (int)a[4].i, (int)a[5].i, (int)a[6].i, (int)a[7].i, stream);
     case 61: return atmvfi_yuv420_to_rgb((const void*)(uintptr_t)a[0].u, (int)a[1].i, (int)a[2].i, (int)a[3].i, (int)a[4].i, (int)a[5].i, (int)a[6].i, (void*)(uintptr_t)a[7].u, (int)a[8].i, (float*)(uintptr_t)a[9].u, (int)a[10].i, (int)a[11].i, (int)a[12].i, (int)a[13].i, stream);
diff --git a/atm-vfi_amd/csrc/pointwise.hip b/atm-vfi_amd/csrc/pointwise.hip
--- a/atm-vfi_amd/csrc/pointwise.hip
+++ b/atm-vfi_amd/csrc/pointwise.hip
@@ -9,10 +9,11 @@
                                                         int in_rpg, const int* __restrict__ src_map,
                                                         const RowSink out,
                                                         const float* __restrict__ gamma, const float* __restrict__ beta,
-                                                        long long rows, int C) {
+                                                        long long rows, int C, int walk) {
     fp16_saturate_on();
     const int lane = threadIdx.x & 63;
-    const long long row = (long long)blockIdx.x * 4 + (threadIdx.x >> 6);
+    const unsigned blk = walk ? gridDim.x - 1u - blockIdx.x : blockIdx.x;
+    const long long row = (long long)blk * 4 + (threadIdx.x >> 6);
     if (row >= rows) return;
     const int c4n = C >> 2;
     long long src = src_map ? src_map[row] : row;
@@ -96,12 +97,14 @@
 __global__ __launch_bounds__(256) void dwconv_gelu_kernel(const float* __restrict__ in, int in_ld,
                                                           const RowSink out,
                                                           const float* __restrict__ w9, const float* __restrict__ bias,
-                                                          int N, int H, int W, int C) {
+                                                          int N, int H, int W, int C, int walk) {
     fp16_saturate_on();
     const int c4n = C >> 2;
     const long long total = (long long)N * H * W * c4n;
-    for (long long idx = (long long)blockIdx.x * blockDim.x + threadIdx.x; idx < total;
-         idx += (long long)gridDim.x * blockDim.x) {
+    const long long chunks = (total + blockDim.x - 1) / blockDim.x;
+    for (long long ch = blockIdx.x; ch < chunks; ch += gridDim.x) {
+        const long long idx = (walk ? chunks - 1 - ch : ch) * blockDim.x + threadIdx.x;
+        if (idx >= total) continue;
         const int c = (int)(idx % c4n) << 2;
         const long long pix = idx / c4n;
         const int x = (int)(pix % W);
@@ -136,9 +139,10 @@
 __global__ __launch_bounds__(256) void dwconv_gelu_rows_kernel(const float* __restrict__ in, int in_ld,
                                                                const RowSink out,
                                                                const float* __restrict__ w9, const float* __restrict__ bias,
-                                                               int N, int H, int W, int C, int xblocks, int cblocks, int strips) {
-    fp16_saturate_on();
-    int bid = blockIdx.x;
+                                                               int N, int H, int W, int C, int xblocks, int cblocks, int strips,
+                                                               int walk) {
+    fp16_saturate_on();
+    int bid = walk ? gridDim.x - 1 - blockIdx.x : blockIdx.x;
     const int cb = bid % cblocks; bid /= cblocks;
     const int xb = bid % xblocks; bid /= xblocks;
     const int sb = bid % strips;
@@ -242,13 +246,13 @@
 __global__ __launch_bounds__(256) void dwconv_gelu_dma_kernel(const float* __restrict__ in, int in_ld, _Float16* __restrict__ out_hi,
                                                               _Float16* __restrict__ out_lo, long long plane_rows,
                                                               const float* __restrict__ w9, const float* __restrict__ bias, int N, int H,
-                                                              int W, int C, int xgroups, int cblocks, int strips) {
+                                                              int W, int C, int xgroups, int cblocks, int strips, int walk) {
     static_assert(RS + 2 >= DW_RING, "the prologue fills the whole ring");
     fp16_saturate_on();
     extern __shared__ __attribute__((aligned(16))) unsigned char dw_smem[];
     const int lane = threadIdx.x & 63;
     const int wave = __builtin_amdgcn_readfirstlane(threadIdx.x >> 6);
-    unsigned u = blockIdx.x * 4u + (unsigned)wave;
+    unsigned u = (walk ? gridDim.x - 1u - blockIdx.x : blockIdx.x) * 4u + (unsigned)wave;
     const int xg = (int)(u % (unsigned)xgroups); u /= (unsigned)xgroups;
     const int cbk = (int)(u % (unsigned)cblocks); u /= (unsigned)cblocks;
     const int sb = (int)(u % (unsigned)strips);
@@ -520,8 +524,9 @@
 
 extern "C" int atmvfi_layernorm(const float* in, int in_ld, int64_t in_gstride, int in_rpg, const int32_t* src_row_map,
                                  float* out, int out_ld, const float* gamma, const float* beta, int64_t rows, int C,
-                                 void* out_hi, void* out_lo, int plane_ld, void* stream) {
+                                 void* out_hi, void* out_lo, int plane_ld, int walk, void* stream) {
     ATMVFI_REQUIRE(in && gamma && beta, ATMVFI_EINVAL, "layernorm: null pointer");
+    ATMVFI_REQUIRE(walk == 0 || walk == 1, ATMVFI_EINVAL, "layernorm: walk %d must be 0 (ascending) or 1 (descending)", walk);
     ATMVFI_REQUIRE(rows > 0 && C > 0 && C % 4 == 0, ATMVFI_EINVAL, "layernorm: C %d must be a positive multiple of 4", C);
     ATMVFI_REQUIRE(in_ld % 4 == 0 && in_ld >= C && in_gstride % 4 == 0, ATMVFI_EALIGN,
                    "layernorm: leading dimensions must be multiples of 4 and >= C");
@@ -532,14 +537,15 @@
     const unsigned blocks = (unsigned)((rows + 3) / 4);
     const RowSink sink{out, out_ld, (_Float16*)out_hi, (_Float16*)out_lo, plane_ld};
     hipLaunchKernelGGL(layernorm_kernel, dim3(blocks), dim3(256), 0, (hipStream_t)stream, in, in_ld, (long long)in_gstride,
-                       in_rpg, src_row_map, sink, gamma, beta, (long long)rows, C);
+                       in_rpg, src_row_map, sink, gamma, beta, (long long)rows, C, walk);
     return atmvfi::check_launch("layernorm");
 }
 
 extern "C" int atmvfi_dwconv3x3_gelu(const float* in, int in_ld, float* out, int out_ld, const float* weight9,
                                       const float* bias, int N, int H, int W, int C, void* out_hi, void* out_lo,
-                                      int plane_ld, void* stream) {
+                                      int plane_ld, int walk, void* stream) {
     ATMVFI_REQUIRE(in && weight9 && bias, ATMVFI_EINVAL, "dwconv3x3_gelu: null pointer");
+    ATMVFI_REQUIRE(walk == 0 || walk == 1, ATMVFI_EINVAL, "dwconv3x3_gelu: walk %d must be 0 (ascending) or 1 (descending)", walk);
     ATMVFI_REQUIRE(N > 0 && H > 0 && W > 0 && C > 0 && C % 4 == 0, ATMVFI_EINVAL, "dwconv3x3_gelu: bad shape");
     ATMVFI_REQUIRE(in_ld % 4 == 0 && in_ld >= C, ATMVFI_EALIGN, "dwconv3x3_gelu: bad ld");
     ATMVFI_REQUIRE(sink_ok(out, out_ld, C, out_hi, out_lo, plane_ld, (long long)N * H * W), ATMVFI_EALIGN,
@@ -563,7 +569,7 @@
         const size_t lds = 4 * DW_RING * DW_SLOT;
         auto go = [&](auto kern) {
             hipLaunchKernelGGL(kern, dim3((unsigned)blocks), dim3(256), lds, (hipStream_t)stream, in, in_ld, (_Float16*)out_hi,
-                               (_Float16*)out_lo, (long long)plane_ld, weight9, bias, N, H, W, C, xgroups, cblocks, strips);
+                               (_Float16*)out_lo, (long long)plane_ld, weight9, bias, N, H, W, C, xgroups, cblocks, strips, walk);
         };
         if (RS == 17) go(dwconv_gelu_dma_kernel<17>);
         else if (RS == 16) go(dwconv_gelu_dma_kernel<16>);
@@ -579,15 +585,15 @@
         ATMVFI_REQUIRE(blocks < (1ll << 31), ATMVFI_EINVAL, "dwconv3x3_gelu: grid too large");
         if (tall)
             hipLaunchKernelGGL(dwconv_gelu_rows_kernel<16>, dim3((unsigned)blocks), dim3(256), 0, (hipStream_t)stream, in, in_ld, sink,
-                               weight9, bias, N, H, W, C, xblocks, cblocks, strips);
+                               weight9, bias, N, H, W, C, xblocks, cblocks, strips, walk);
         else
             hipLaunchKernelGGL(dwconv_gelu_rows_kernel<8>, dim3((unsigned)blocks), dim3(256), 0, (hipStream_t)stream, in, in_ld, sink,
-                               weight9, bias, N, H, W, C, xblocks, cblocks, strips);
+                               weight9, bias, N, H, W, C, xblocks, cblocks, strips, walk);
         return atmvfi::check_launch("dwconv3x3_gelu");
     }
     const long long total = (long long)N * H * W * (C / 4);
     hipLaunchKernelGGL(dwconv_gelu_kernel, dim3(grid_for(total)), dim3(256), 0, (hipStream_t)stream, in, in_ld, sink,
-                       weight9, bias, N, H, W, C);
+                       weight9, bias, N, H, W, C, walk);
     return atmvfi::check_launch("dwconv3x3_gelu");
 }
 
diff --git a/atm-vfi_amd/hip_ops.py b/atm-vfi_amd/hip_ops.py
--- a/atm-vfi_amd/hip_ops.py
+++ b/atm-vfi_amd/hip_ops.py
@@ -109,11 +109,11 @@
     "atmvfi_head1x1_planes": (c_i, [c_f, c_f, c_l, c_l, c_i, c_f, c_f, c_i, c_f, c_i, c_f]),
     "atmvfi_conv3x3_planes_workspace_floats": (c_l, [c_i, c_i, c_i, c_i, c_i]),
     "atmvfi_refine_tail": (c_i, [c_f, c_l, c_f, c_f, c_f, c_f, c_f, c_i, c_i, c_i, c_f]),
-    "atmvfi_layernorm": (c_i, [c_f, c_i, c_l, c_i, c_f, c_f, c_i, c_f, c_f, c_l, c_i, c_f, c_f, c_i, c_f]),
-    "atmvfi_dwconv3x3_gelu": (c_i, [c_f, c_i, c_f, c_i, c_f, c_f, c_i, c_i, c_i, c_i, c_f, c_f, c_i, c_f]),
+    "atmvfi_layernorm": (c_i, [c_f, c_i, c_l, c_i, c_f, c_f, c_i, c_f, c_f, c_l, c_i, c_f, c_f, c_i, c_i, c_f]),
+    "atmvfi_dwconv3x3_gelu": (c_i, [c_f, c_i, c_f, c_i, c_f, c_f, c_i, c_i, c_i, c_i, c_f, c_f, c_i, c_i, c_f]),
     "atmvfi_pack_dw_weight": (c_i, [c_f, c_f, c_i, c_f]),
-    "atmvfi_window_attention": (c_i, [c_f, c_f, c_f, c_f, c_i, c_i, c_i, c_i, c_i, c_i, c_f, c_f, c_i, c_f]),
-    "atmvfi_window_attention_f16x3": (c_i, [c_f, c_f, c_f, c_f, c_i, c_i, c_i, c_i, c_i, c_i, c_f, c_f, c_i, c_f]),
+    "atmvfi_window_attention": (c_i, [c_f, c_f, c_f, c_f, c_i, c_i, c_i, c_i, c_i, c_i, c_f, c_f, c_i, c_i, c_f]),
+    "atmvfi_window_attention_f16x3": (c_i, [c_f, c_f, c_f, c_f, c_i, c_i, c_i, c_i, c_i, c_i, c_f, c_f, c_i, c_i, c_f]),
     "atmvfi_window_attn_cross_motion": (c_i, [c_f, c_f, c_f, c_f, c_i, c_i, c_i, c_i, c_i, c_f]),
     "atmvfi_window_attn_self": (c_i, [c_f, c_f, c_f, c_i, c_i, c_i, c_i, c_i, c_f]),
     "atmvfi_motion_head": (c_i, [c_f, c_f, c_f, c_f, c_f, c_f, c_f, c_i, c_l, c_i, c_l, c_i, c_f]),
@@ -1047,7 +1047,7 @@
             raise ValueError(f"{what}: planes hold {planes.rows} x {planes.c}, kernel writes {rows} x {c}")
         return _ptr(planes.t[0]), _ptr(planes.t[1]), planes.ld_rows
 
-    def layernorm(self, x, out, gamma, beta, src_row_map=None, planes: Optional[Planes] = None):
+    def layernorm(self, x, out, gamma, beta, src_row_map=None, planes: Optional[Planes] = None, walk: int = 0):
         ld, m, c, gs, rpg = rows_view(x, "layernorm.in")
         if out is None:
             if planes is None:
@@ -1064,9 +1064,9 @@
         hi, lo, pld = self._sink(planes, mo, c, "layernorm")
         meta = {"bytes": 4.0 * mo * c * (1 + (out is not None) + (planes is not None))}
         self._run("layernorm", meta, self.lib.atmvfi_layernorm, _ptr(x), ld, gs, rpg, _ptr(src_row_map), _ptr(out), old,
-                  _ptr(gamma), _ptr(beta), mo, c, hi, lo, pld, self._stream())
-
-    def dwconv_gelu(self, x, out, w9, bias, planes: Optional[Planes] = None):
+                  _ptr(gamma), _ptr(beta), mo, c, hi, lo, pld, int(walk), self._stream())
+
+    def dwconv_gelu(self, x, out, w9, bias, planes: Optional[Planes] = None, walk: int = 0):
         ld, n, h, w, c = nhwc_view(x, "dwconv.in")
         old = 0
         if out is not None:
@@ -1078,9 +1078,9 @@
         hi, lo, pld = self._sink(planes, n * h * w, c, "dwconv")
         meta = {"bytes": 4.0 * n * h * w * c * (1 + (out is not None) + (planes is not None))}
         self._run("dwconv3x3_gelu", meta, self.lib.atmvfi_dwconv3x3_gelu, _ptr(x), ld, _ptr(out), old, _ptr(w9), _ptr(bias),
-                  n, h, w, c, hi, lo, pld, self._stream())
-
-    def window_attention(self, qkv, out, motion, labels, bw, nw, ws, heads, hd, kv_shift, planes: Optional[Planes] = None):
+                  n, h, w, c, hi, lo, pld, int(walk), self._stream())
+
+    def window_attention(self, qkv, out, motion, labels, bw, nw, ws, heads, hd, kv_shift, planes: Optional[Planes] = None, walk: int = 0):
         _chk(qkv, "attn.qkv")
         n = ws * ws
         c = heads * hd
@@ -1099,7 +1099,7 @@
         hi, lo, pld = self._sink(planes, bw * n, c, "window_attention")
         fn = self.lib.atmvfi_window_attention_f16x3 if self.precision == "f16x3" and self.attention_f16x3 else self.lib.atmvfi_window_attention
         self._run("window_attention", meta, fn, _ptr(qkv), _ptr(out), _ptr(motion), _ptr(labels),
-                  bw, nw, ws, heads, hd, kv_shift, hi, lo, pld, self._stream())
+                  bw, nw, ws, heads, hd, kv_shift, hi, lo, pld, int(walk), self._stream())
 
     def motion_head(self, motion, row_map, w0, b0, w1, b1, out, planes: Optional[Planes] = None, planes_c0: int = 0, planes_gc: int = 0):
         old, mo, co, ogs, orpg = rows_view(out, "motion_head.out")
diff --git a/atm-vfi_amd/network.py b/atm-vfi_amd/network.py
--- a/atm-vfi_amd/network.py
+++ b/atm-vfi_amd/network.py
@@ -62,12 +62,36 @@
         self.p, self.n, self.h, self.w, self.chunk0, self.c = p, n, h, w, chunk0, c
 
 
+class _Walks:
+
+    force: Optional[int] = None
+
+    def __init__(self):
+        self._last: Dict[int, int] = {}
+
+    @staticmethod
+    def _key(buf) -> int:
+        t = buf.t if isinstance(buf, Planes) else buf
+        return t.untyped_storage().data_ptr()
+
+    def against(self, src) -> int:
+        if self.force is not None:
+            return self.force
+        return 1 - self._last.get(self._key(src), 0)
+
+    def wrote(self, walk: int, *dsts):
+        for d in dsts:
+            if d is not None:
+                self._last[self._key(d)] = walk
+
+
 class BlockRunner:
 
     def _init_runner(self):
         self._ops_obj = None
         self._bufs: Dict[Tuple, object] = {}
         self._geo: Dict[Tuple, Tuple[WindowGeometry, torch.Tensor, Optional[torch.Tensor]]] = {}
+        self._walks = _Walks()
 
     def buf(self, name: str, *shape) -> torch.Tensor:
         key = (name,) + tuple(shape)
@@ -115,16 +139,24 @@
         pl = self._plane_deconvs(ops)
         xn = self.buf(f"{tag}xn", mw, c)
         xn_p = self.planes(f"{tag}xn_p", mw, c) if pl else None
-        ops.layernorm(x, xn, P[f"{p}.norm1.weight"], P[f"{p}.norm1.bias"], src_row_map=row_map, **({"planes": xn_p} if pl else {}))
+        wk = self._walks
+        wn1 = 0
+        ops.layernorm(x, xn, P[f"{p}.norm1.weight"], P[f"{p}.norm1.bias"], src_row_map=row_map,
+                      **({"planes": xn_p, "walk": wn1} if pl else {}))
+        wk.wrote(wn1, xn, xn_p)
         qkv = self.buf(f"{tag}qkv", mw, 3 * c)
         ops.linear(xn_p if pl else xn, P[f"pk:{p}.attn.qkv.weight"], qkv)
+        wk.wrote(0, qkv)
         ao = None if pl else self.buf(f"{tag}ao", mw, c)
         ao_p = self.planes(f"{tag}ao_p", mw, c) if pl else None
         mo = self.buf(f"{tag}mo", mw, heads, 2) if cross else None
+        wat = wk.against(qkv) if pl else 0
         ops.window_attention(qkv, ao, mo, labels, bw, geo.n_windows, ws, heads, hd, bw // 2 if cross else 0,
-                             **({"planes": ao_p} if pl else {}))
+                             **({"planes": ao_p, "walk": wat} if pl else {}))
+        wk.wrote(wat, ao, ao_p)
         xb = self.buf(f"{tag}xb", frames * h * w, c)
         ops.linear(ao_p if pl else ao, P[f"pk:{p}.attn.proj.weight"], xb, bias=P[f"{p}.attn.proj.bias"], residual=xn, out_row_map=row_map)
+        wk.wrote(0, xb)
         if cross:
             mk = {} if motion_sink is None else {"planes": motion_sink[0], "planes_c0": motion_sink[1], "planes_gc": motion_sink[2]}
             ops.motion_head(mo, row_map, P[f"{p}.attn.mlp.0.weight"], P[f"{p}.attn.mlp.0.bias"],
@@ -133,12 +165,18 @@
         f1 = self.buf(f"{tag}fc1", frames, h, w, hid)
         if pl:
             y_p = self.planes(f"{tag}ln2_p", frames * h * w, c)
-            ops.layernorm(xb, None, P[f"{p}.norm2.weight"], P[f"{p}.norm2.bias"], planes=y_p)
+            wn2 = 0
+            ops.layernorm(xb, None, P[f"{p}.norm2.weight"], P[f"{p}.norm2.bias"], planes=y_p, walk=wn2)
+            wk.wrote(wn2, y_p)
             ops.linear(y_p, P[f"pk:{p}.mlp.fc1.weight"], f1.reshape(frames * h * w, hid), bias=P[f"{p}.mlp.fc1.bias"])
+            wk.wrote(0, f1)
             f2_p = self.planes(f"{tag}dw_p", frames * h * w, hid)
-            ops.dwconv_gelu(f1, None, P[f"pk:{p}.mlp.dwconv.dwconv.weight"], P[f"{p}.mlp.dwconv.dwconv.bias"], planes=f2_p)
+            wdw = 0
+            ops.dwconv_gelu(f1, None, P[f"pk:{p}.mlp.dwconv.dwconv.weight"], P[f"{p}.mlp.dwconv.dwconv.bias"], planes=f2_p, walk=wdw)
+            wk.wrote(wdw, f2_p)
             sk = {} if out_sink is None else {"sink": out_sink[0], "sink_c0": out_sink[1], "sink_gc": out_sink[2]}
             ops.linear(f2_p, P[f"pk:{p}.mlp.fc2.weight"], out, bias=P[f"{p}.mlp.fc2.bias"], residual=xb, **sk)
+            wk.wrote(0, out)
         else:
             y = self.buf(f"{tag}ln2", frames * h * w, c)
             ops.layernorm(xb, y, P[f"{p}.norm2.weight"], P[f"{p}.norm2.bias"])
@@ -577,7 +615,10 @@
             t = self.buf(f"{tag}fproj", f * h * w, c)
             ops.linear(fuse.p, P[f"pk:{p}.proj.weight"], t, bias=P[f"{p}.proj.bias"])
             out = self.buf(f"{tag}fnorm", f * h * w, c)
-            ops.layernorm(t, out, P[f"{p}.norm.weight"], P[f"{p}.norm.bias"])
+            self._walks.wrote(0, t)
+            wfn = 0
+            ops.layernorm(t, out, P[f"{p}.norm.weight"], P[f"{p}.norm.bias"], walk=wfn)
+            self._walks.wrote(wfn, out)
             return out
         f, h, w, c = fuse.shape
         self._conv_plain(ops, P, f"{p}.layers.0", mid, fuse[..., 0:c_mid], stride=2, pad=1, dil=1)
diff --git a/include/atmvfi.h b/include/atmvfi.h
--- a/include/atmvfi.h
+++ b/include/atmvfi.h
@@ -120,19 +120,19 @@
 int atmvfi_layernorm(const float* in, int in_ld, int64_t in_gstride, int in_rpg,
                      const int32_t* src_row_map, float* out, int out_ld,
                      const float* gamma, const float* beta, int64_t rows, int C,
-                     void* out_hi, void* out_lo, int plane_rows, void* stream);
+                     void* out_hi, void* out_lo, int plane_rows, int walk, void* stream);
 
 int atmvfi_dwconv3x3_gelu(const float* in, int in_ld, float* out, int out_ld,
                           const float* weight9, const float* bias,
-                          int N, int H, int W, int C, void* out_hi, void* out_lo, int plane_rows, void* stream);
+                          int N, int H, int W, int C, void* out_hi, void* out_lo, int plane_rows, int walk, void* stream);
 int atmvfi_pack_dw_weight(const float* src , float* dst , int C, void* stream);
 
 int atmvfi_window_attention(const float* qkv, float* out , float* motion,
                             const int32_t* labels, int Bw, int nW, int ws, int heads, int hd,
-                            int kv_shift, void* out_hi, void* out_lo, int plane_rows, void* stream);
+                            int kv_shift, void* out_hi, void* out_lo, int plane_rows, int walk, void* stream);
 int atmvfi_window_attention_f16x3(const float* qkv, float* out , float* motion,
                                   const int32_t* labels, int Bw, int nW, int ws, int heads, int hd,
-                                  int kv_shift, void* out_hi, void* out_lo, int plane_rows, void* stream);
+                                  int kv_shift, void* out_hi, void* out_lo, int plane_rows, int walk, void* stream);
 int atmvfi_window_attn_cross_motion(const float* qkv, float* out, float* motion, const int32_t* labels,
                                     int Bw, int nW, int ws, int heads, int hd, void* stream);
 int atmvfi_window_attn_self(const float* qkv, float* out, const int32_t* labels,
```
